# thierrydumas/context_adaptive_neural_network_based_prediction

Hardware: AMD Instinct MI355X
Metric: pnn_intra_pred_blocks_per_s (higher is better)
Workload: dtype f32; 1 GPU; configs[1]: 8x8 fully-connected PNN, batch 4096; batch_per_gpu=4096, global_batch=4096, weights=seeded random init (reference initialisers' statistics), parallelism=independent blocks sharded over ranks, no collective, timing=one region of K steps

## Files before the change

### context_adaptive_neural_network_based_prediction_amd/_lib.py

```python
import ctypes
import os

_HERE = os.path.dirname(os.path.abspath(__file__))
LIB_PATH = os.environ.get("PNN_LIB_PATH") or os.path.join(_HERE, "libpnn_hip.so")

f32p = ctypes.POINTER(ctypes.c_float)
i32p = ctypes.POINTER(ctypes.c_int32)
u8p = ctypes.POINTER(ctypes.c_uint8)
vp = ctypes.c_void_p
ci = ctypes.c_int


class TbDev(ctypes.Structure):
    _fields_ = [("origin", ctypes.c_int64), ("stride", ctypes.c_int32), ("above_mask", ctypes.c_uint32),
                ("left_units", ctypes.c_int32), ("reserved", ctypes.c_int32)]


BACKEND = ctypes.CFUNCTYPE(ci, vp, ci, f32p, f32p, ci, i32p, f32p)

SERVICE_SIGNATURES = {
    "pnn_service_run_backend": (ci, [ctypes.c_char_p, BACKEND, vp, ci, ci, ctypes.POINTER(ci), ctypes.POINTER(ctypes.c_long)]),
    "pnn_service_run": (ci, [ctypes.c_char_p, vp, ci, ci, ctypes.POINTER(ci), ctypes.POINTER(ctypes.c_long)]),
    "pnn_service_run_table": (ci, [ctypes.c_char_p, ctypes.c_char_p, ci, ctypes.c_float, ci, ci, ci, ctypes.POINTER(ci), ctypes.POINTER(ctypes.c_long)]),
    "pnn_client_connect": (ci, [ctypes.POINTER(vp), ctypes.c_char_p]),
    "pnn_client_predict_pel": (ci, [vp, ci, f32p, f32p, i32p, ci]),
    "pnn_client_predict_f32": (ci, [vp, ci, f32p, f32p, f32p]),
    "pnn_client_cache_stats": (ci, [vp, ctypes.POINTER(ctypes.c_long), ctypes.POINTER(ctypes.c_long)]),
    "pnn_client_arithmetic_tag": (ci, [vp, ci, ctypes.c_char_p, ctypes.c_size_t]),
    "pnn_client_close": (None, [vp]),
}

SIGNATURES = {
    "pnn_create_empty": (ci, [ctypes.POINTER(vp), ctypes.c_float, ci]),
    "pnn_create": (ci, [ctypes.POINTER(vp), ctypes.c_char_p, ci, ctypes.c_float, ci]),
    "pnn_load_model_file": (ci, [vp, ctypes.c_char_p]),
    "pnn_load_model_params": (ci, [vp, ci, ci, f32p, ctypes.c_size_t]),
    "pnn_model_info": (ci, [vp, ci, ctypes.POINTER(ci), ctypes.POINTER(ci), ctypes.POINTER(ctypes.c_long)]),
    "pnn_destroy": (None, [vp]),
    "pnn_last_error": (ctypes.c_char_p, [vp]),
    "pnn_mean": (ctypes.c_float, [vp]),
    "pnn_set_option": (ci, [vp, ctypes.c_char_p, ctypes.c_long]),
    "pnn_num_split_configs": (ci, []),
    "pnn_num_f32_configs": (ci, []),
    "pnn_check_range": (ci, [vp, vp, ctypes.POINTER(ctypes.c_long)]),
    "pnn_last_call_issued_flops": (ci, [vp, ctypes.POINTER(ctypes.c_double)]),
    "pnn_arithmetic_tag": (ci, [vp, ctypes.c_char_p, ctypes.c_size_t]),
    "pnn_host_alloc": (ci, [ctypes.POINTER(vp), ctypes.c_size_t]),
    "pnn_host_free": (None, [vp]),
    "pnn_streams_on_distinct_queues": (ci, [ctypes.POINTER(vp), ci]),
    "pnn_streams_release": (None, [ctypes.POINTER(vp), ci]),
    "pnn_cache_stats": (ci, [vp, ctypes.POINTER(ctypes.c_long), ctypes.POINTER(ctypes.c_long)]),
    "pnn_predict_fc": (ci, [vp, ci, f32p, ci, f32p]),
    "pnn_predict_conv": (ci, [vp, ci, f32p, f32p, ci, f32p]),
    "pnn_predict_pel": (ci, [vp, ci, f32p, f32p, ci, i32p, ci]),
    "pnn_predict_f32_pel": (ci, [vp, ci, f32p, f32p, ci, f32p, i32p]),
    "pnn_extract_context": (ci, [i32p, f32p, f32p, u8p] + [ci] * 8 + [ctypes.c_float]),
    "pnn_parse_model_table": (ci, [ctypes.c_char_p, ctypes.POINTER(ci), ctypes.POINTER(ci), ctypes.POINTER(ci),
                                   ctypes.POINTER(ctypes.c_char_p), ci]),
    "pnn_predict_fc_device": (ci, [vp, ci, vp, ci, vp, vp]),
    "pnn_predict_conv_device": (ci, [vp, ci, vp, vp, ci, vp, vp]),
    "pnn_make_tb_desc": (ci, [ctypes.POINTER(TbDev), ctypes.c_int64, ctypes.c_int32, u8p, ci, ci, ci]),
    "pnn_gather_device": (ci, [vp, ci, ci, vp, ci, vp, ci, vp, ctypes.c_long, vp, ctypes.c_long, vp]),
    "pnn_predict_tbs_device": (ci, [vp, ci, vp, ci, vp, ci, vp, vp, vp]),
    "pnn_block_cost_device": (ci, [vp, ci, vp, ci, vp, ci, vp, ci, vp, vp]),
    "pnn_predict_tbs_cost_device": (ci, [vp, ci, vp, vp, ci, vp, ci, ci, vp, vp, vp]),
    "pnn_hevc_intra_predict": (ci, [u8p, ci, ci, ci, ci, u8p]),
    "pnn_hevc_mode_uses_smoothing": (ci, [ci, ci]),
    "pnn_hevc_smoothed_reference_host": (ci, [vp, ci, ci, ci, ci, vp, ctypes.POINTER(ci)]),
    "pnn_hevc_intra_predict_hm": (ci, [u8p, ci, ci, ci, ci, ci, u8p]),
    "pnn_hevc_best_mode_device": (ci, [vp, ci, vp, ci, ci, vp, ci, vp, vp, vp, vp, vp]),
    "pnn_hevc_best_mode_hm_device": (ci, [vp, ci, vp, ci, ci, vp, ci, ci, vp, vp, vp, vp, vp]),
    "pnn_first_pass_list_size": (ci, [ci]),
    "pnn_hevc_mode_hads_host": (ci, [vp, ci, ci, vp, ci, ci, vp, vp, vp, vp, vp]),
    "pnn_hevc_mode_hads_device": (ci, [vp, ci, vp, ci, ci, vp, ci, vp, vp, vp, vp, vp, vp]),
    "pnn_hevc_mode_hads_hm_host": (ci, [vp, ci, ci, vp, ci, ci, vp, ci, vp, vp, vp, vp]),
    "pnn_hevc_mode_hads_hm_device": (ci, [vp, ci, vp, ci, ci, vp, ci, vp, ci, vp, vp, vp, vp, vp]),
    "pnn_first_pass_picture_pairs_device": (ci, [vp, ci, vp, vp, ci, ci, ci, vp, vp, ci, ci, ci, vp, vp, vp, vp, vp, vp]),
    "pnn_first_pass_picture_pairs_hm_device": (ci, [vp, ci, vp, vp, ci, ci, ci, vp, vp, ci, ci, ci, vp, ci, vp, vp, vp, vp, vp]),
    "pnn_ipfcns_forward_host": (ci, [ci, f32p, f32p, ci, ci, f32p]),
    "pnn_ipfcns_load": (ci, [vp, ci, f32p, ctypes.c_size_t]),
    "pnn_ipfcns_forward_device": (ci, [vp, ci, vp, ci, vp, vp]),
    "pnn_ipfcns_predict_device": (ci, [vp, ci, vp, ci, ci, ci, vp, vp, ci, vp, vp, vp, vp, vp, vp]),
    "pnn_score_pictures_device": (ci, [vp, ci, vp, ci, ci, ci, vp, vp, ci, ci, ci, vp, vp, vp, vp, vp, vp, vp, vp]),
    "pnn_score_picture_pairs_device": (ci, [vp, ci, vp, vp, ci, ci, ci, vp, vp, ci, ci, ci, vp, vp, vp, vp, vp, vp, vp, vp]),
    "pnn_score_picture_pairs_hm_device": (ci, [vp, ci, vp, vp, ci, ci, ci, vp, vp, ci, ci, ci, ci, vp, vp, vp, vp, vp, vp, vp, vp]),
    "pnn_score_f32_device": (ci, [vp, ci, vp, vp, ci, ci, ci, vp, vp, ci, vp, vp, vp]),
    "pnn_trquant_host": (ci, [vp, vp, ci, ci, ctypes.POINTER(ci), ci, vp, vp, vp, vp]),
    "pnn_trquant_stages_host": (ci, [vp, vp, ci, ci, vp, vp, vp, vp]),
    "pnn_trquant_device": (ci, [vp, ci, vp, vp, ci, ctypes.POINTER(ci), ci, vp, vp, vp, vp, vp]),
    "pnn_trquant_rate_host": (ci, [vp, vp, ci, ci, vp, ctypes.POINTER(ci), ci, vp, vp, vp, vp, vp]),
    "pnn_cabac_rate_levels_host": (ci, [vp, ci, ci, ci, ctypes.POINTER(ctypes.c_uint64)]),
    "pnn_trquant_rate_device": (ci, [vp, ci, vp, vp, ci, vp, ctypes.POINTER(ci), ci, vp, vp, vp, vp, vp, vp]),
    "pnn_sign_hide_unit_host": (ci, [vp, vp, vp, ci, ci]),
    "pnn_trquant_sdh_host": (ci, [vp, vp, ci, ci, vp, ctypes.POINTER(ci), ci, vp, vp, vp, vp, vp, ci]),
    "pnn_trquant_stages_sdh_host": (ci, [vp, vp, ci, ci, ci, ci, vp, vp, vp, vp, vp, vp]),
    "pnn_cabac_rate_levels_sdh_host": (ci, [vp, ci, ci, ci, ci, ctypes.POINTER(ctypes.c_uint64)]),
    "pnn_trquant_sdh_device": (ci, [vp, ci, vp, vp, ci, vp, ctypes.POINTER(ci), ci, vp, vp, vp, vp, vp, ci, vp]),
    "pnn_hm_intra_lambda": (ctypes.c_double, [ci]),
    "pnn_rd_pass_host": (ci, [vp, ci, ci, vp, ci, ci, vp, ci, ctypes.POINTER(ci), ci, ctypes.POINTER(ctypes.c_double), ci] + [vp] * 7),
    "pnn_rd_pass_workspace_bytes": (ctypes.c_size_t, [ci, ci, ci]),
    "pnn_rd_pass_device": (ci, [vp, ci, vp, ci, ci, vp, ci, vp, ci, ctypes.POINTER(ci), ci, ctypes.POINTER(ctypes.c_double), ci] + [vp] * 8 +
                           [ctypes.c_size_t, vp]),
    "pnn_rd_pass_picture_pairs_device": (ci, [vp, ci, vp, vp, ci, ci, ci, vp, vp, ci, ci, ci, vp, ci, ctypes.POINTER(ci), ci,
                                              ctypes.POINTER(ctypes.c_double), ci] + [vp] * 8 + [ctypes.c_size_t, vp]),
    "pnn_trquant_rdoq_host": (ci, [vp, vp, ci, ci, vp, ctypes.POINTER(ci), ci, vp, vp, vp, vp, vp, ci, ci, ctypes.POINTER(ctypes.c_double)]),
    "pnn_trquant_stages_rdoq_host": (ci, [vp, vp, ci, ci, ci, ci, ci, ctypes.c_double, ci, vp, vp, vp, vp, vp, vp]),
    "pnn_rdoq_unit_host": (ci, [vp, ci, ci, ci, ctypes.c_double, ci, ci, vp, ctypes.POINTER(ctypes.c_int32)]),
    "pnn_rdoq_est_bits_host": (ci, [ci, ci, vp]),
    "pnn_trquant_rdoq_device": (ci, [vp, ci, vp, vp, ci, vp, ctypes.POINTER(ci), ci, vp, vp, vp, vp, vp, ci, ci, ctypes.POINTER(ctypes.c_double),
                                     vp]),
    "pnn_rd_pass_rdoq_host": (ci, [vp, ci, ci, vp, ci, ci, vp, ci, ctypes.POINTER(ci), ci, ctypes.POINTER(ctypes.c_double), ci, ci] + [vp] * 7),
    "pnn_rd_pass_rdoq_device": (ci, [vp, ci, vp, ci, ci, vp, ci, vp, ci, ctypes.POINTER(ci), ci, ctypes.POINTER(ctypes.c_double), ci, ci] +
                                [vp] * 8 + [ctypes.c_size_t, vp]),
    "pnn_rd_pass_rdoq_picture_pairs_device": (ci, [vp, ci, vp, vp, ci, ci, ci, vp, vp, ci, ci, ci, vp, ci, ctypes.POINTER(ci), ci,
                                                   ctypes.POINTER(ctypes.c_double), ci, ci] + [vp] * 8 + [ctypes.c_size_t, vp]),
    "pnn_rd_pass_slot_count": (ci, [ci, ci]),
    "pnn_intra_mode_signal_host": (ci, [vp, vp, ci, ci, ci, vp, vp, vp, vp]),
    "pnn_first_pass_signal_host": (ci, [vp, ci, ci, vp, ci, ci, vp, ci, ctypes.POINTER(ci), ci, ctypes.POINTER(ctypes.c_double), vp, vp, vp, vp, vp]),
    "pnn_rd_pass_signal_host": (ci, [vp, ci, ci, vp, ci, ci, vp, ci, ctypes.POINTER(ci), ci, ctypes.POINTER(ctypes.c_double), ci, ci, ci, vp, vp] +
                                [vp] * 9),
    "pnn_rd_pass_signal_workspace_bytes": (ctypes.c_size_t, [ci, ci, ci, ci]),
    "pnn_rd_pass_signal_device": (ci, [vp, ci, vp, ci, ci, vp, ci, vp, ci, ctypes.POINTER(ci), ci, ctypes.POINTER(ctypes.c_double), ci, ci, ci,
                                       vp, vp] + [vp] * 10 + [ctypes.c_size_t, vp]),
    "pnn_rd_pass_signal_picture_pairs_device": (ci, [vp, ci, vp, vp, ci, ci, ci, vp, vp, ci, ci, ci, vp, ci, ctypes.POINTER(ci), ci,
                                                     ctypes.POINTER(ctypes.c_double), ci, ci, ci, vp, vp] + [vp] * 10 + [ctypes.c_size_t, vp]),
    "pnn_last_call_stats": (ci, [vp, ctypes.POINTER(ci), ctypes.POINTER(ctypes.c_double), ctypes.POINTER(ci)]),
    "pnn_launch_times": (ci, [vp, ci, ctypes.POINTER(ci), ctypes.POINTER(ctypes.c_double), ctypes.POINTER(ctypes.c_double)]),
}

_lib = None
SKIP_TORCH = False


def lib():
    global _lib
    if _lib is None:
        if not os.path.exists(LIB_PATH):
            raise ImportError("%s is missing: build it with `python -c 'import __graft_entry__ as g; g.build()'` "
                              "(or `make -C %s/csrc`). There is no CPU fallback." % (LIB_PATH, _HERE))
        if not SKIP_TORCH:
            try:
                import torch
            except ImportError:
                pass
        L = ctypes.CDLL(LIB_PATH)
        for name, (res, args) in list(SIGNATURES.items()) + list(SERVICE_SIGNATURES.items()):
            if os.environ.get("PNN_LIB_PATH") and not hasattr(L, name):
                continue
            fn = getattr(L, name)
            fn.restype = res
            fn.argtypes = args
        _lib = L
    return _lib


class PnnError(RuntimeError):
    pass


def check(rc, ctx=None):
    if rc != 0:
        msg = lib().pnn_last_error(ctx)
        raise PnnError("libpnn_hip error %d: %s" % (rc, msg.decode() if msg else "?"))
```

### context_adaptive_neural_network_based_prediction_amd/csrc/pnn_abi.cpp

```cpp
#include "pnn_ctx.h"

#include <algorithm>
#include <cmath>
#include <cstdarg>
#include <cstdio>
#include <cstdlib>
#include <cstring>
#include <ctime>
#include <condition_variable>
#include <mutex>
#include <thread>

using namespace pnn;

namespace pnn { std::recursive_mutex& unsafe_calls_lock() { static std::recursive_mutex m; return m; } }
namespace pnn { thread_local const LaunchEvents* g_launch_events = nullptr; thread_local double g_last_issued_frac = 1.0; }
namespace { thread_local std::string g_create_error; }
namespace pnn {

const DeviceInfo& device_info()
{
    static DeviceInfo cache[16];
    static std::once_flag filled[16];
    int dev = 0;
// ... 89 lines not shown
            HIPCHK(c, launch_gather(g, s));
            c->stat_launches++;
        }
        rc = run_net(c, m, ab, pa, lf, pl, nb, d_out_f32 ? d_out_f32 + b0 * w2 : nullptr, d_dst ? d_dst + b0 * w2 : nullptr, s, split_ctx);
        c->lazy = pnn_ctx::LazyGather();
        if (rc) return rc;
    }
    return PNN_OK;
}

}

namespace {

Model* model_for(pnn_ctx* c, int width, int want_fc , int* rc)
{
    const int idx = width_index(width);
    if (!c) { *rc = PNN_E_ARG; return nullptr; }
    if (idx < 0 || !c->models[idx]) { *rc = fail(c, PNN_E_MODEL, "no model loaded for width %d", width); return nullptr; }
    Model* m = c->models[idx];
    if (want_fc >= 0 && (int)m->is_fc != want_fc) {
        *rc = fail(c, PNN_E_MODEL, "model for width %d is %s", width, m->is_fc ? "fully-connected" : "convolutional");
        return nullptr;
    }
    *rc = PNN_OK;
    return m;
}

int wait_stream(pnn_ctx* c, hipStream_t s)
{
    HIPCHK(c, hipStreamSynchronize(s));
    return PNN_OK;
}

int wait_done_flag(pnn_ctx* c, hipStream_t s, long n = 1, int width = 4)
{
    const unsigned* const flag0 = reinterpret_cast<const unsigned*>(c->h_range) + (c->done_nflags > 0 ? pnn_ctx::kDoneFlag0 : 1);
    const int nflags = c->done_nflags > 0 ? c->done_nflags : 1;
    int first_open = 0;
    auto raised = [&]() {
        while (first_open < nflags && __atomic_load_n(flag0 + first_open, __ATOMIC_ACQUIRE) == c->done_seq) ++first_open;
        return first_open == nflags;
    };
    if (c->opt_wait_sleep) {
        constexpr double kMarginUs = 14.0, kMinSleepUs = 12.0;
        int b = 0;
        while ((2L << b) <= n && b < 11) b++;
        const int wi = width_index(width) < 0 ? 0 : width_index(width);
        double& ema = c->wait_ema_us[wi][b];
        timespec t0, t1;
        clock_gettime(CLOCK_MONOTONIC, &t0);
        const double nap = ema - kMarginUs;
        bool overslept = false;
        if (nap >= kMinSleepUs) {
            timespec ts{0, (long)(nap * 1e3)};
            nanosleep(&ts, nullptr);
            overslept = raised();
        }
        for (long spins = 0; !raised(); spins++) {
            if (spins < 400000) { __builtin_ia32_pause(); continue; }
            HIPCHK(c, hipStreamSynchronize(s));
            if (!raised()) return fail(c, PNN_E_HIP, "the pass finished without raising its completion flag");
            break;
        }
        clock_gettime(CLOCK_MONOTONIC, &t1);
        const double us = (t1.tv_sec - t0.tv_sec) * 1e6 + (t1.tv_nsec - t0.tv_nsec) * 1e-3;
        ema = overslept ? ema * 0.85 : (ema == 0.0 ? us : 0.9 * ema + 0.1 * us);
        return PNN_OK;
    }
    for (long spins = 0; !raised(); spins++) {
        if (spins < 200000) { __builtin_ia32_pause(); continue; }
        HIPCHK(c, hipStreamSynchronize(s));
        if (!raised()) return fail(c, PNN_E_HIP, "the pass finished without raising its completion flag");
        break;
    }
    return PNN_OK;
}

template <typename Pass>
int range_fallback(pnn_ctx* c, long n, Pass pass, hipStream_t s)
{
    constexpr long kPerBlockMax = 256;
    *c->h_range = 0;
    c->range_fallbacks++;
    const long keep = c->opt_precision;
    int rc = PNN_OK;
    if (n == 1 || n > kPerBlockMax) {
        c->opt_precision = 0;
        rc = pass(0, n);
        c->opt_precision = keep;
        if (rc) return rc;
        HIPCHK(c, hipStreamSynchronize(s));
        return PNN_OK;
    }
    for (long i = 0; i < n; i++) {
        if ((rc = pass(i, 1))) return rc;
        HIPCHK(c, hipStreamSynchronize(s));
        if (!*c->h_range) continue;
        *c->h_range = 0;
        c->opt_precision = 0;
        rc = pass(i, 1);
        c->opt_precision = keep;
        if (rc) return rc;
        HIPCHK(c, hipStreamSynchronize(s));
    }
    return PNN_OK;
}

struct PnnwHeader { char magic[4]; uint32_t version, width, is_fc; uint64_t n_params, reserved; };

enum OptionEffect { kStore, kRetune, kNewTuneGen };

int set_canonical_order(pnn_ctx* c, long value)
{
    if (value != 1) return fail(c, PNN_E_ARG, "canonical_order = %ld: the kernels with another summation order were removed; 1 is the only mode", value);
    return PNN_OK;
}

int set_stream_priority(pnn_ctx* c, long value)
{
    HIPCHK(c, hipSetDevice(c->device));
    int least = 0, greatest = 0;
    HIPCHK(c, hipDeviceGetStreamPriorityRange(&least, &greatest));
    const int pr = value < 0 ? greatest : value > 0 ? least : (least + greatest) / 2;
    hipStream_t ns = nullptr;
    HIPCHK(c, hipStreamCreateWithPriority(&ns, hipStreamNonBlocking, pr));
    if (c->stream) { (void)hipStreamSynchronize(c->stream); if (c->stream_owned) (void)hipStreamDestroy(c->stream); }
    c->stream = ns; c->stream_owned = true;
    return PNN_OK;
}

int set_stream(pnn_ctx* c, long value)
{
    if (!value) return fail(c, PNN_E_ARG, "stream = NULL");
    HIPCHK(c, hipSetDevice(c->device));
    if (c->stream) { (void)hipStreamSynchronize(c->stream); if (c->stream_owned) (void)hipStreamDestroy(c->stream); }
    c->stream = reinterpret_cast<hipStream_t>(value); c->stream_owned = false;
    return PNN_OK;
}

int set_cache_mb(pnn_ctx* c, long value) { c->opt_cache_mb = value; c->cache_hits = c->cache_misses = 0; return PNN_OK; }
int set_ws_cap_mb(pnn_ctx* c, long value) { c->ws_cap_bytes = (size_t)value << 20; return PNN_OK; }

struct OptionRow { const char* name; long pnn_ctx::*field; const char* env; OptionEffect effect; int (*set)(pnn_ctx*, long); };
const OptionRow kOptions[] = {
    {"precision",            &pnn_ctx::opt_precision,           "PNN_PRECISION",        kStore,       nullptr},
    {"canonical_order",      nullptr,                           nullptr,                kStore,       set_canonical_order},
    {"f32_small",            &pnn_ctx::opt_f32_small,           "PNN_F32_SMALL",        kStore,       nullptr},
    {"f32_small_max_tiles",  &pnn_ctx::opt_f32_small_tiles,     "PNN_F32_SMALL_TILES",  kStore,       nullptr},
    {"fc_out_f32",           &pnn_ctx::opt_fc_out_f32,          nullptr,                kStore,       nullptr},
    {"chain_io",             &pnn_ctx::opt_chain_io,            "PNN_CHAIN_IO",         kStore,       nullptr},
    {"tails",                &pnn_ctx::opt_tails,               "PNN_TAILS",            kStore,       nullptr},
    {"f32_cfg",              &pnn_ctx::opt_f32_cfg,             "PNN_F32_CFG",          kStore,       nullptr},
    {"f32_seg_mode",         &pnn_ctx::opt_f32_seg_mode,        "PNN_F32_SEG_MODE",     kRetune,      nullptr},
    {"f32_persist",          &pnn_ctx::opt_f32_persist,         "PNN_F32_PERSIST",      kRetune,      nullptr},
    {"f32_overlap",          &pnn_ctx::opt_f32_overlap,         "PNN_F32_OVERLAP",      kStore,       nullptr},
    {"fuse_last",            &pnn_ctx::opt_fuse_last,           "PNN_FUSE_LAST",        kStore,       nullptr},
    {"seg_fold",             &pnn_ctx::opt_seg_fold,            nullptr,                kStore,       nullptr},
    {"f32_small_deep",       &pnn_ctx::opt_f32_small_deep,      "PNN_F32_SMALL_DEEP",   kStore,       nullptr},
    {"sp_cfg",               &pnn_ctx::opt_sp_cfg,              nullptr,                kStore,       nullptr},
    {"ring",                 &pnn_ctx::opt_ring,                "PNN_RING",             kRetune,      nullptr},
    {"convimg",              &pnn_ctx::opt_convimg,             "PNN_CONVIMG",          kRetune,      nullptr},
    {"small",                &pnn_ctx::opt_small,               "PNN_SMALL",            kStore,       nullptr},
    {"small_max_tiles",      &pnn_ctx::opt_small_tiles,         nullptr,                kStore,       nullptr},
    {"fuse_first",           &pnn_ctx::opt_fuse_first,          "PNN_FUSE_FIRST",       kRetune,      nullptr},
    {"fuse_tail",            &pnn_ctx::opt_fuse_tail,           "PNN_FUSE_TAIL",        kRetune,      nullptr},
    {"ring_pm",              &pnn_ctx::opt_ring_pm,             "PNN_RING_PM",          kRetune,      nullptr},
    {"autotune",             &pnn_ctx::opt_autotune,            "PNN_AUTOTUNE",         kNewTuneGen,  nullptr},
    {"host_slice",           &pnn_ctx::opt_host_slice,          nullptr,                kStore,       nullptr},
    {"pair",                 &pnn_ctx::opt_pair,                nullptr,                kStore,       nullptr},
    {"branch_streams",       &pnn_ctx::opt_branch_streams,      "PNN_BRANCH_STREAMS",   kStore,       nullptr},
    {"fuse_gather",          &pnn_ctx::opt_fuse_gather,         "PNN_FUSE_GATHER",      kStore,       nullptr},
    {"cache_mb",             &pnn_ctx::opt_cache_mb,            "PNN_CACHE_MB",         kStore,       set_cache_mb},
    {"flag_wait",            &pnn_ctx::opt_flag_wait,           "PNN_FLAG_WAIT",        kStore,       nullptr},
    {"stream_priority",      nullptr,                           nullptr,                kStore,       set_stream_priority},
    {"stream",               nullptr,                           nullptr,                kStore,       set_stream},
    {"wait_sleep",           &pnn_ctx::opt_wait_sleep,          "PNN_WAIT_SLEEP",       kStore,       nullptr},
    {"graphs",               &pnn_ctx::opt_graphs,              "PNN_GRAPHS",           kStore,       nullptr},
    {"max_chunk",            &pnn_ctx::opt_max_chunk,           "PNN_MAX_CHUNK",        kStore,       nullptr},
    {"ws_cap_mb",            nullptr,                           nullptr,                kStore,       set_ws_cap_mb},
    {"time_launches",        &pnn_ctx::opt_time_launches,       nullptr,                kStore,       nullptr},
};

}

extern "C" {

int pnn_create_empty(pnn_ctx** out, float mean, int device)
{
    PNN_UNSAFE_CALLS_GUARD;
    if (!out) return fail(nullptr, PNN_E_ARG, "`out` is NULL");
    *out = nullptr;
    int ndev = 0;
    if (hipGetDeviceCount(&ndev) != hipSuccess || ndev <= 0)
        return fail(nullptr, PNN_E_HIP, "no HIP device is visible: libpnn_hip.so has no CPU fallback");
    if (device < 0 || device >= ndev) return fail(nullptr, PNN_E_ARG, "device %d out of range [0, %d)", device, ndev);
    pnn_ctx* c = new pnn_ctx();
    c->device = device; c->mean = mean;
    if (hipSetDevice(device) != hipSuccess || hipStreamCreateWithFlags(&c->stream, hipStreamNonBlocking) != hipSuccess) {
        delete c;
        return fail(nullptr, PNN_E_HIP, "cannot initialise HIP device %d", device);
    }
    for (const OptionRow& o : kOptions)
        if (o.env)
            if (const char* e = getenv(o.env)) c->*o.field = atol(e);
    if (hipHostMalloc((void**)&c->h_range, (pnn_ctx::kDoneFlag0 + pnn_ctx::kDoneFlagsMax) * 4, hipHostMallocDefault) != hipSuccess) {
        pnn_destroy(c);
        return fail(nullptr, PNN_E_NOMEM, "hipHostMalloc of the range flag failed");
    }
    *c->h_range = 0;
    for (int i = 1; i < pnn_ctx::kDoneFlag0 + pnn_ctx::kDoneFlagsMax; i++) c->h_range[i] = 0;
    if (hipMalloc((void**)&c->d_done, 256) != hipSuccess || hipMemset(c->d_done, 0, 256) != hipSuccess) {
        pnn_destroy(c);
        return fail(nullptr, PNN_E_NOMEM, "hipMalloc of the completion counter failed");
    }
    if (hipMalloc((void**)&c->d_seg_cnt, pnn_ctx::kCntWords * 4) != hipSuccess || hipMemset(c->d_seg_cnt, 0, pnn_ctx::kCntWords * 4) != hipSuccess) {
        pnn_destroy(c);
        return fail(nullptr, PNN_E_NOMEM, "hipMalloc of the K-segment counters failed");
    }
    if (hipMalloc(&c->d_zero, 4096) != hipSuccess || hipMemset(c->d_zero, 0, 4096) != hipSuccess) {
        pnn_destroy(c);
        return fail(nullptr, PNN_E_NOMEM, "hipMalloc of the zero page failed");
    }
    *out = c;
    return PNN_OK;
}

int pnn_load_model_params(pnn_ctx* c, int width, int is_fc, const float* params, size_t n)
{
    if (!c || !params) return fail(c, PNN_E_ARG, "NULL argument");
    const int idx = width_index(width);
    if (idx < 0) return fail(c, PNN_E_ARG, "width %d is not in {4, 8, 16, 32, 64}", width);
    HIPCHK(c, hipSetDevice(c->device));
    Model* m = nullptr;
    const int rc = build_model(c, width, is_fc, params, n, &m);
    if (rc) return rc;
    PNN_UNSAFE_CALLS_GUARD;
    free_model(c->models[idx]);
    c->models[idx] = m;
    c->tuned.clear(); c->tune_gen++;
    cache_clear(c);
    return PNN_OK;
}

int pnn_load_model_file(pnn_ctx* c, const char* path)
{
    if (!c || !path) return fail(c, PNN_E_ARG, "NULL argument");
    std::vector<char> data;
    if (!read_file(path, &data)) return fail(c, PNN_E_IO, "The model file at \"%s\" cannot be loaded.", path);
    if (data.size() < sizeof(PnnwHeader)) return fail(c, PNN_E_IO, "%s: truncated header", path);
    PnnwHeader h;
    memcpy(&h, data.data(), sizeof h);
    if (memcmp(h.magic, "PNNW", 4) || h.version != 1) return fail(c, PNN_E_IO, "%s is not a PNNW v1 file", path);
    if (data.size() != sizeof h + h.n_params * 4) return fail(c, PNN_E_IO, "%s: size does not match its header", path);
    std::vector<float> params(h.n_params);
    memcpy(params.data(), data.data() + sizeof h, h.n_params * 4);
    return pnn_load_model_params(c, (int)h.width, (int)h.is_fc, params.data(), params.size());
}

int pnn_create(pnn_ctx** out, const char* table_path, int use_pair, float mean, int device)
{
    if (!out) return fail(nullptr, PNN_E_ARG, "`out` is NULL");
    *out = nullptr;
    std::vector<TableEntry> entries;
    std::string err;
    int rc = parse_table(table_path, &entries, &err);
    if (rc) return fail(nullptr, rc, "%s", err.c_str());
    bool have_pair = false;
    for (const TableEntry& e : entries) have_pair |= e.is_pair != 0;
    const int want_pair = (have_pair && use_pair) ? 1 : 0;
    pnn_ctx* c = nullptr;
    if ((rc = pnn_create_empty(&c, mean, device))) return rc;
    std::string dir(table_path);
    const size_t slash = dir.find_last_of('/');
    dir = slash == std::string::npos ? std::string(".") : dir.substr(0, slash);
    static const int widths[5] = {4, 8, 16, 32, 64};
    for (int wi = 0; wi < 5; wi++) {
        const TableEntry* hit = nullptr;
        for (const TableEntry& e : entries)
            if (e.width == widths[wi] && e.is_pair == want_pair && e.channel == 0) hit = &e;
        if (!hit) {
            rc = fail(nullptr, PNN_E_MODEL, "model table has no (%d, %s, luminance) entry", widths[wi], want_pair ? "pair" : "single");
            break;
        }
        std::string p = hit->path;
        if (!p.empty() && p[0] != '/') {
            FILE* f = fopen((dir + "/" + p).c_str(), "rb");
            if (f) { fclose(f); p = dir + "/" + p; }
        }
        rc = pnn_load_model_file(c, p.c_str());
        if (rc) { g_create_error = c->err; break; }
        const Model* m = c->models[wi];
        if (m->width != widths[wi]) { rc = fail(nullptr, PNN_E_MODEL, "%s holds a width-%d model, table says %d", p.c_str(), m->width, widths[wi]); break; }
    }
    if (rc) { pnn_destroy(c); return rc; }
    *out = c;
    return PNN_OK;
}

void pnn_destroy(pnn_ctx* c)
{
    if (!c) return;
    PNN_UNSAFE_CALLS_GUARD;
    (void)hipSetDevice(c->device);
    if (c->stream) (void)hipStreamSynchronize(c->stream);
    cache_clear(c);
    for (Model*& m : c->models) { free_model(m); m = nullptr; }
    for (Model*& m : c->ipfcns) { free_model(m); m = nullptr; }
    for (DevBuf& b : c->ws) if (b.p) (void)hipFree(b.p);
    for (DevBuf& b : c->ipfcns_ws) if (b.p) (void)hipFree(b.p);
    for (DevBuf& b : c->score_ws) if (b.p) (void)hipFree(b.p);
    for (DevBuf& b : c->stage_in) if (b.p) (void)hipFree(b.p);
    for (DevBuf& b : c->stage_out) if (b.p) (void)hipFree(b.p);
    if (c->stage_tbs.p) (void)hipFree(c->stage_tbs.p);
    for (auto& b : c->seg_part) if (b.p) (void)hipFree(b.p);
    if (c->d_zero) (void)hipFree(c->d_zero);
    if (c->d_done) (void)hipFree(c->d_done);
    if (c->d_seg_cnt) (void)hipFree(c->d_seg_cnt);
    if (c->copy_in) {
        (void)hipStreamDestroy(c->copy_in); (void)hipStreamDestroy(c->copy_out);
        for (int i = 0; i < 2; i++) { (void)hipEventDestroy(c->ev_in[i]); (void)hipEventDestroy(c->ev_pass[i]); (void)hipEventDestroy(c->ev_out[i]); }
    }
    for (pnn::DevBuf* b : {&c->stage2_in[0], &c->stage2_in[1], &c->stage2_out[0], &c->stage2_out[1]}) if (b->p) (void)hipFree(b->p);
    if (c->side_stream) { (void)hipStreamSynchronize(c->side_stream); (void)hipStreamDestroy(c->side_stream); }
    if (c->ev_fork) (void)hipEventDestroy(c->ev_fork);
    if (c->ev_join) (void)hipEventDestroy(c->ev_join);
    if (c->h_pin) (void)hipHostFree(c->h_pin);
    if (c->h_range) (void)hipHostFree(c->h_range);
    if (c->stream && c->stream_owned) (void)hipStreamDestroy(c->stream);
    delete c;
}

const char* pnn_last_error(const pnn_ctx* c) { return c ? c->err.c_str() : g_create_error.c_str(); }
float pnn_mean(const pnn_ctx* c) { return c ? c->mean : 0.f; }

int pnn_model_info(const pnn_ctx* c, int width, int* is_fc, int* n_layers, long* n_params)
{
    const int idx = width_index(width);
    if (!c || idx < 0 || !c->models[idx]) return PNN_E_MODEL;
    if (is_fc) *is_fc = c->models[idx]->is_fc;
    if (n_layers) *n_layers = c->models[idx]->n_layers;
    if (n_params) *n_params = c->models[idx]->n_params;
    return PNN_OK;
}

int pnn_arithmetic_tag(const pnn_ctx* c, char* out, size_t bytes)
{
    if (!c || !out || bytes == 0) return PNN_E_ARG;
    if (c->opt_precision == 0)
        snprintf(out, bytes, "pnn-order-6:f32:fmaf-chain k=0,8,1,9..7,15 per 16:kseg %d/%d:fc-kseg %d:fc-out-seg 160", kSegDepth, kSegMinDepth, 16 * kFcSegChunks);
    else
        snprintf(out, bytes, "pnn-order-5:split-f16x3:hi*hi,hi*lo,lo*hi per 16:fc-out-seg %d", 16 * kFuseSegChunks);
    return PNN_OK;
}

int pnn_num_split_configs(void) { return tapgemm_sp_num_cfgs() + convimg_sp_num_cfgs() + tapgemm_ring_num_cfgs(); }
int pnn_num_f32_configs(void) { return tapgemm_f32_num_cfgs(); }

int pnn_set_option(pnn_ctx* c, const char* name, long value)
{
    if (!c || !name) return PNN_E_ARG;
    PNN_UNSAFE_CALLS_GUARD;
    const OptionRow* o = std::find_if(std::begin(kOptions), std::end(kOptions), [name](const OptionRow& r) { return !strcmp(r.name, name); });
    if (o == std::end(kOptions)) return fail(c, PNN_E_ARG, "unknown option %s", name);
    if (o->set) {
        if (const int rc = o->set(c, value)) return rc;
    } else {
        c->*o->field = value;
    }
    if (o->effect == kRetune) c->tuned.clear();
    if (o->effect != kStore) c->tune_gen++;
    cache_clear(c);
    return PNN_OK;
}

int pnn_last_call_stats(const pnn_ctx* c, int* n_gemm, double* flops, int* n_launches)
{
    if (!c) return PNN_E_ARG;
    if (n_gemm) *n_gemm = c->stat_gemm_launches;
    if (flops) *flops = c->stat_gemm_flops;
    if (n_launches) *n_launches = c->stat_launches;
    return PNN_OK;
}

int pnn_last_call_issued_flops(const pnn_ctx* c, double* flops)
{
    if (!c || !flops) return PNN_E_ARG;
    *flops = c->stat_gemm_flops - c->stat_gemm_flops_skipped;
    return PNN_OK;
}

int pnn_launch_times(pnn_ctx* c, int kind, int* n_launches, double* total_us, double* total_flops)
{
    if (!c) return PNN_E_ARG;
    int n = 0;
    double us = 0, fl = 0;
    std::vector<pnn_ctx::LaunchRec> keep;
    for (pnn_ctx::LaunchRec& r : c->launch_recs) {
        if (r.kind != kind) { keep.push_back(r); continue; }
        HIPCHK(c, hipEventSynchronize(r.e1));
        float ms = 0.f;
        HIPCHK(c, hipEventElapsedTime(&ms, r.e0, r.e1));
        us += ms * 1e3; fl += r.flops; n++;
        (void)hipEventDestroy(r.e0);
        (void)hipEventDestroy(r.e1);
    }
    c->launch_recs.swap(keep);
    if (n_launches) *n_launches = n;
    if (total_us) *total_us = us;
    if (total_flops) *total_flops = fl;
    return PNN_OK;
}


int pnn_predict_fc_device(pnn_ctx* c, int width, const float* d_ctx, int n, float* d_out, void* stream)
{
    int rc;
    Model* m = model_for(c, width, 1, &rc);
    if (!m) return rc;
    if (n < 0 || (n > 0 && (!d_ctx || !d_out))) return fail(c, PNN_E_ARG, "bad buffers / batch size");
    HIPCHK(c, hipSetDevice(c->device));
    if ((rc = pending_range_error(c))) return rc;
    reset_stats(c);
    hipStream_t s = (hipStream_t)stream;
    return run_net(c, m, d_ctx, 5L * width * width, nullptr, 0, n, d_out, nullptr, s);
}

int pnn_predict_conv_device(pnn_ctx* c, int width, const float* d_above, const float* d_left, int n, float* d_out, void* stream)
{
    int rc;
    Model* m = model_for(c, width, 0, &rc);
    if (!m) return rc;
    if (n < 0 || (n > 0 && (!d_above || !d_left || !d_out))) return fail(c, PNN_E_ARG, "bad buffers / batch size");
    HIPCHK(c, hipSetDevice(c->device));
    if ((rc = pending_range_error(c))) return rc;
    reset_stats(c);
    hipStream_t s = (hipStream_t)stream;
    return run_net(c, m, d_above, 3L * width * width, d_left, 2L * width * width, n, d_out, nullptr, s);
}

int pnn_gather_device(pnn_ctx* c, int width, int unit, const void* d_plane, int pel_bytes, const pnn_tb_dev* d_tbs, int n,
                      float* d_above, long pitch_above, float* d_left, long pitch_left, void* stream)
{
    if (!c) return PNN_E_ARG;
    if (width_index(width) < 0 || (unit != 4 && unit != 2) || n < 0 || (n > 0 && (!d_plane || !d_tbs || !d_above || !d_left)))
        return fail(c, PNN_E_ARG, "bad gather arguments");
    if (pel_bytes != 4 && pel_bytes != 1) return fail(c, PNN_E_ARG, "pel_bytes must be 4 (HM Pel) or 1 (uint8)");
    HIPCHK(c, hipSetDevice(c->device));
    GatherParams g;
    g.plane = d_plane; g.pel_bytes = pel_bytes; g.tbs = reinterpret_cast<const TbDev*>(d_tbs); g.N = n; g.w = width;
    g.unit = unit; g.mean = c->mean; g.above = d_above; g.left = d_left; g.pitch_above = pitch_above; g.pitch_left = pitch_left;
    g.split = 0;
    HIPCHK(c, launch_gather(g, (hipStream_t)stream));
    return PNN_OK;
}

int pnn_predict_tbs_device(pnn_ctx* c, int width, const void* d_plane, int pel_bytes, const pnn_tb_dev* d_tbs, int n,
                           int32_t* d_dst, float* d_out_f32, void* stream)
{
    int rc;
    Model* m = model_for(c, width, -1, &rc);
    if (!m) return rc;
    if (n < 0 || (n > 0 && (!d_plane || !d_tbs || (!d_dst && !d_out_f32)))) return fail(c, PNN_E_ARG, "bad buffers / batch size");
    HIPCHK(c, hipSetDevice(c->device));
    if ((rc = pending_range_error(c))) return rc;
    reset_stats(c);
    return tbs_pass(c, m, d_plane, pel_bytes, d_tbs, n, d_dst, d_out_f32, (hipStream_t)stream);
}

int pnn_block_cost_device(pnn_ctx* c, int width, const void* d_org_plane, int pel_bytes, const pnn_tb_dev* d_tbs, int n,
                          const int32_t* d_pred, int hadamard, uint32_t* d_cost, void* stream)
{
    if (!c) return PNN_E_ARG;
    if (width_index(width) < 0 || n < 0 || (n > 0 && (!d_org_plane || !d_tbs || !d_pred || !d_cost))) return fail(c, PNN_E_ARG, "bad cost arguments");
    if (pel_bytes != 4 && pel_bytes != 1) return fail(c, PNN_E_ARG, "pel_bytes must be 4 (HM Pel) or 1 (uint8)");
    HIPCHK(c, hipSetDevice(c->device));
    BlockCostParams b;
    b.org_plane = d_org_plane; b.pel_bytes = pel_bytes; b.tbs = reinterpret_cast<const TbDev*>(d_tbs); b.N = n; b.w = width;
    b.pred = d_pred; b.hadamard = hadamard; b.cost = d_cost;
    HIPCHK(c, launch_block_cost(b, (hipStream_t)stream));
    return PNN_OK;
}

int pnn_predict_tbs_cost_device(pnn_ctx* c, int width, const void* d_plane, const void* d_org_plane, int pel_bytes,
                                const pnn_tb_dev* d_tbs, int n, int hadamard, uint32_t* d_cost, int32_t* d_dst, void* stream)
{
    if (!c) return PNN_E_ARG;
    if (n > 0 && (!d_org_plane || !d_cost)) return fail(c, PNN_E_ARG, "bad cost arguments");
    int rc;
    if (!d_dst && n > 0) {
        if ((rc = dev_reserve(c, c->stage_out[1], (size_t)n * width * width * 4))) return rc;
        d_dst = (int32_t*)c->stage_out[1].p;
    }
    if ((rc = pnn_predict_tbs_device(c, width, d_plane, pel_bytes, d_tbs, n, d_dst, nullptr, stream))) return rc;
    rc = pnn_block_cost_device(c, width, d_org_plane, pel_bytes, d_tbs, n, d_dst, hadamard, d_cost, stream);
    if (rc == PNN_OK) c->stat_launches++;
    return rc;
}


static uint64_t hash_bytes(const void* data, size_t bytes, uint64_t h = 0x9e3779b97f4a7c15ull)
{
    const unsigned char* p = static_cast<const unsigned char*>(data);
    size_t i = 0;
    for (; i + 8 <= bytes; i += 8) {
        uint64_t v;
        memcpy(&v, p + i, 8);
        h = (h ^ v) * 0xff51afd7ed558ccdull;
        h ^= h >> 32;
    }
    for (; i < bytes; i++) h = (h ^ p[i]) * 0x100000001b3ull;
    return h ^ (h >> 29);
}

static bool all_finite(const float* x, size_t n)
{
    uint32_t bad = 0;
    for (size_t i = 0; i < n; i++) {
        uint32_t u;
        memcpy(&u, x + i, 4);
        bad |= (uint32_t)((u & 0x7f800000u) == 0x7f800000u);
    }
    return bad == 0;
}

static int host_predict(pnn_ctx* c, Model* m, const float* above, const float* left, int n, float* out, int32_t* dst, int dst_stride);

static int host_predict_sliced(pnn_ctx* c, Model* m, const float* above, const float* left, int n, float* out, int32_t* dst, int dst_stride, long slice)
{
    const int w = m->width;
    const long w2 = (long)w * w;
    const size_t pa = (size_t)(m->is_fc ? 5 : 3) * w2, pl = m->is_fc ? 0 : (size_t)2 * w2;
    HIPCHK(c, hipSetDevice(c->device));
    reset_stats(c);
// ... 447 lines not shown
```

### context_adaptive_neural_network_based_prediction_amd/csrc/pnn_ctx.h

```cpp
#pragma once
#include "../../include/pnn_hip.h"
#include "pnn_kernels.h"
#include "pnn_host.h"

#include <functional>
#include <map>
#include <mutex>
#include <tuple>
#include <string>
#include <vector>

namespace pnn {

constexpr int kHidden = 1200;
constexpr int kFuseSegChunks = 10;
inline int strides_for(int w, int* st)
{
    switch (w) {
    case 4: st[0] = 1; st[1] = 1; return 2;
    case 8: st[0] = 2; st[1] = 1; return 2;
    case 16: st[0] = 2; st[1] = 1; st[2] = 2; st[3] = 1; return 4;
    case 32: st[0] = 2; st[1] = 2; st[2] = 1; st[3] = 2; st[4] = 1; return 5;
    case 64: st[0] = 2; st[1] = 2; st[2] = 2; st[3] = 2; st[4] = 1; return 5;
    default: return -1;
    }
}

inline int width_index(int w)
{
    switch (w) { case 4: return 0; case 8: return 1; case 16: return 2; case 32: return 3; case 64: return 4; default: return -1; }
}

inline bool ipfcns_dims(int w, int* K, int* H)
{
    switch (w) {
    case 4: *H = 512; break;
    case 8: case 16: *H = 1024; break;
    case 32: *H = 2048; break;
    default: return false;
    }
    *K = 64 + 32 * w;
    return true;
}
inline int ipfcns_index(int w) { return w == 4 ? 0 : w == 8 ? 1 : w == 16 ? 2 : w == 32 ? 3 : -1; }
inline long ipfcns_n_params(int w)
{
    int K, H;
    if (!ipfcns_dims(w, &K, &H)) return -1;
    const long o = (long)w * w;
    return (long)H * K + 2L * H + 2L * ((long)H * H + 2L * H) + o * H + o;
}

struct DevBuf {
    void* p = nullptr;
    size_t bytes = 0;
};

struct GemmLayer {
    TapGemmParams proto{};
    float* d_w = nullptr;
    float* d_w_ch = nullptr;
    float* d_w_sp = nullptr;
    float sp_inv_scale = 1.f;
    float* d_bias = nullptr;
    double k_total = 0;
    int nseg = 1;
    int fc_seg_chunks = 0;
    long out_per_block = 0;
};
struct Conv1Layer { Conv1Params proto{}; float* d_w = nullptr; float* d_w_sp = nullptr; float sp_inv_scale = 1.f; int npad = 0; float* d_bias = nullptr; long out_per_block = 0; };
struct TConv1Layer { TConv1Params proto{}; float* d_w = nullptr; };
struct MergerLayer { MergerParams proto{}; float* d_w = nullptr; float* d_bias = nullptr; };

struct Model {
    int width = 0;
    bool is_fc = false;
    long n_params = 0;
    int n_layers = 0;
    std::vector<GemmLayer> fc;
    Conv1Layer first[2];
    std::vector<GemmLayer> branch[2];
    MergerLayer merger;
    std::vector<GemmLayer> tconv;
    TConv1Layer last;
    int C = 0;
    long pmax = 0;
    float* d_slope[3] = {nullptr, nullptr, nullptr};
    std::vector<void*> allocs;
};

}

struct pnn_ctx {
    int device = 0;
    float mean = 0.f;
    hipStream_t stream = nullptr;
    pnn::Model* models[5] = {nullptr, nullptr, nullptr, nullptr, nullptr};
    pnn::Model* ipfcns[4] = {nullptr, nullptr, nullptr, nullptr};
    pnn::DevBuf ipfcns_ws[4];
    pnn::DevBuf score_ws[2];
    pnn::DevBuf ws[6];
    bool stream_owned = true;
    long opt_branch_streams = 1;
    hipStream_t side_stream = nullptr;
    hipEvent_t ev_fork = nullptr, ev_join = nullptr;
    pnn::DevBuf stage_in[2], stage_out[2], stage_tbs;
    pnn::DevBuf stage2_in[2], stage2_out[2];
    hipStream_t copy_in = nullptr, copy_out = nullptr;
    hipEvent_t ev_in[2] = {nullptr, nullptr}, ev_pass[2] = {nullptr, nullptr}, ev_out[2] = {nullptr, nullptr};
    long opt_host_slice = 0;
    pnn::DevBuf seg_part[2];
    struct CacheEntry { uint64_t hash = 0; bool valid = false; std::vector<float> in, out; std::vector<int32_t> pel; };
    std::vector<CacheEntry> cache[5];
    long opt_cache_mb = 0;
    long cache_hits = 0, cache_misses = 0;
    char* h_pin = nullptr;
    struct GraphEntry {
        hipGraphExec_t exec = nullptr;
        int uses = 0;
        bool failed = false, armed = false;
        unsigned seq = 0;
        int nflags = 0;
        int stat_gemm_launches = 0, stat_launches = 0;
        double stat_gemm_flops = 0, stat_gemm_flops_skipped = 0;
    };
    std::map<std::tuple<const void*, int, int>, GraphEntry> graphs;
    long opt_graphs = 0;
    void* d_zero = nullptr;
    long opt_max_chunk = 0;
    long opt_precision = 0;
    long opt_sp_cfg = -1;
    long opt_f32_small = 1;
    long opt_fc_out_f32 = 1;
    long opt_seg_fold = 1;
    long opt_f32_small_deep = 1;
    unsigned* d_seg_cnt = nullptr;
    bool seg_cnt_dirty = false;
    static constexpr int kSegCntTiles = 2048;
    static constexpr int kTailCnt = 2048, kCntWords = 2 * kSegCntTiles + kTailCnt;
    long opt_tails = 1;
    long opt_chain_io = 1;
    long opt_f32_small_tiles = 1024;
    long opt_f32_overlap = 1;
    long opt_f32_cfg = -1;
    long opt_fuse_first = 1;
    long opt_fuse_last = 1;
    long opt_f32_seg_mode = 0;
    long opt_f32_persist = -1;
    long opt_ring = 1;
    long opt_small = 1;
    long opt_small_tiles = 512;
    long opt_pair = 1;
    long opt_convimg = 1;
    long opt_autotune = 2;
    std::map<std::pair<const void*, long>, int> tuned;
    long tune_gen = 0;
    std::map<std::pair<const void*, long>, long> overlap_ready;
    long opt_time_launches = 0;
    struct LaunchRec { hipEvent_t e0, e1; int kind; double flops; };
    std::vector<LaunchRec> launch_recs;
    int* h_range = nullptr;
    long range_fallbacks = 0;
    const float* host_input = nullptr;
    struct LazyGather { const void* plane = nullptr; const void* tbs = nullptr; int pel_bytes = 0, unit = 0; } lazy;
    long opt_fuse_gather = 1;
    long opt_fuse_tail = 1;
    unsigned* d_done = nullptr;
    unsigned done_seq = 0;
    unsigned done_seq_alloc = 0;
    bool done_want = false, done_last_chunk = true, done_armed = false;
    int done_nflags = 0;
    static constexpr int kDoneFlag0 = 16, kDoneFlagsMax = 512;
    long opt_flag_wait = 1;
    long opt_wait_sleep = 0;
    double wait_ema_us[5][12] = {};
    long opt_ring_pm = 1;
    size_t ws_cap_bytes = (size_t)8 << 30;
    static constexpr int kDiagLaunches = 32, kDiagWgs = 2048;
    void* diag_stamps = nullptr;
    int diag_launch = 0;
    std::vector<std::string> diag_names;
    std::vector<int> diag_wgs;
    std::vector<double> diag_k;
    std::string err;
    int stat_gemm_launches = 0, stat_launches = 0;
    double stat_gemm_flops = 0;
    double stat_gemm_flops_skipped = 0;
};

namespace pnn {

int fail(pnn_ctx* c, int code, const char* fmt, ...);
std::recursive_mutex& unsafe_calls_lock();
#define PNN_UNSAFE_CALLS_GUARD std::lock_guard<std::recursive_mutex> unsafe_guard_(pnn::unsafe_calls_lock())

#define HIPCHK(c, expr)                                                                             \
    do {                                                                                            \
        hipError_t e_ = (expr);                                                                     \
        if (e_ != hipSuccess) return pnn::fail((c), PNN_E_HIP, "%s failed: %s", #expr, hipGetErrorString(e_)); \
    } while (0)

int dev_reserve(pnn_ctx* c, DevBuf& b, size_t bytes);
void reset_stats(pnn_ctx* c);
int pending_range_error(pnn_ctx* c);
int tbs_pass(pnn_ctx* c, Model* m, const void* d_plane, int pel_bytes, const pnn_tb_dev* d_tbs, long n, int32_t* d_dst, float* d_out_f32,
             hipStream_t s);
int build_model(pnn_ctx* c, int width, int is_fc, const float* params, size_t n, Model** out);
int build_ipfcns_model(pnn_ctx* c, int width, const float* params, size_t n, Model** out);
void free_model(Model* m);
int convimg_images(const TapGemmParams& p, const TileCfg& t, bool one_tap);
int choose_cfg_convimg(const TapGemmParams& p, bool one_tap);
bool pnn_ring_few_images(const TapGemmParams& p, long M, double k_total);
int choose_cfg_ring(const TapGemmParams& p, long M, bool one_tap, double k_total, bool fused = false);
int choose_cfg_sp(const pnn_ctx* c, long M, int cout, int ncls, int cin, double k_total);
int choose_cfg_f32(const pnn_ctx* c, long M, int cout, int ncls, int cin, double k_total, bool fused, double* cost_out = nullptr);
inline DoneSignal take_done_signal(pnn_ctx* c)
{
    if (!c->done_want || !c->done_last_chunk || !c->d_done) return DoneSignal{nullptr, nullptr, 0, 0};
    c->done_armed = true;
    c->done_nflags = 0;
    c->done_seq = ++c->done_seq_alloc;
    return DoneSignal{c->d_done, reinterpret_cast<unsigned*>(c->h_range) + 1, c->done_seq, 0};
}
inline DoneSignal take_done_signal_per_wg(pnn_ctx* c, int nwg)
{
    if (nwg < 1 || nwg > pnn_ctx::kDoneFlagsMax) return take_done_signal(c);
    if (!c->done_want || !c->done_last_chunk || !c->d_done) return DoneSignal{nullptr, nullptr, 0, 0};
    c->done_armed = true;
    c->done_nflags = nwg;
    c->done_seq = ++c->done_seq_alloc;
    return DoneSignal{nullptr, reinterpret_cast<unsigned*>(c->h_range) + pnn_ctx::kDoneFlag0, c->done_seq, 1};
}
int tuned_cfg(pnn_ctx* c, const void* key, long M, int ncodes, int rule, const std::function<bool(int)>& legal,
              const std::function<hipError_t(int)>& launch, hipStream_t s, int* cfg, float* best_us);
bool env_debug();
bool env_profile();
bool env_f32s_diag();
bool env_f32_diag();
bool env_sp_diag();
void* diag_stamp_slot(pnn_ctx* c, const char* name, long wgs, double k);
int diag_f32_small(pnn_ctx* c, const GemmLayer& L, const TapGemmParams& ps, int nseg, const float* host_rows, hipStream_t s);
int diag_f32_tiles(pnn_ctx* c, const GemmLayer& L, const TapGemmParams& p, int tile, bool fused, int par_segs, hipStream_t s);
int diag_sp(pnn_ctx* c, const GemmLayer& L, const TapGemmParams& p, int cfg, hipStream_t s);
long chunk_blocks(const pnn_ctx* c, const Model* m);
bool pass_uses_split(const pnn_ctx* c, const Model* m, long nb);
bool conv_pass_fuses_first(pnn_ctx* c, Model* m, long nb);
long ipfcns_chunk(const pnn_ctx* c, const Model* m);
int ipfcns_pass(pnn_ctx* c, const Model* m, const float* d_x, long n, float* d_fc4, hipStream_t s);
int run_net(pnn_ctx* c, Model* m, const float* d_a, long pitch_a, const float* d_l, long pitch_l, long n, float* d_out,
            int32_t* d_dst, hipStream_t s, bool ctx_is_split = false);

}
```

### context_adaptive_neural_network_based_prediction_amd/csrc/pnn_diag.cpp

```cpp
#include "pnn_ctx.h"

#include <algorithm>
#include <cmath>
#include <cstdio>
#include <cstdlib>
#include <vector>

namespace pnn {

bool env_debug() { static const bool on = getenv("PNN_DEBUG") != nullptr; return on; }
bool env_profile() { static const bool on = getenv("PNN_PROFILE") != nullptr; return on; }
bool env_f32s_diag() { static const bool on = getenv("PNN_F32S_DIAG") != nullptr; return on; }
bool env_f32_diag() { static const bool on = getenv("PNN_F32_DIAG") != nullptr; return on; }
bool env_sp_diag() { static const bool on = getenv("PNN_SP_DIAG") != nullptr; return on; }

void* diag_stamp_slot(pnn_ctx* c, const char* name, long wgs, double k)
{
    if (!c->diag_stamps || c->diag_launch >= pnn_ctx::kDiagLaunches || wgs > pnn_ctx::kDiagWgs) return nullptr;
    c->diag_names.push_back(name);
    c->diag_wgs.push_back((int)wgs);
    c->diag_k.push_back(k);
    return (char*)c->diag_stamps + (size_t)c->diag_launch++ * pnn_ctx::kDiagWgs * 64;
}

int diag_f32_small(pnn_ctx* c, const GemmLayer& L, const TapGemmParams& ps, int nseg, const float* host_rows, hipStream_t s)
{
    HIPCHK(c, hipStreamSynchronize(s));
    if (dev_reserve(c, c->stage_tbs, (size_t)4 << 20)) return PNN_E_NOMEM;
    HIPCHK(c, hipMemset(c->stage_tbs.p, 0, (size_t)4 << 20));
    TapGemmParams q = ps;
    q.Xlo = c->stage_tbs.p;
    HIPCHK(c, launch_tapgemm_f32_small(q, s, host_rows, (int)c->opt_f32_small_deep));
    HIPCHK(c, hipStreamSynchronize(s));
    const size_t nwg = std::min<size_t>((size_t)tapgemm_f32_small_tiles(ps), ((size_t)4 << 20) / 64);
    std::vector<unsigned long long> hbuf(8 * nwg);
    HIPCHK(c, hipMemcpy(hbuf.data(), c->stage_tbs.p, hbuf.size() * 8, hipMemcpyDeviceToHost));
    double cyc = 0, ticks = 0, chunks = 0;
    unsigned long long r0 = ~0ull, r1 = 0;
    for (size_t i = 0; i < nwg; i++) { cyc += (double)hbuf[8 * i]; ticks += (double)hbuf[8 * i + 1]; chunks += (double)hbuf[8 * i + 2]; r0 = std::min(r0, hbuf[8 * i + 3]); r1 = std::max(r1, hbuf[8 * i + 3] + hbuf[8 * i + 1]); }
    fprintf(stderr, "[pnn-f32s-diag] M=%ld K=%.0f N=%d ncls=%d nseg=%d: %zu WGs, loop %.0f cycles for %.0f chunks = %.0f cycles per chunk (160 = the chain), %.2f us, clock %.0f MHz; first loop start -> last loop end %.1f us\n",
            (long)ps.M, L.k_total, ps.Cout, ps.ncls, nseg, nwg, cyc / nwg, chunks / nwg, cyc / std::max(1.0, chunks), ticks / nwg / 100.0, cyc / std::max(1.0, ticks) * 100.0, (double)(r1 - r0) / 100.0);
    return PNN_OK;
}

int diag_f32_tiles(pnn_ctx* c, const GemmLayer& L, const TapGemmParams& p, int tile, bool fused, int par_segs, hipStream_t s)
{
    const TileCfg t = tapgemm_f32_cfg(tile);
    const long M = p.M;
    HIPCHK(c, hipStreamSynchronize(s));
    if (dev_reserve(c, c->stage_tbs, (size_t)16 << 20)) return PNN_E_NOMEM;
    TapGemmParams q = p;
    q.Xlo = c->stage_tbs.p;
    HIPCHK(c, hipMemset(c->stage_tbs.p, 0, (size_t)16 << 20));
    for (int rep = 0; rep < 400; rep++) HIPCHK(c, launch_tapgemm_f32(q, tile, fused, s));
    HIPCHK(c, hipStreamSynchronize(s));
    const size_t nwg = (size_t)((M + 128L * t.rt - 1) / (128L * t.rt)) * ((p.Cout + 32L * t.nt - 1) / (32L * t.nt)) * p.ncls * par_segs;
    std::vector<unsigned long long> hbuf(8 * nwg);
    HIPCHK(c, hipMemcpy(hbuf.data(), c->stage_tbs.p, hbuf.size() * 8, hipMemcpyDeviceToHost));
    double sum[4] = {0, 0, 0, 0};
    unsigned long long r0 = ~0ull, r1 = 0;
    for (size_t i = 0; i < nwg; i++) {
        for (int k = 0; k < 4; k++) sum[k] += (double)hbuf[8 * i + k];
        r0 = std::min(r0, hbuf[8 * i + 4]); r1 = std::max(r1, hbuf[8 * i + 4] + hbuf[8 * i + 3]);
    }
    size_t late = 0; unsigned long long life_max = 0;
    for (size_t i = 0; i < nwg; i++) { late += hbuf[8 * i + 4] > r0 + 500; life_max = std::max(life_max, hbuf[8 * i + 3]); }
    const double chunks = std::ceil(L.k_total / 16.0 / p.ncls / par_segs / t.kc) * t.kc;
    const double cyc = (sum[0] + sum[1] + sum[2]) / nwg, rt_ticks = sum[3] / nwg;
    fprintf(stderr, "[pnn-f32diag] M=%ld K=%.0f N=%d {%d,%d,%d}%s: %zu WGs; wave 0 mean cycles: prologue %.0f  loop %.0f (MFMA work %.0f = %.3f)  epilogue %.0f;"
            " lifetime %.1f us (max %.1f), in-kernel clock %.0f MHz; first start -> last end %.1f us, %zu workgroups start > 5 us late\n", M, L.k_total, p.Cout, t.rt, t.nt, t.kc, fused ? "+out" : "", nwg,
            sum[0] / nwg, sum[1] / nwg, chunks * 8 * t.rt * t.nt * 64, chunks * 8 * t.rt * t.nt * 64 / (sum[1] / nwg), sum[2] / nwg, rt_ticks / 100.0, (double)life_max / 100.0,
            cyc / (rt_ticks / 100.0), (double)(r1 - r0) / 100.0, late);
    return PNN_OK;
}

int diag_sp(pnn_ctx* c, const GemmLayer& L, const TapGemmParams& p, int cfg, hipStream_t s)
{
    HIPCHK(c, hipStreamSynchronize(s));
    const TileCfg tt = tapgemm_sp_cfg(cfg);
    const long M = p.M, bm = 32L * tt.rt * tt.wm, bn = 32L * tt.nt * (4 / tt.wm);
    const size_t nwg = (size_t)((M + bm - 1) / bm) * ((p.Cout + bn - 1) / bn) * p.ncls;
    std::vector<unsigned long long> h(4 * nwg);
    HIPCHK(c, hipMemcpy(h.data(), c->stage_tbs.p, h.size() * 8, hipMemcpyDeviceToHost));
    double sum[4] = {0, 0, 0, 0};
    for (size_t i = 0; i < nwg; i++) for (int k = 0; k < 4; k++) sum[k] += (double)h[4 * i + k];
    const double stages = std::ceil(L.k_total / 16.0 / p.ncls / tt.kc);
    fprintf(stderr, "[pnn-diag] M=%ld K=%.0f N=%d cfg {%d,%d,%d,wm%d}: per stage (cycles, wave 0 mean over %zu WGs): issue %.0f  mfma %.0f  store %.0f  barrier %.0f\n",
            M, L.k_total, p.Cout, tt.rt, tt.nt, tt.kc, tt.wm, nwg, sum[0] / nwg / stages, sum[1] / nwg / stages, sum[2] / nwg / stages, sum[3] / nwg / stages);
    return PNN_OK;
}

}
```

### context_adaptive_neural_network_based_prediction_amd/csrc/pnn_gemm_f32.hip

```cpp
#include "pnn_kernels.h"
#include "pnn_device_common.h"

#include <algorithm>
#include <cstdio>
#include <cstdlib>

namespace pnn {

typedef float f32x16 __attribute__((ext_vector_type(16)));

namespace {

__device__ __forceinline__ void dma16(const __amdgpu_buffer_rsrc_t& r, unsigned voff, unsigned soff, f32x4* l)
{
    __builtin_amdgcn_raw_ptr_buffer_load_lds(r, (__attribute__((address_space(3))) void*)l, 16, voff, soff, 0, 0);
}

template <int N>
__device__ __forceinline__ void wait_vm_le()
{
    asm volatile("s_waitcnt vmcnt(%0)" ::"n"(N) : "memory");
}

}

template <int RT, int NT, int KC, bool FUSE, int SEQ>
__device__ __forceinline__ void f32_tile(const TapGemmParams& p, f32x4* const lds, const int bx, const int by, const int bz, const int gx, const int gy)
{
    static_assert(KC >= 2 && KC % 2 == 0, "fragment sets alternate by chunk parity");
    constexpr int BM = 128 * RT, BN = 32 * NT;
    constexpr int E = 4 * BN;
    constexpr int SE = KC * E;
    constexpr int NDMA = SE / 64;
    constexpr int NPW = NDMA / 4;
    constexpr int W2R = BN / 4;
    static_assert(SE % 64 == 0 && NDMA % 4 == 0, "a stage is a whole number of wave instructions, the same number for every wave");
    constexpr int SLOTS = 8 * NT * RT;
    constexpr bool kCoalescedOut = true;
    f32x4* const W2s = lds + 3 * SE;

    const int tid = threadIdx.x;
    const int lane = tid & 63, wave = __builtin_amdgcn_readfirstlane(tid >> 6);
    const int l31 = lane & 31, h = lane >> 5;
    const int nseg = (!FUSE && !SEQ && p.nseg > 1) ? p.nseg : 1;
    const int cls = nseg > 1 ? bz / nseg : bz;
    const int seg = bz - cls * nseg;
    const int n0 = by * BN;
    const int m0 = bx * BM + wave * (32 * RT);
#ifdef PNN_F32_DIAG
    const unsigned long long dq0 = __builtin_amdgcn_s_memtime(), dr0 = __builtin_amdgcn_s_memrealtime();
    unsigned long long dq1 = 0, dq2 = 0;
#endif

    const int SP = p.SH * p.SW;
    const int cpt = p.Cin >> 4;
    const int t0 = p.tap_begin[cls], t1 = p.tap_begin[cls + 1];
    const int pmg = p.pm_groups;
    int pmi = 0, pmj = 0, mblk = 0;
    unsigned tmask = t1 - t0 >= 32 ? 0xffffffffu : (1u << (t1 - t0)) - 1u;
    unsigned smask = 0xffffffffu;
    if (nseg > 1) {
        const int base = (t1 - t0) / nseg, rem = (t1 - t0) - base * nseg;
        smask = ((1u << (base + (seg < rem ? 1 : 0))) - 1u) << (seg * base + (seg < rem ? seg : rem));
        tmask &= smask;
    }
    if (pmg) {
        const int gc = bx / (SP * 8), r = bx - gc * (SP * 8);
        const int c = gc < (pmg >> 3) ? 8 : (pmg & 7);
        const int pr = r / c;
        const int pos = SP <= 64 ? (int)((p.pos_order[pr >> 2] >> ((pr & 3) * 8)) & 0xffu) : pr;
        pmi = pos / p.SW;
        pmj = pos - pmi * p.SW;
        mblk = (gc * 8 + r - pr * c) * BM;
        unsigned m = 0;
        for (int t = t0; t < t1; t++) {
            const int tp = p.tap[t];
            const int iy = pmi * p.a + (tp >> 16), ix = pmj * p.a + (int)(short)(tp & 0xffff);
            if ((unsigned)iy < (unsigned)p.IH && (unsigned)ix < (unsigned)p.IW) m |= 1u << (t - t0);
        }
        m &= smask;
        tmask = m ? m : (smask & (0u - smask));
    }
    auto next_tap = [&](int t) {
        const unsigned rest = tmask & ~((2u << t) - 1u);
        return rest ? (int)__builtin_ctz(rest) : t;
    };
    int pb[RT], pi[RT], pj[RT];
    bool mv[RT];
#pragma unroll
    for (int rt = 0; rt < RT; rt++) {
        const int row = wave * (32 * RT) + rt * 32 + l31;
        if (pmg) {
            mv[rt] = mblk + row < p.nblk;
            pb[rt] = mv[rt] ? mblk + row : 0; pi[rt] = pmi; pj[rt] = pmj;
            continue;
        }
        const int mg = m0 + rt * 32 + l31;
        mv[rt] = mg < p.M;
        const int mc = mv[rt] ? mg : 0;
        if (SP == 1) { pb[rt] = mc; pi[rt] = 0; pj[rt] = 0; }
        else {
            const int b = mc / SP;
            const int r = mc - b * SP;
            pb[rt] = b;
            pi[rt] = r / p.SW;
            pj[rt] = r - pi[rt] * p.SW;
        }
    }
    const int nchunks = __builtin_popcount(tmask) * cpt;
    const int nstages = (nchunks + KC - 1) / KC;
    const int sq_n = SEQ != 0 ? p.nseg : 1, sq_base = (t1 - t0) / sq_n, sq_rem = (t1 - t0) - sq_base * sq_n;
    auto seg_stages = [&](int k) {
        const unsigned mk = ((1u << (sq_base + (k < sq_rem ? 1 : 0))) - 1u) << (k * sq_base + (k < sq_rem ? k : sq_rem));
        return __builtin_popcount(tmask & mk) * (cpt / KC);
    };
    int sq_k = 0, fold_at = SEQ == 1 ? seg_stages(0) : 0, sq_done = 0;

    const unsigned wbytes = (unsigned)p.chunk_begin[p.ncls] * 4u * (unsigned)p.Npad * 16u;
    const __amdgpu_buffer_rsrc_t wrsrc = __builtin_amdgcn_make_buffer_rsrc((void*)p.Wp, 0, wbytes, 0x00020000);
    const unsigned wcls = (unsigned)p.chunk_begin[cls] * 4u * (unsigned)p.Npad * 16u;
    const unsigned wchunk = 4u * (unsigned)p.Npad * 16u;
    int dt = (int)__builtin_ctz(tmask), dcc = 0;
    auto advance_d = [&]() {
        dcc += KC;
        if (dcc >= cpt) {
            const int n = next_tap(dt);
            if (n != dt) { dt = n; dcc = 0; } else dcc -= KC;
        }
    };
    unsigned bsrc[NPW];
#pragma unroll
    for (int ii = 0; ii < NPW; ii++) {
        const int i = wave + 4 * ii;
        const int e = 64 * i + lane;
        const int j = e / E, ee = e - j * E;
        const int q = ee / BN, nn = ee - q * BN;
        bsrc[ii] = (unsigned)(((j * 4 + q) * p.Npad + n0 + nn) << 4) + wcls;
    }
    auto dma_b = [&](int buf, int ii) {
        dma16(wrsrc, bsrc[ii], (unsigned)(dt * cpt + dcc) * wchunk, lds + buf * SE + 64 * (wave + 4 * ii));
    };

    const __amdgpu_buffer_rsrc_t xrsrc = __builtin_amdgcn_make_buffer_rsrc((void*)p.X, 0, p.x_bytes, 0x00020000);
    unsigned aoff[RT];
    auto tap_setup = [&](int tp) {
        const int dy = tp >> 16, dx = (int)(short)(tp & 0xffff);
#pragma unroll
        for (int rt = 0; rt < RT; rt++) {
            const int iy = pi[rt] * p.a + dy, ix = pj[rt] * p.a + dx;
            const bool ok = mv[rt] && (unsigned)iy < (unsigned)p.IH && (unsigned)ix < (unsigned)p.IW;
            const unsigned off = ((unsigned)((pb[rt] * p.IH + iy) * p.IW + ix) * (unsigned)p.Cin + (h << 3)) << 2;
            aoff[rt] = ok ? off : 0x80000000u;
        }
    };
    int lt = (int)__builtin_ctz(tmask), lcc = 0;
    tap_setup(p.tap[t0 + lt]);
    int ltp_next = p.tap[t0 + next_tap(lt)];
    auto load_a_chunk = [&](int j, f32x4 (&dst)[KC][RT][2]) {
        const int cj = lcc + j < cpt ? lcc + j : cpt - 1;
#pragma unroll
        for (int rt = 0; rt < RT; rt++) {
            dst[j][rt][0] = __builtin_bit_cast(f32x4, __builtin_amdgcn_raw_buffer_load_b128(xrsrc, aoff[rt], cj << 6, 0));
            dst[j][rt][1] = __builtin_bit_cast(f32x4, __builtin_amdgcn_raw_buffer_load_b128(xrsrc, aoff[rt] + 16u, cj << 6, 0));
        }
    };
    auto advance_a = [&]() {
        lcc += KC;
        if (lcc >= cpt) {
            const int n = next_tap(lt);
            if (n != lt) {
                lcc = 0;
                lt = n;
                tap_setup(ltp_next);
                ltp_next = p.tap[t0 + next_tap(lt)];
            }
        }
    };

    f32x16 acc[RT][NT];
    f32x16 total[SEQ ? RT : 1][SEQ ? NT : 1];
#pragma unroll
    for (int rt = 0; rt < RT; rt++)
#pragma unroll
        for (int nt = 0; nt < NT; nt++)
#pragma unroll
            for (int i = 0; i < 16; i++) {
                acc[rt][nt][i] = 0.f;
                if (SEQ) total[SEQ ? rt : 0][SEQ ? nt : 0][i] = 0.f;
            }
    auto fold_now = [&](bool first = false) {
#pragma unroll
        for (int rt = 0; rt < RT; rt++)
#pragma unroll
            for (int nt = 0; nt < NT; nt++)
#pragma unroll
                for (int i = 0; i < 16; i++) {
                    if (first) total[SEQ ? rt : 0][SEQ ? nt : 0][i] = acc[rt][nt][i];
                    else total[SEQ ? rt : 0][SEQ ? nt : 0][i] += acc[rt][nt][i];
                    acc[rt][nt][i] = 0.f;
                }
    };
    auto after_stage = [&]() {
        if (SEQ != 1) return;
        ++sq_done;
        if (sq_done != fold_at || sq_k >= sq_n - 1) return;
        fold_now();
        do { ++sq_k; fold_at += seg_stages(sq_k); } while (fold_at == sq_done && sq_k < sq_n - 1);
    };

    auto read_wf = [&](int buf, int j, int nt, f32x4 (&wf)[NT][2]) {
        wf[nt][0] = lds[buf * SE + j * E + (2 * h) * BN + nt * 32 + l31];
        wf[nt][1] = lds[buf * SE + j * E + (2 * h + 1) * BN + nt * 32 + l31];
    };

    f32x4 a0[KC][RT][2], a1[KC][RT][2];
    f32x4 wf0[NT][2], wf1[NT][2];
#pragma unroll
    for (int ii = 0; ii < NPW; ii++) dma_b(0, ii);
    advance_d();
#pragma unroll
    for (int j = 0; j < KC; j++) load_a_chunk(j, a0);
    advance_a();
#pragma unroll
    for (int ii = 0; ii < NPW; ii++) dma_b(1, ii);
    advance_d();
    if (FUSE) {
        const __amdgpu_buffer_rsrc_t w2rsrc = __builtin_amdgcn_make_buffer_rsrc((void*)p.W2p, 0, (unsigned)p.K2chunks * 4u * (unsigned)p.Npad2 * 16u, 0x00020000);
        for (int r = wave; r < W2R; r += 4) dma16(w2rsrc, (unsigned)(((n0 >> 2) + r) * p.Npad2 + lane) << 4, 0, W2s + r * 64);
    }
    static_assert(!FUSE || W2R % 4 == 0, "every wave fetches the same number of rows of the output layer's tile");
    wait_vm_le<NPW + (FUSE ? W2R / 4 : 0)>();
    __builtin_amdgcn_s_barrier();
#pragma unroll
    for (int nt = 0; nt < NT; nt++) read_wf(0, 0, nt, wf0);

    auto stage = [&](int buf, f32x4 (&acur)[KC][RT][2], f32x4 (&anxt)[KC][RT][2]) {
        const int buf1 = buf == 2 ? 0 : buf + 1, buf2 = buf == 0 ? 2 : buf - 1;
#pragma unroll
        for (int j = 0; j < KC; j++) {
            constexpr int kLast = KC - 1;
            const int d0 = j * NPW / KC, d1 = (j + 1) * NPW / KC;
            const int nops = 2 * NT + 2 * RT + (d1 - d0);
            if (j == kLast) {
                wait_vm_le<(2 * RT) * (KC - 1) + (KC - 1) * NPW / KC>();
                asm volatile("s_waitcnt lgkmcnt(0)" ::: "memory");
                __builtin_amdgcn_s_barrier();
            }
            f32x4 (&wc)[NT][2] = (j & 1) ? wf1 : wf0;
            f32x4 (&wn)[NT][2] = (j & 1) ? wf0 : wf1;
#pragma unroll
            for (int e = 0; e < 8; e++)
#pragma unroll
                for (int nt = 0; nt < NT; nt++)
#pragma unroll
                    for (int rt = 0; rt < RT; rt++) {
                        acc[rt][nt] = __builtin_amdgcn_mfma_f32_32x32x2f32(wc[nt][e >> 2][e & 3], acur[j][rt][e >> 2][e & 3], acc[rt][nt], 0, 0, 0);
                        const int sl = (e * NT + nt) * RT + rt;
                        const int k = (sl * nops + SLOTS - 1) / SLOTS;
                        if (k < nops && k * SLOTS / nops == sl) {
                            if (k < 2 * NT) {
                                const int fnt = k >> 1, fh = k & 1;
                                const int src = (j == kLast ? buf1 * SE : buf * SE + (j + 1) * E) + (2 * h + fh) * BN + fnt * 32 + l31;
                                wn[fnt][fh] = lds[src];
                            } else if (k < 2 * NT + 2 * RT) {
                                const int ar = (k - 2 * NT) >> 1, ah = (k - 2 * NT) & 1;
                                const int cj = lcc + j < cpt ? lcc + j : cpt - 1;
                                anxt[j][ar][ah] = __builtin_bit_cast(f32x4, __builtin_amdgcn_raw_buffer_load_b128(xrsrc, aoff[ar] + 16u * ah, cj << 6, 0));
                            } else {
                                dma_b(buf2, d0 + (k - 2 * NT - 2 * RT));
                            }
                        }
                        __builtin_amdgcn_sched_barrier(0);
                    }
        }
        advance_a();
        advance_d();
    };
#ifdef PNN_F32_DIAG
    dq1 = __builtin_amdgcn_s_memtime();
#endif
    auto tail = [&](int buf, f32x4 (&acur)[KC][RT][2], int nlive) {
#pragma unroll
        for (int j = 0; j < KC; j++) {
            if (j >= nlive) break;
            f32x4 (&wc)[NT][2] = (j & 1) ? wf1 : wf0;
            f32x4 (&wn)[NT][2] = (j & 1) ? wf0 : wf1;
#pragma unroll
            for (int e = 0; e < 8; e++)
#pragma unroll
                for (int nt = 0; nt < NT; nt++)
#pragma unroll
                    for (int rt = 0; rt < RT; rt++) {
                        acc[rt][nt] = __builtin_amdgcn_mfma_f32_32x32x2f32(wc[nt][e >> 2][e & 3], acur[j][rt][e >> 2][e & 3], acc[rt][nt], 0, 0, 0);
                        const int sl = (e * NT + nt) * RT + rt;
                        constexpr int nops = 2 * NT;
                        const int k = (sl * nops + SLOTS - 1) / SLOTS;
                        if (j + 1 < KC && k < nops && k * SLOTS / nops == sl)
                            wn[k >> 1][k & 1] = lds[buf * SE + (j + 1) * E + (2 * h + (k & 1)) * BN + (k >> 1) * 32 + l31];
                        __builtin_amdgcn_sched_barrier(0);
                    }
        }
    };
    const int nlive = nchunks - (nstages - 1) * KC;
    int s = 0, buf = 0;
    if (SEQ == 1) while (fold_at == 0 && sq_k < sq_n - 1) { ++sq_k; fold_at += seg_stages(sq_k); }
    if constexpr (SEQ == 2) {
        const bool one_tap_seq = t1 - t0 == 1;
        int last_live = 0;
        if (one_tap_seq) last_live = p.nseg - 1;
        else for (int k = 0; k < p.nseg; k++) if (seg_stages(k) > 0) last_live = k;
        for (int k = 0; k < last_live; k++) {
            const int spp = one_tap_seq ? (int)p.seg_chunks / KC : seg_stages(k);
            for (int i = 0; i < spp; i += 2) {
                stage(buf, a0, a1);
                buf = buf == 2 ? 0 : buf + 1;
                stage(buf, a1, a0);
                buf = buf == 2 ? 0 : buf + 1;
            }
            s += spp;
            if (k == 0) fold_now(true); else fold_now();
        }
    }
    for (; s + 2 < nstages; s += 2) {
        stage(buf, a0, a1);
        buf = buf == 2 ? 0 : buf + 1;
        after_stage();
        stage(buf, a1, a0);
        buf = buf == 2 ? 0 : buf + 1;
        after_stage();
    }
    if (s + 1 < nstages) {
        stage(buf, a0, a1);
        buf = buf == 2 ? 0 : buf + 1;
        after_stage();
        tail(buf, a1, nlive);
    } else {
        tail(buf, a0, nlive);
    }
    if (SEQ) {
#pragma unroll
        for (int rt = 0; rt < RT; rt++)
#pragma unroll
            for (int nt = 0; nt < NT; nt++)
#pragma unroll
                for (int i = 0; i < 16; i++) acc[rt][nt][i] = total[SEQ ? rt : 0][SEQ ? nt : 0][i] + acc[rt][nt][i];
    }
#ifdef PNN_F32_DIAG
    dq2 = __builtin_amdgcn_s_memtime();
    auto diag_out = [&]() {
        if (tid == 0 && p.Xlo) {
            unsigned long long* d = (unsigned long long*)p.Xlo + 8 * ((bz * gy + by) * gx + bx);
            d[0] = dq1 - dq0; d[1] = dq2 - dq1; d[2] = __builtin_amdgcn_s_memtime() - dq2; d[3] = __builtin_amdgcn_s_memrealtime() - dr0;
            d[4] = dr0;
        }
    };
#else
    auto diag_out = [&]() {};
#endif

    asm volatile("s_waitcnt vmcnt(0)" ::: "memory");
    if (FUSE && nstages < 2) __builtin_amdgcn_s_barrier();
    const int py = p.py[cls], px = p.px[cls];
    f32x4 bvs[NT][4];
#pragma unroll
    for (int nt = 0; nt < NT; nt++)
#pragma unroll
        for (int g = 0; g < 4; g++) {
            const int n = n0 + nt * 32 + 8 * g + 4 * h;
            bvs[nt][g] = *reinterpret_cast<const f32x4*>(p.bias + (n < p.Cout ? n : 0));
        }
    if (FUSE && p.W2p) {
        static_assert(!FUSE || RT == 1, "the fused output layer is written for one row tile per wave");
        constexpr int OT = 2;
        f32x16 acc2[OT];
#pragma unroll
        for (int ot = 0; ot < OT; ot++)
#pragma unroll
            for (int i = 0; i < 16; i++) acc2[ot][i] = 0.f;
#pragma unroll
        for (int nt = 0; nt < NT; nt++) {
            f32x4 w2[4][OT];
#pragma unroll
            for (int g = 0; g < 4; g++)
#pragma unroll
                for (int ot = 0; ot < OT; ot++) w2[g][ot] = W2s[(8 * nt + 2 * g + h) * 64 + ot * 32 + l31];
#pragma unroll
            for (int g = 0; g < 4; g++) {
                f32x4 v = (f32x4){acc[0][nt][4 * g], acc[0][nt][4 * g + 1], acc[0][nt][4 * g + 2], acc[0][nt][4 * g + 3]} + bvs[nt][g];
                if (p.act) { v[0] = leaky(v[0]); v[1] = leaky(v[1]); v[2] = leaky(v[2]); v[3] = leaky(v[3]); }
#pragma unroll
                for (int r = 0; r < 4; r++)
#pragma unroll
                    for (int ot = 0; ot < OT; ot++) acc2[ot] = __builtin_amdgcn_mfma_f32_32x32x2f32(w2[g][ot][r], v[r], acc2[ot], 0, 0, 0);
            }
        }
        if (mv[0]) {
            float* dst = p.part + ((size_t)by * p.M + (m0 + l31)) * 64;
#pragma unroll
            for (int ot = 0; ot < OT; ot++)
#pragma unroll
                for (int g = 0; g < 4; g++)
                    *reinterpret_cast<f32x4*>(dst + ot * 32 + 8 * g + 4 * h) =
                        (f32x4){acc2[ot][4 * g], acc2[ot][4 * g + 1], acc2[ot][4 * g + 2], acc2[ot][4 * g + 3]};
        }
        diag_out();
        return;
    }
    constexpr int TP = BN / 4 + 1;
    float* const Yo = (nseg > 1 && p.Y) ? p.Y + (size_t)seg * p.seg_stride : p.Y;
    if (kCoalescedOut && p.Y && !p.Yi && SP == 1) {
        asm volatile("s_waitcnt vmcnt(0)" ::: "memory");
        __syncthreads();
        f32x4* tile = lds + wave * (32 * RT * TP);
#pragma unroll
        for (int rt = 0; rt < RT; rt++)
#pragma unroll
            for (int nt = 0; nt < NT; nt++)
#pragma unroll
                for (int g = 0; g < 4; g++) {
                    f32x4 v = (f32x4){acc[rt][nt][4 * g], acc[rt][nt][4 * g + 1], acc[rt][nt][4 * g + 2], acc[rt][nt][4 * g + 3]} + bvs[nt][g];
                    if (p.act) { v[0] = leaky(v[0]); v[1] = leaky(v[1]); v[2] = leaky(v[2]); v[3] = leaky(v[3]); }
                    tile[(rt * 32 + l31) * TP + nt * 8 + 2 * g + h] = v;
                }
        __builtin_amdgcn_wave_barrier();
        const int cq = p.Cout >> 2, nq0 = n0 >> 2;
        const int rows = p.M - m0 < 32 * RT ? p.M - m0 : 32 * RT;
        f32x4* __restrict__ yo = reinterpret_cast<f32x4*>(Yo) + (size_t)m0 * cq + nq0;
#pragma unroll 4
        for (int i = lane; i < 32 * RT * (BN / 4); i += 64) {
            const int row = i / (BN / 4), col = i - row * (BN / 4);
            if (row < rows && nq0 + col < cq) store16_through(yo + (size_t)row * cq + col, tile[row * TP + col]);
        }
        diag_out();
        return;
    }
#pragma unroll
    for (int rt = 0; rt < RT; rt++) {
        if (!mv[rt]) continue;
        const int oy = pi[rt] * p.os + py, ox = pj[rt] * p.os + px;
        const size_t obase = (((size_t)pb[rt] * p.OH + oy) * p.OW + ox) * p.Cout;
#pragma unroll
        for (int nt = 0; nt < NT; nt++)
#pragma unroll
            for (int g = 0; g < 4; g++) {
                const int n = n0 + nt * 32 + 8 * g + 4 * h;
                if (n < p.Cout) {
                    f32x4 v = (f32x4){acc[rt][nt][4 * g], acc[rt][nt][4 * g + 1], acc[rt][nt][4 * g + 2], acc[rt][nt][4 * g + 3]} + bvs[nt][g];
                    if (p.act) { v[0] = leaky(v[0]); v[1] = leaky(v[1]); v[2] = leaky(v[2]); v[3] = leaky(v[3]); }
                    if (p.Y) *reinterpret_cast<f32x4*>(Yo + obase + n) = v;
                    if (p.Yi) {
                        int4 iv = make_int4(hm_round(v[0], p.mean), hm_round(v[1], p.mean), hm_round(v[2], p.mean), hm_round(v[3], p.mean));
                        *reinterpret_cast<int4*>(p.Yi + obase + n) = iv;
                    }
                }
            }
    }
    diag_out();
}

template <int RT, int NT, int KC, bool FUSE, int SEQ = 0>
__global__ __launch_bounds__(256) void tapgemm_f32_kernel(const TapGemmParams p)
{
    touch_kernargs<sizeof(TapGemmParams)>();
    extern __shared__ __attribute__((aligned(16))) f32x4 lds[];
    const int gx = p.grid_x, gy = p.grid_y, ntiles = gx * gy * p.grid_z;
    for (int lin = blockIdx.x; lin < ntiles; lin += gridDim.x) {
        if (lin != (int)blockIdx.x) __syncthreads();
        const int bx = lin % gx, rest = lin / gx;
        f32_tile<RT, NT, KC, FUSE, SEQ>(p, lds, bx, rest % gy, rest / gy, gx, gy);
    }
}

__global__ __launch_bounds__(64) void fc_out_f32_kernel(const TapGemmParams p)
{
    constexpr int NT = 5, OT = 2;
    const int lane = threadIdx.x, l31 = lane & 31, h = lane >> 5;
    const int m = blockIdx.x * 32 + l31, seg = blockIdx.y, n0 = seg * 32 * NT;
    const bool mv = m < p.M;
    const __amdgpu_buffer_rsrc_t xrsrc = __builtin_amdgcn_make_buffer_rsrc((void*)p.X, 0, p.x_bytes, 0x00020000);
    const __amdgpu_buffer_rsrc_t wrsrc = __builtin_amdgcn_make_buffer_rsrc((void*)p.Wp, 0, (unsigned)p.chunk_begin[1] * 4u * (unsigned)p.Npad * 16u, 0x00020000);
    f32x16 acc2[OT];
#pragma unroll
    for (int ot = 0; ot < OT; ot++)
#pragma unroll
        for (int i = 0; i < 16; i++) acc2[ot][i] = 0.f;
    f32x4 x[NT][4], w2[NT][4][OT];
#pragma unroll
    for (int nt = 0; nt < NT; nt++)
#pragma unroll
        for (int g = 0; g < 4; g++) {
            const int n = n0 + 32 * nt + 8 * g + 4 * h;
            const unsigned xo = (mv && n < p.Cin) ? ((unsigned)m * (unsigned)p.Cin + (unsigned)n) << 2 : 0x80000000u;
            x[nt][g] = __builtin_bit_cast(f32x4, __builtin_amdgcn_raw_buffer_load_b128(xrsrc, xo, 0, 0));
#pragma unroll
            for (int ot = 0; ot < OT; ot++)
                w2[nt][g][ot] = __builtin_bit_cast(f32x4, __builtin_amdgcn_raw_buffer_load_b128(wrsrc, (unsigned)((n >> 2) * p.Npad + ot * 32 + l31) << 4, 0, 0));
        }
#pragma unroll
    for (int nt = 0; nt < NT; nt++)
#pragma unroll
        for (int g = 0; g < 4; g++)
#pragma unroll
            for (int r = 0; r < 4; r++)
#pragma unroll
                for (int ot = 0; ot < OT; ot++) acc2[ot] = __builtin_amdgcn_mfma_f32_32x32x2f32(w2[nt][g][ot][r], x[nt][g][r], acc2[ot], 0, 0, 0);
    if (mv) {
        float* dst = p.part + ((size_t)seg * p.M + m) * 64;
#pragma unroll
        for (int ot = 0; ot < OT; ot++)
#pragma unroll
            for (int g = 0; g < 4; g++)
                *reinterpret_cast<f32x4*>(dst + ot * 32 + 8 * g + 4 * h) = (f32x4){acc2[ot][4 * g], acc2[ot][4 * g + 1], acc2[ot][4 * g + 2], acc2[ot][4 * g + 3]};
    }
}

hipError_t launch_fc_out_f32(const TapGemmParams& p, hipStream_t s, int* segments)
{
    if (p.M <= 0) return hipSuccess;
    const int segs = (p.Cin + 159) / 160;
    if (segments) *segments = segs;
    pnn_launch(fc_out_f32_kernel, dim3((p.M + 31) / 32, segs), dim3(64), 0, s, p);
    return hipGetLastError();
}

struct FcOutF32Args { TapGemmParams p; DoneSignal done; };
__global__ __launch_bounds__(512) void fc_out_f32_chain_kernel(const FcOutF32Args a)
{
    touch_kernargs<sizeof(FcOutF32Args)>();
#ifdef PNN_F32_DIAG
    const unsigned long long de0 = __builtin_amdgcn_s_memrealtime();
#endif
    const TapGemmParams& p = a.p;
    constexpr int NT = 5;
    __shared__ __attribute__((aligned(16))) float part[8][16][16];
    const int tid = threadIdx.x, lane = tid & 63, l15 = lane & 15, q = lane >> 4;
    const int z = __builtin_amdgcn_readfirstlane(tid >> 6);
    const int mblk = blockIdx.x * 16, nblk = blockIdx.y * 16;
    const int segs = (p.Cin + 159) / 160;
    const bool odd = (q >> 1) != 0;
#ifdef PNN_F32_DIAG
    unsigned long long dr0 = 0, dr1 = 0;
#endif
    f32x4 bias4 = {0.f, 0.f, 0.f, 0.f};
    if (z == 0 && nblk + 4 * q < p.Cout) bias4 = *reinterpret_cast<const f32x4*>(p.bias + nblk + 4 * q);
    if (z < segs) {
        const int m = mblk + l15, n0 = z * 32 * NT;
        const bool mv = m < p.M;
        const __amdgpu_buffer_rsrc_t xrsrc = __builtin_amdgcn_make_buffer_rsrc((void*)p.X, 0, p.x_bytes, 0x00020000);
        const __amdgpu_buffer_rsrc_t wrsrc = __builtin_amdgcn_make_buffer_rsrc((void*)p.Wp, 0, (unsigned)p.chunk_begin[1] * 4u * (unsigned)p.Npad * 16u, 0x00020000);
        f32x4 x[NT][4], w2[NT][4];
#pragma unroll
        for (int nt = 0; nt < NT; nt++)
#pragma unroll
            for (int g = 0; g < 4; g++) {
                const int n = n0 + 32 * nt + 8 * g + 4 * (q & 1);
                const unsigned xo = (mv && n < p.Cin) ? ((unsigned)m * (unsigned)p.Cin + (unsigned)n) << 2 : 0x80000000u;
                x[nt][g] = __builtin_bit_cast(f32x4, __builtin_amdgcn_raw_buffer_load_b128(xrsrc, xo, 0, 0));
                w2[nt][g] = __builtin_bit_cast(f32x4, __builtin_amdgcn_raw_buffer_load_b128(wrsrc, (unsigned)((n >> 2) * p.Npad + nblk + l15) << 4, 0, 0));
            }
        __builtin_amdgcn_sched_barrier(0);
        float xs[NT][4][2], ws[NT][4][2];
#pragma unroll
        for (int nt = 0; nt < NT; nt++)
#pragma unroll
            for (int g = 0; g < 4; g++) {
                xs[nt][g][0] = odd ? x[nt][g][1] : x[nt][g][0]; xs[nt][g][1] = odd ? x[nt][g][3] : x[nt][g][2];
                ws[nt][g][0] = odd ? w2[nt][g][1] : w2[nt][g][0]; ws[nt][g][1] = odd ? w2[nt][g][3] : w2[nt][g][2];
            }
        __builtin_amdgcn_sched_barrier(0);
#ifdef PNN_F32_DIAG
        dr0 = __builtin_amdgcn_s_memrealtime();
#endif
        f32x4 acc = {0.f, 0.f, 0.f, 0.f};
#pragma unroll
        for (int nt = 0; nt < NT; nt++)
#pragma unroll
            for (int g = 0; g < 4; g++) {
                acc = __builtin_amdgcn_mfma_f32_16x16x4f32(ws[nt][g][0], xs[nt][g][0], acc, 0, 0, 0);
                acc = __builtin_amdgcn_mfma_f32_16x16x4f32(ws[nt][g][1], xs[nt][g][1], acc, 0, 0, 0);
            }
        *reinterpret_cast<f32x4*>(&part[z][l15][4 * q]) = acc;
#ifdef PNN_F32_DIAG
        dr1 = __builtin_amdgcn_s_memrealtime();
#endif
    }
    __syncthreads();
    const int mg = mblk + l15, n = nblk + 4 * q;
    if (z == 0 && mg < p.M && n < p.Cout) {
        f32x4 sum = {0.f, 0.f, 0.f, 0.f};
        for (int t = 0; t < segs; t++) sum += *reinterpret_cast<const f32x4*>(&part[t][l15][4 * q]);
        const f32x4 v = sum + bias4;
        if (p.Y) *reinterpret_cast<f32x4*>(p.Y + (size_t)mg * p.Cout + n) = v;
        if (p.Yi) *reinterpret_cast<int4*>(p.Yi + (size_t)mg * p.Cout + n) = make_int4(hm_round(v[0], p.mean), hm_round(v[1], p.mean), hm_round(v[2], p.mean), hm_round(v[3], p.mean));
    }
#ifdef PNN_F32_DIAG
    const unsigned long long dr2 = __builtin_amdgcn_s_memrealtime();
#endif
    if (a.done.per_wg) { if (z == 0) signal_done_by_wave(a.done, blockIdx.y * gridDim.x + blockIdx.x); }
    else signal_done(a.done);
#ifdef PNN_F32_DIAG
    if (p.Xlo && tid == 0) {
        unsigned long long* d = (unsigned long long*)p.Xlo + 8 * (blockIdx.y * gridDim.x + blockIdx.x);
        d[1] = dr1 - dr0; d[3] = dr0; d[4] = de0; d[5] = __builtin_amdgcn_s_memrealtime(); d[6] = dr2;
    }
#endif
}

bool fc_out_f32_small_fits(const TapGemmParams& p) { return p.ncls == 1 && p.SH * p.SW == 1 && p.Cout <= 64 && p.Cout % 4 == 0 && (p.Cin + 159) / 160 <= 8 && p.M > 0; }

hipError_t launch_fc_out_f32_small(const TapGemmParams& p, hipStream_t s, const DoneSignal& done)
{
    if (!fc_out_f32_small_fits(p)) return hipErrorInvalidValue;
    const FcOutF32Args a{p, done};
    pnn_launch(fc_out_f32_chain_kernel, dim3((unsigned)((p.M + 15) / 16), (unsigned)((p.Cout + 15) / 16)), dim3(512), 0, s, a);
    return hipGetLastError();
}

__global__ __launch_bounds__(256) void seg_reduce_kernel(const float* __restrict__ part, int nseg, size_t n4, size_t stride4, int cq, const float* __restrict__ bias,
                                                         int act, float* __restrict__ Y)
{
    const size_t i = (size_t)blockIdx.x * 256 + threadIdx.x;
    if (i >= n4) return;
    const f32x4* __restrict__ src = reinterpret_cast<const f32x4*>(part) + i;
    f32x4 acc = src[0];
    for (int sgm = 1; sgm < nseg; sgm++) acc += src[(size_t)sgm * stride4];
    f32x4 v = acc + reinterpret_cast<const f32x4*>(bias)[i % (size_t)cq];
    if (act) { v[0] = leaky(v[0]); v[1] = leaky(v[1]); v[2] = leaky(v[2]); v[3] = leaky(v[3]); }
    reinterpret_cast<f32x4*>(Y)[i] = v;
}

hipError_t launch_seg_reduce(const float* part, int nseg, size_t n, int Cout, const float* bias, int act, float* Y, hipStream_t s)
{
    if (n == 0) return hipSuccess;
    if (nseg < 1 || n % 4 || Cout % 4) return hipErrorInvalidValue;
    const size_t n4 = n / 4;
    hipLaunchKernelGGL(seg_reduce_kernel, dim3((unsigned)((n4 + 255) / 256)), dim3(256), 0, s, part, nseg, n4, n4, Cout / 4, bias, act, Y);
    return hipGetLastError();
}

#define PNN_F32_CFGS(X) \
    X(1, 5, 4) X(1, 5, 2) X(1, 4, 4) X(1, 4, 2) X(1, 3, 4) X(1, 2, 4) X(1, 2, 2) X(1, 1, 4) X(1, 1, 2) \
    X(2, 4, 2) X(2, 2, 4) X(2, 2, 2) X(2, 1, 4) X(2, 3, 2)

static const TileCfg kCfgsF32[] = {
#define X(rt, nt, kc) {rt, nt, kc, 32},
    PNN_F32_CFGS(X)
#undef X
};

static const int kRegsF32[] = {360, 360, 296, 296, 224, 176, 152, 116, 92, 492, 288, 252, 208, 360};
static_assert(sizeof(kRegsF32) / sizeof(kRegsF32[0]) == sizeof(kCfgsF32) / sizeof(kCfgsF32[0]), "one register count per tile");
int tapgemm_f32_regs(int idx) { return kRegsF32[idx]; }

int tapgemm_f32_num_cfgs() { return (int)(sizeof(kCfgsF32) / sizeof(kCfgsF32[0])); }
TileCfg tapgemm_f32_cfg(int idx) { return kCfgsF32[idx]; }
size_t tapgemm_f32_lds_bytes(const TileCfg& t, bool fuse, bool row_out)
{
    const size_t ring = (size_t)3 * t.kc * 4 * 32 * t.nt, out_tile = (size_t)128 * t.rt * (8 * t.nt + 1);
    return (std::max(ring, (row_out && !fuse) ? out_tile : (size_t)0) + (fuse ? (size_t)8 * t.nt * 64 : 0)) * 16;
}
bool tapgemm_f32_can_fuse(int idx) { return kCfgsF32[idx].rt == 1 && kCfgsF32[idx].nt == 5; }

template <int RT, int NT, int KC>
static hipError_t launch_f32(const TapGemmParams& p0, bool fuse, hipStream_t s)
{
    const bool seq = p0.nseg > 1 && p0.seg_seq;
    if (fuse && p0.nseg > 1 && !seq) return hipErrorInvalidValue;
    dim3 grid((p0.M + 128 * RT - 1) / (128 * RT), (p0.Cout + 32 * NT - 1) / (32 * NT), p0.ncls * (!seq && p0.nseg > 1 ? p0.nseg : 1));
    const TileCfg t{RT, NT, KC, 32};
    TapGemmParams p = p0;
    p.pm_groups = 0;
    g_last_issued_frac = 1.0;
    const long nblk = p0.M / (p0.SH * p0.SW), bm = 128 * RT;
    if (!fuse && p0.pm_groups >= 0 && p0.SH * p0.SW > 1 && (p0.pm_groups == 1 || (nblk + bm - 1) / bm * bm * 100 <= nblk * 115)) {
        TapGemmParams q = p0;
        q.W2p = nullptr;
        static const double l2_mb = getenv("PNN_F32_PM_L2_MB") ? atof(getenv("PNN_F32_PM_L2_MB")) : 7.0;
        const PmPlan& plan = position_major_plan(q, 128 * RT, 32 * NT, KC, tapgemm_f32_lds_bytes(t, false, false), l2_mb);
        g_last_issued_frac = plan.use ? plan.live_frac : 1.0;
        if (plan.use) {
            p.pm_groups = plan.groups;
            p.nblk = p0.M / (p0.SH * p0.SW);
            for (int i = 0; i < 16; i++) p.pos_order[i] = plan.order[i];
            grid.x = (unsigned)(plan.groups * p0.SH * p0.SW);
            static const bool debug = getenv("PNN_DEBUG") != nullptr;
            if (debug) fprintf(stderr, "[pnn] f32 %dx%d: position-major tiles, %d block groups x %d positions\n", 128 * RT, 32 * NT, plan.groups, p0.SH * p0.SW);
        }
    }
    p.grid_x = (int)grid.x; p.grid_y = (int)grid.y; p.grid_z = (int)grid.z;
    const long ntiles = (long)grid.x * grid.y * grid.z;
    if (ntiles > 0x7fffffffL) return hipErrorInvalidValue;
    const DeviceInfo& di = device_info();
    int idx_self = 0;
    for (int i = 0; i < tapgemm_f32_num_cfgs(); i++) if (kCfgsF32[i].rt == RT && kCfgsF32[i].nt == NT && kCfgsF32[i].kc == KC) idx_self = i;
    const int by_regs = std::max(1, 512 / kRegsF32[idx_self]);
    int W = p0.persist >= 0 ? p0.persist : (ntiles > 2L * di.cus && ntiles <= 6L * di.cus ? 2 : 0);
    W = std::min(W, by_regs);
    size_t lds = tapgemm_f32_lds_bytes(t, fuse, p0.SH * p0.SW == 1);
    dim3 g1((unsigned)ntiles);
    if (W > 0 && ntiles > (long)di.cus * W && lds * (size_t)W <= di.lds) {
        g1.x = (unsigned)di.cus * (unsigned)W;
        lds = std::max(lds, (size_t)(di.lds / (W + 1) + 1024) / 16 * 16);
    }
    auto set_attr = [&](const void* fn, int (&done)[16]) -> hipError_t {
        const int dev = di.dev >= 0 && di.dev < 16 ? di.dev : 0;
        if (done[dev]) return hipSuccess;
        const hipError_t e = hipFuncSetAttribute(fn, hipFuncAttributeMaxDynamicSharedMemorySize, (int)di.lds);
        if (e == hipSuccess) done[dev] = 1;
        return e;
    };
    const bool one_tap = p0.ncls == 1 && p0.tap_begin[1] - p0.tap_begin[0] == 1;
    if (seq && (one_tap ? (p0.seg_chunks == 0 || p0.seg_chunks % (2 * KC) || (long)(p0.nseg - 1) * p0.seg_chunks >= p0.Cin / 16) : ((p0.Cin / 16) % KC) != 0)) return hipErrorInvalidValue;
    if constexpr (RT == 1 && NT == 5) {
        if (fuse && seq) {
            if (!one_tap) return hipErrorInvalidValue;
            static int done[16] = {};
            const hipError_t e = set_attr((const void*)tapgemm_f32_kernel<RT, NT, KC, true, 2>, done);
            if (e != hipSuccess) return e;
            pnn_launch(tapgemm_f32_kernel<RT, NT, KC, true, 2>, g1, dim3(256), lds, s, p);
            return hipGetLastError();
        }
        if (fuse) {
            static int done[16] = {};
            const hipError_t e = set_attr((const void*)tapgemm_f32_kernel<RT, NT, KC, true>, done);
            if (e != hipSuccess) return e;
            pnn_launch(tapgemm_f32_kernel<RT, NT, KC, true>, g1, dim3(256), lds, s, p);
            return hipGetLastError();
        }
    }
    if (fuse) return hipErrorInvalidValue;
    if (seq && one_tap) {
        static int done[16] = {};
        const hipError_t e = set_attr((const void*)tapgemm_f32_kernel<RT, NT, KC, false, 2>, done);
        if (e != hipSuccess) return e;
        pnn_launch(tapgemm_f32_kernel<RT, NT, KC, false, 2>, g1, dim3(256), lds, s, p);
        return hipGetLastError();
    }
    if (seq && ((p0.Cin / 16) / KC) % 2 == 0) {
        static int done[16] = {};
        const hipError_t e = set_attr((const void*)tapgemm_f32_kernel<RT, NT, KC, false, 2>, done);
        if (e != hipSuccess) return e;
        pnn_launch(tapgemm_f32_kernel<RT, NT, KC, false, 2>, g1, dim3(256), lds, s, p);
        return hipGetLastError();
    }
    if (seq) {
        static int done[16] = {};
        const hipError_t e = set_attr((const void*)tapgemm_f32_kernel<RT, NT, KC, false, 1>, done);
        if (e != hipSuccess) return e;
        pnn_launch(tapgemm_f32_kernel<RT, NT, KC, false, 1>, g1, dim3(256), lds, s, p);
        return hipGetLastError();
    }
    static int done[16] = {};
    const hipError_t e = set_attr((const void*)tapgemm_f32_kernel<RT, NT, KC, false>, done);
    if (e != hipSuccess) return e;
    pnn_launch(tapgemm_f32_kernel<RT, NT, KC, false>, g1, dim3(256), lds, s, p);
    return hipGetLastError();
}

hipError_t launch_tapgemm_f32(const TapGemmParams& p, int idx, bool fuse, hipStream_t s)
{
    if (p.M <= 0) return hipSuccess;
    int i = 0;
#define X(rt, nt, kc) if (idx == i++) return launch_f32<rt, nt, kc>(p, fuse, s);
    PNN_F32_CFGS(X)
#undef X
    return hipErrorInvalidValue;
}

}
```

### context_adaptive_neural_network_based_prediction_amd/csrc/pnn_kernels.h

```cpp
#pragma once
#include <hip/hip_runtime.h>
#include <hip/hip_ext.h>
#include <stdint.h>

#include "pnn_cabac_tables.h"
#include "pnn_mode_signal.h"
#include "pnn_rdoq.h"
#include "pnn_trquant_tables.h"

namespace pnn {

struct DoneSignal { unsigned* counter; unsigned* host_flag; unsigned seq, per_wg; };

struct LaunchEvents { hipEvent_t start, stop; };
extern thread_local const LaunchEvents* g_launch_events;
template <typename K, typename... A>
inline void pnn_launch(K kernel, dim3 grid, dim3 block, size_t lds, hipStream_t s, A... args)
{
    if (g_launch_events) hipExtLaunchKernelGGL(kernel, grid, block, (unsigned)lds, s, g_launch_events->start, g_launch_events->stop, 0, args...);
    else hipLaunchKernelGGL(kernel, grid, block, lds, s, args...);
}

struct DeviceInfo { int cus = 256; size_t lds = (size_t)160 << 10; int dev = -1; };
const DeviceInfo& device_info();

hipError_t probe_queue_shared(hipStream_t a, hipStream_t b, bool* shared);

constexpr int kMaxTaps = 32;
constexpr int kMaxClasses = 4;

struct TbDev;
struct TapGemmParams {
    const float* X;
    const void* Xlo;
    const void* zero;
    union {
        struct { const float* W2p; int Npad2; int K2chunks; float* part; };
        struct { const float* W1; float* Y1; int32_t* Yi1; };
        struct { unsigned* seg_cnt; float* seg_Y; };
    };
    union {
        struct {
            const float* X0; const float* W0; const float* B0; int s0, k0, pad0;
            const float* W0sp; float scale0; int Npad0;
            const void* plane0; const void* tbs0; int pel0, branch0, unit0, w0;
        };
        unsigned pos_order[16];
    };
    const float* Wp;
    const float* bias;
    float* Y;
    int32_t* Yi;
    void* Yhi;
    void* Ylo;
    int* range_flag;
    float out_scale;
    unsigned x_bytes;
    int M, SH, SW;
    int IH, IW, Cin, a;
    int OH, OW, Cout, os;
    int Npad;
    int act;
    float mean;
    int ncls;
    int tap_begin[kMaxClasses + 1];
    int chunk_begin[kMaxClasses + 1];
    int py[kMaxClasses], px[kMaxClasses];
    int tap[kMaxTaps];
    int pm_groups; union { int nblk; int chain_io; };
    float bias1; int k1, s1, pad1;
    int nseg; union { unsigned seg_stride; unsigned seg_chunks; };
    int seg_seq;
    int grid_x, grid_y, grid_z;
    int persist;
};
static_assert(sizeof(TapGemmParams) <= 512, "the argument block of the tap-GEMM kernels: 8 lines of 64 bytes");
inline int pack_tap(int dy, int dx) { return (int)(((unsigned)dy << 16) | ((unsigned)dx & 0xffffu)); }

constexpr int kChunkPad = 4;
constexpr int kSegDepth = 1600, kSegMinDepth = 2304;
constexpr int kFcSegChunks = 20;
struct TileCfg { int rt, nt, kc, mf, wm = 4, d = 2; };
int tapgemm_sp_num_cfgs();
TileCfg tapgemm_sp_cfg(int idx);
hipError_t launch_tapgemm_sp(const TapGemmParams& p, int idx, hipStream_t s);
int tapgemm_ring_num_cfgs();
TileCfg tapgemm_ring_cfg(int idx);
size_t tapgemm_ring_lds_bytes(const TileCfg& t);
bool tapgemm_ring_can_fuse(int idx);
hipError_t launch_seg_reduce(const float* part, int nseg, size_t n, int Cout, const float* bias, int act, float* Y, hipStream_t s);
hipError_t launch_fuse_reduce(const float* part, int ntiles, int M, int N2, const float* bias, float scale, float mean, float* Y, int32_t* Yi,
                              hipStream_t s, const DoneSignal& done = DoneSignal{nullptr, nullptr, 0, 0});
hipError_t launch_tapgemm_ring(const TapGemmParams& p, int idx, hipStream_t s);
struct PmPlan { bool use = false; int groups = 0; unsigned order[16] = {}; double live_frac = 1.0; };
extern thread_local double g_last_issued_frac;
const PmPlan& position_major_plan(const TapGemmParams& p, int BM, int BN, int KC, size_t lds, double l2_mb = 4.5);
int convimg_sp_num_cfgs();
TileCfg convimg_sp_cfg(int idx);
size_t convimg_sp_lds_bytes(const TapGemmParams& p, const TileCfg& t, int G);
bool convimg_sp_can_fuse_first(const TapGemmParams& p, const TileCfg& t, int G, int s0, int k0);
struct TConv1Params;
bool convimg_sp_can_fuse_last(const TapGemmParams& p, const TileCfg& t, int G, const TConv1Params& last);
hipError_t launch_convimg_sp(const TapGemmParams& p, int idx, int G, hipStream_t s);
hipError_t launch_split(const float* x, long n, void* hi, void* lo, int* range_flag, hipStream_t s);
long tapgemm_small_tiles(const TapGemmParams& p);
hipError_t launch_tapgemm_small(const TapGemmParams& p, bool a_is_f32, int seg_chunks, hipStream_t s, const float* host_input = nullptr);
hipError_t launch_tapgemm_small_pair(const TapGemmParams& a, const TapGemmParams& b, hipStream_t s);
int tapgemm_f32_num_cfgs();
TileCfg tapgemm_f32_cfg(int idx);
size_t tapgemm_f32_lds_bytes(const TileCfg& t, bool fuse, bool row_out = false);
bool tapgemm_f32_can_fuse(int idx);
int tapgemm_f32_regs(int idx);
hipError_t launch_tapgemm_f32(const TapGemmParams& p, int idx, bool fuse, hipStream_t s);
long tapgemm_f32_small_tiles(const TapGemmParams& p);
hipError_t launch_tapgemm_f32_small(const TapGemmParams& p, hipStream_t s, const float* host_input = nullptr, int deep_mode = 1);
hipError_t launch_tapgemm_f32_small_pair(const TapGemmParams& a, const TapGemmParams& b, hipStream_t s, int deep_mode = 1);
long fcseg_f32_small_tiles(const TapGemmParams& p);
bool fcseg_f32_small_fits(const TapGemmParams& p);
hipError_t launch_fcseg_f32_small(const TapGemmParams& p, hipStream_t s);
hipError_t launch_fc_out_f32(const TapGemmParams& p, hipStream_t s, int* segments);
bool fc_out_f32_small_fits(const TapGemmParams& p);
hipError_t launch_fc_out_f32_small(const TapGemmParams& p, hipStream_t s, const DoneSignal& done = DoneSignal{nullptr, nullptr, 0, 0});

struct Conv1Params {
    const float* X; const float* W; const float* bias; float* Y;
    int B, IH, IW, s, k, pad, OH, OW, Cout;
    int split;
    int band_rows;
    int* range_flag;
    const float* Wsp; float out_scale; int npad;
    const void* plane; const TbDev* tbs; int pel_bytes, unit, w, branch; float mean;
    int chain;
    int mfma;
};
hipError_t launch_conv_cin1(const Conv1Params& p, hipStream_t s);
hipError_t launch_conv_cin1_pair(const Conv1Params& a, const Conv1Params& b, hipStream_t s);

struct TConv1Params {
    const float* X; const float* W;  float bias; float* Y; int32_t* Yi;
    int B, IH, IW, Cin, s, k, pad; float mean;
    int ni;
    DoneSignal done;
};
hipError_t launch_tconv_cout1(const TConv1Params& p, hipStream_t s);

struct MergerParams {
    const float* A; const float* L; const float* Wp; const float* bias ; float* Y;
    int B, C, na, nl, nout;
    int split;
    int* range_flag;
    int chain;
};
hipError_t launch_merger(const MergerParams& p, hipStream_t s);

struct SmallTail { int kind; unsigned* cnt; MergerParams m; TConv1Params t; };
bool f32_small_cout1_tail_ok(const TapGemmParams& p, const TConv1Params& t);
bool f32_small_merger_tail_ok(const TapGemmParams& a, const TapGemmParams& b, const MergerParams& m);
hipError_t launch_tapgemm_f32_small_tail(const TapGemmParams& p, const SmallTail& t, hipStream_t s, int deep_mode = 1);
hipError_t launch_tapgemm_f32_small_pair_tail(const TapGemmParams& a, const TapGemmParams& b, const SmallTail& t, hipStream_t s, int deep_mode = 1);

struct TbDev {
    int64_t origin;
    int32_t stride;
    uint32_t above_mask;
    int32_t left_units;
    int32_t reserved;
};
struct GatherParams {
    const void* plane; int pel_bytes; const TbDev* tbs; int N; int w; int unit; float mean;
    float* above; float* left; long pitch_above; long pitch_left;
    int split;
};
hipError_t launch_gather(const GatherParams& p, hipStream_t s);

struct BlockCostParams {
    const void* org_plane; int pel_bytes; const TbDev* tbs; int N; int w; const int32_t* pred; int hadamard; uint32_t* cost;
};
hipError_t launch_block_cost(const BlockCostParams& p, hipStream_t s);

struct PictureBlocks {
    const uint8_t* channels; int H, W; const int32_t* rows; const int32_t* cols; int positions;
};

struct HevcBestModeParams {
    const uint8_t* patterns; int ph; int pw; const uint8_t* targets; int N; int w;
    uint8_t* best_mode; uint32_t* best_sse; uint8_t* best_pred; uint32_t* mode_sse;
    PictureBlocks pic;
    const uint8_t* pic_targets;
    int smoothing;
};
hipError_t launch_hevc_best_mode(const HevcBestModeParams& p, hipStream_t s);

struct HevcModeHadsParams {
    const uint8_t* patterns; int ph; int pw; const uint8_t* targets; int N; int w;
    const uint8_t* cand_pred; uint32_t* mode_hads; uint32_t* cand_hads; uint8_t* list_modes; uint32_t* list_costs;
    PictureBlocks pic;
    const uint8_t* pic_targets;
    int smoothing;
};
inline int hevc_first_pass_list_size(int w) { return w <= 8 ? 8 : 3; }
hipError_t launch_hevc_mode_hads(const HevcModeHadsParams& p, hipStream_t s);

struct RdCandidatesParams {
    const uint8_t* patterns; int ph; int pw; const uint8_t* targets; int N; int w;
    const uint8_t* cand_pred; const uint8_t* list_modes; uint8_t* cand_modes; uint8_t* slot_pred; uint8_t* slot_targets;
    PictureBlocks pic;
    const uint8_t* pic_targets;
    int smoothing;
};
constexpr int kRdUnusedSlot = 255;
int rd_candidates_blocks_per_workgroup(int w);
hipError_t launch_rd_candidates(const RdCandidatesParams& p, hipStream_t s);
struct RdDecideParams {
    const uint32_t* sse; const uint64_t* rate; const uint8_t* cand_modes; int N; int w; int nb_qps; double lambda[trquant::kMaxQps];
    double* cand_costs; uint8_t* best_mode; uint8_t* best_slot; double* best_cost; uint32_t* best_sse; uint64_t* best_rate;
};
hipError_t launch_rd_decide(const RdDecideParams& p, hipStream_t s);

struct SignalListParams {
    const uint32_t* mode_hads; const uint32_t* cand_hads; const uint8_t* left; const uint8_t* above; int N; int w; int nb_qps;
    msig::FlagBits bits[trquant::kMaxQps]; double sqrt_lambda[trquant::kMaxQps];
    double* list_costs; uint8_t* slot_modes;
};
hipError_t launch_signal_list(const SignalListParams& p, hipStream_t s);
hipError_t launch_rd_candidates_slots(const RdCandidatesParams& p, hipStream_t s);
struct RdDecideSignalParams {
    const uint32_t* sse; const uint64_t* rate; const uint32_t* nonzero; const uint8_t* slot_modes; const uint8_t* left; const uint8_t* above;
    int N; int w; int cbf_ctx; double lambda; msig::FlagBits bits;
    double* cand_costs; uint8_t* best_mode; uint8_t* best_slot; double* best_cost; uint32_t* best_sse; uint64_t* best_rate;
    uint64_t* best_side_rate;
};
hipError_t launch_rd_decide_signal(const RdDecideSignalParams& p, hipStream_t s);

struct TrQuantParams {
    const uint8_t* pred; const uint8_t* targets; int N; int w; int nb_qps; trquant::QpConsts qp[trquant::kMaxQps];
    uint32_t* sse; uint32_t* nonzero; uint32_t* sum_abs; uint8_t* recon;
    uint64_t* rate; const uint8_t* modes; uint8_t init_states[trquant::kMaxQps][cabac::kNumCtx];
    int sdh;
    int rdoq; int cbf_ctx; rdoq::Consts rd[trquant::kMaxQps]; uint8_t cbf_states[trquant::kMaxQps][2];
};
int trquant_blocks_per_workgroup(int w);
hipError_t launch_trquant(const TrQuantParams& p, hipStream_t s);

struct IpfcnsGatherParams {
    const uint8_t* channels; int H, W; const int32_t* rows; const int32_t* cols; int positions; long b0; int nb; int w;
    float* x; float* mean;
};
hipError_t launch_ipfcns_gather(const IpfcnsGatherParams& p, hipStream_t s);
hipError_t launch_ipfcns_prelu(float* y, const float* slope, long total, int H, hipStream_t s);
struct IpfcnsEpilogueParams {
    const float* fc4; const float* mean; int nb; int w2; uint8_t* u8; float* f32; const uint8_t* targets; uint32_t* sse;
};
hipError_t launch_ipfcns_epilogue(const IpfcnsEpilogueParams& p, hipStream_t s);

struct ScoreDescParams { PictureBlocks pic; long b0; int nb; int w; int mask_w, mask_h; TbDev* tbs; };
hipError_t launch_score_desc(const ScoreDescParams& p, hipStream_t s);
struct ScoreEpilogueParams {
    PictureBlocks pic; long b0; int nb; int w; const float* pred; float mean; uint8_t* u8; uint8_t* targets; uint32_t* sse;
};
hipError_t launch_score_epilogue(const ScoreEpilogueParams& p, hipStream_t s);

hipError_t launch_epilogue(const float* pred, long n, float mean, int32_t* dst, hipStream_t s);

}
```

### context_adaptive_neural_network_based_prediction_amd/csrc/pnn_passes.cpp

```cpp
#include "pnn_ctx.h"

#include <algorithm>
#include <cmath>
#include <cstdio>
#include <cstdlib>
#include <cstring>
#include <thread>
#include <vector>

namespace pnn {

namespace {

void count_gemm(pnn_ctx* c, double flops)
{
    c->stat_gemm_launches++; c->stat_launches++;
    c->stat_gemm_flops += flops;
}

template <typename Launch, typename... Args>
int timed_launch(pnn_ctx* c, int kind, double flops, bool profile, Launch&& launch, const char* fmt = nullptr, Args... args)
{
    if (profile || c->opt_time_launches) {
        pnn_ctx::LaunchRec r;
// ... 6 lines not shown
        g_launch_events = nullptr;
        HIPCHK(c, le);
        if (profile) {
            HIPCHK(c, hipEventSynchronize(r.e1));
            float ms = 0.f;
            HIPCHK(c, hipEventElapsedTime(&ms, r.e0, r.e1));
            fprintf(stderr, fmt, args..., ms * 1e3, flops / (ms * 1e-3) / 1e12);
            (void)hipEventDestroy(r.e0);
            (void)hipEventDestroy(r.e1);
        } else {
            c->launch_recs.push_back(r);
        }
    } else {
        HIPCHK(c, launch());
    }
    count_gemm(c, flops);
    return PNN_OK;
}

int bind_layer(pnn_ctx* c, const GemmLayer& L, long nblocks, const char* noun, TapGemmParams* p)
{
    *p = L.proto;
    const long M = nblocks * p->SH * p->SW;
    if (M > 0x7fffffffL) return fail(c, PNN_E_ARG, "batch too large for one pass");
    p->M = (int)M;
    const double xb = 4.0 * (double)nblocks * p->IH * p->IW * p->Cin;
    if (xb >= 2147483648.0) return fail(c, PNN_E_ARG, "activation %s of %.0f bytes exceeds the 2 GiB descriptor bound", noun, xb);
    p->x_bytes = (unsigned)xb;
    return PNN_OK;
}

bool fc_segmented(const GemmLayer& L) { return L.fc_seg_chunks > 0 && L.nseg > 1; }

bool f32_small_applies(pnn_ctx* c, const GemmLayer& L, long nb, bool has_next, bool has_yi)
{
    if (has_next || !c->opt_f32_small || c->opt_f32_cfg >= 0 || env_f32_diag()) return false;
    TapGemmParams p;
    if (bind_layer(c, L, nb, "tensor", &p)) return false;
    if (fc_segmented(L)) {
        p.nseg = L.nseg; p.seg_chunks = (unsigned)L.fc_seg_chunks;
        return fcseg_f32_small_fits(p) && fcseg_f32_small_tiles(p) <= c->opt_f32_small_tiles;
    }
    p.nseg = (!has_yi && L.nseg > 1) ? L.nseg : 1;
    return tapgemm_f32_small_tiles(p) <= c->opt_f32_small_tiles;
}

bool launch_folds_segments(const pnn_ctx* c, const TapGemmParams& p)
{
    return p.nseg > 1 && c->opt_seg_fold && c->d_seg_cnt && !c->opt_time_launches && tapgemm_f32_small_tiles(p) / p.nseg <= pnn_ctx::kSegCntTiles;
}

bool f32_small_chain_out_ok(pnn_ctx* c, const GemmLayer& L, long nb)
{
    if (!c->opt_chain_io || L.proto.Cout % 16) return false;
    if (L.nseg <= 1 || L.fc_seg_chunks > 0) return true;
    TapGemmParams p;
    if (bind_layer(c, L, nb, "tensor", &p)) return false;
    p.nseg = L.nseg;
    return launch_folds_segments(c, p);
}

int stream_slot(const pnn_ctx* c, hipStream_t s) { return (c->side_stream && s == c->side_stream) ? 1 : 0; }

int seg_planes(pnn_ctx* c, TapGemmParams& p, int nseg, size_t out_floats, DevBuf& sb)
{
    int rc;
    if ((rc = dev_reserve(c, sb, (size_t)nseg * out_floats * 4))) return rc;
    if (out_floats >= 0xffffffffull) return fail(c, PNN_E_ARG, "batch too large for one pass");
    p.Y = (float*)sb.p; p.bias = (const float*)c->d_zero; p.act = 0; p.nseg = nseg; p.seg_stride = (unsigned)out_floats;
    return PNN_OK;
}

int seg_planes_folded(pnn_ctx* c, TapGemmParams& p, const GemmLayer& L, float* Y, DevBuf& sb, int slot)
{
    int rc;
    if ((rc = dev_reserve(c, sb, (size_t)tapgemm_f32_small_tiles(p) * 1024))) return rc;
    p.Y = (float*)sb.p;
    p.seg_cnt = c->d_seg_cnt + slot * pnn_ctx::kSegCntTiles;
    p.seg_Y = Y; p.bias = L.d_bias; p.act = L.proto.act;
    return PNN_OK;
}

int clear_tail_counters(pnn_ctx* c, hipStream_t s, bool sync_for_side)
{
    if (!c->seg_cnt_dirty) return PNN_OK;
    HIPCHK(c, hipMemsetAsync(c->d_seg_cnt, 0, pnn_ctx::kCntWords * 4, s));
    if (sync_for_side && c->side_stream && s != c->side_stream) HIPCHK(c, hipStreamSynchronize(s));
    c->seg_cnt_dirty = false;
    return PNN_OK;
}

int gemm_fcseg_small(pnn_ctx* c, const GemmLayer& L, const TapGemmParams& p, double flops, int chain_io, hipStream_t s)
{
    const long M = p.M;
    TapGemmParams ps = p;
    ps.Wp = L.d_w_ch;
    ps.chain_io = chain_io;
    if (env_debug()) fprintf(stderr, "[pnn] gemm M=%ld K=%.0f N=%d nseg=%d -> f32 small kernel, %d K segments side by side (%ld tiles of 16 x 16)\n", M, L.k_total, p.Cout, L.nseg, L.nseg, fcseg_f32_small_tiles(p));
    if (void* slot = diag_stamp_slot(c, "fcseg_f32_small", fcseg_f32_small_tiles(p), L.k_total)) ps.Xlo = slot;
    return timed_launch(c, 6, flops, env_profile(), [&] { return launch_fcseg_f32_small(ps, s); },
                        "[pnn-prof] M=%ld K=%.0f N=%d nseg=%d f32-small-fcseg us=%.1f tflops=%.2f\n", M, L.k_total, p.Cout, L.nseg);
}

int gemm_small(pnn_ctx* c, const GemmLayer& L, const TapGemmParams& p, float* Y, int nseg, long nblocks, double flops, hipStream_t s,
               const float* host_rows, int chain_io, const SmallTail* tail, bool* tail_ran)
{
    const long M = p.M;
    const bool debug = env_debug(), profile = env_profile();
    TapGemmParams ps = p;
    ps.Wp = L.d_w_ch;
    ps.chain_io = chain_io;
    if ((chain_io & 1) && host_rows) host_rows = nullptr;
    const bool fold = nseg > 1 && launch_folds_segments(c, p);
    if (fold) {
        int rc;
        if ((rc = clear_tail_counters(c, s, true))) return rc;
        if ((rc = seg_planes_folded(c, ps, L, Y, c->seg_part[stream_slot(c, s)], stream_slot(c, s)))) return rc;
    }
    if (debug) fprintf(stderr, "[pnn] gemm M=%ld K=%.0f N=%d ncls=%d nseg=%d -> f32 small kernel (%ld tiles of 16 x 16)\n", M, L.k_total, p.Cout, p.ncls, nseg, tapgemm_f32_small_tiles(p));
    if (void* slot = diag_stamp_slot(c, "tapgemm_f32_small", tapgemm_f32_small_tiles(p), L.k_total)) ps.Xlo = slot;
    const bool with_tail = !profile && !c->opt_time_launches && tail && tail_ran && nseg == 1 && !(chain_io & 2) && f32_small_cout1_tail_ok(ps, tail->t);
    if (with_tail && debug) fprintf(stderr, "[pnn]   ... with the last transposed convolution as its tail\n");
    const int rc = timed_launch(c, 6, flops, profile, [&] {
        return with_tail ? launch_tapgemm_f32_small_tail(ps, *tail, s, (int)c->opt_f32_small_deep)
                         : launch_tapgemm_f32_small(ps, s, host_rows, (int)c->opt_f32_small_deep);
    }, "[pnn-prof] M=%ld K=%.0f N=%d ncls=%d f32-small us=%.1f tflops=%.2f\n", M, L.k_total, p.Cout, p.ncls);
    if (rc) return rc;
    if (with_tail) *tail_ran = true;
    if (nseg > 1 && !fold) {
        if (chain_io & 2) return fail(c, PNN_E_ARG, "internal: chain-order output of a layer whose K segments are reduced by a second launch");
        HIPCHK(c, launch_seg_reduce(p.Y, nseg, (size_t)nblocks * (size_t)L.out_per_block, p.Cout, L.d_bias, L.proto.act, Y, s));
        c->stat_launches++;
    }
    return env_f32s_diag() ? diag_f32_small(c, L, ps, nseg, host_rows, s) : PNN_OK;
}

int gemm_tiles(pnn_ctx* c, const GemmLayer& L, TapGemmParams& p, const TapGemmParams& pseq, float* Y, int nseg, long nblocks, double flops,
               hipStream_t s, const GemmLayer* next, float* part, int* tiles_out)
{
    const long M = p.M;
    const bool debug = env_debug(), fcseg = fc_segmented(L);
    const bool one_tap = (L.k_total == (double)p.Cin);
    const int cpt = p.Cin / 16;
    const size_t out_floats = (size_t)nblocks * (size_t)L.out_per_block;
    const int ntile = tapgemm_f32_num_cfgs();
    if (next) { p.W2p = next->d_w; p.Npad2 = next->proto.Npad; p.K2chunks = next->proto.chunk_begin[1]; p.part = part; }
    const long seg_mode = c->opt_f32_seg_mode;
    auto legal = [&](int code) {
        if (code >= ntile && (nseg == 1 || seg_mode == 0)) return false;
        if (code < ntile && nseg > 1 && seg_mode == 1) return false;
        const TileCfg t = tapgemm_f32_cfg(code % ntile);
        if (fcseg && L.fc_seg_chunks % (2 * t.kc)) return false;
        if (fcseg && t.rt * t.nt >= 8) return false;
        return (one_tap || cpt % t.kc == 0) && (!next || tapgemm_f32_can_fuse(code % ntile));
    };
    float* const Yreal = Y;
    const float* const bias_real = L.d_bias;
    const int act_real = L.proto.act;
    std::function<hipError_t(int)> launch = [&, p, pseq, Yreal, bias_real, act_real, fcseg](int code) {
        if (code >= ntile) return launch_tapgemm_f32(pseq, code - ntile, false, s);
        const hipError_t e = launch_tapgemm_f32(p, code, next != nullptr, s);
        if (e != hipSuccess || p.nseg <= 1 || fcseg) return e;
        return launch_seg_reduce(p.Y, p.nseg, out_floats, p.Cout, bias_real, act_real, Yreal, s);
    };
    double cost_par = 0, cost_seq = 0;
    int cfg = choose_cfg_f32(c, M, p.Cout, p.ncls * nseg, p.Cin, L.k_total, next != nullptr, &cost_par);
    if (cfg < 0) return fail(c, PNN_E_ARG, "no tapgemm_f32 tile fits a layer with %d-deep taps", p.Cin);
    if (fcseg && !legal(cfg)) {
        const TileCfg want = tapgemm_f32_cfg(cfg);
        int alt = -1;
        for (int i = 0; i < ntile; i++) if (legal(i) && (alt < 0 || (tapgemm_f32_cfg(i).rt == want.rt && tapgemm_f32_cfg(i).nt == want.nt))) alt = i;
        if (alt < 0) return fail(c, PNN_E_ARG, "no tapgemm_f32 tile fits K segments of %d chunks", L.fc_seg_chunks);
        cfg = alt;
    }
    if (nseg > 1) {
        cost_par += (double)(nseg + 1) * (double)out_floats * 4.0 / 4.0e12 * 2.4e9 + 9000.0;
        const int cs = choose_cfg_f32(c, M, p.Cout, p.ncls, p.Cin, L.k_total, false, &cost_seq);
        if (seg_mode == 1 || (seg_mode < 0 && cs >= 0 && cost_seq < cost_par)) cfg = ntile + cs;
    }
    bool tune = c->opt_f32_cfg < 0 && (c->opt_autotune == 1 || (c->opt_autotune == 2 && flops >= 4.0e9));
    if (tune) {
        hipStreamCaptureStatus cap = hipStreamCaptureStatusNone;
        if (hipStreamIsCapturing(s, &cap) == hipSuccess && cap != hipStreamCaptureStatusNone) tune = false;
    }
    if (tune) {
        const void* key = (const void*)((const char*)&L + 8 + (next ? 1 : 0));
        float best_us = -1.f;
        const int rule = cfg;
        const int trc = tuned_cfg(c, key, M, nseg > 1 ? 2 * ntile : ntile, rule, legal, launch, s, &cfg, &best_us);
        if (trc) return trc;
        if (best_us >= 0.f && debug) {
            const TileCfg tb = tapgemm_f32_cfg(cfg % ntile), th = tapgemm_f32_cfg(rule % ntile);
            fprintf(stderr, "[pnn] f32 autotune M=%ld K=%.0f N=%d ncls=%d nseg=%d: best {%d,%d,%d}%s %.1f us (rule {%d,%d,%d}%s)\n", M, L.k_total, p.Cout, p.ncls, nseg,
                    tb.rt, tb.nt, tb.kc, cfg >= ntile ? " seq" : "", best_us, th.rt, th.nt, th.kc, rule >= ntile ? " seq" : "");
        }
    }
    const bool seq = nseg > 1 && cfg >= ntile;
    const TileCfg t = tapgemm_f32_cfg(cfg % ntile);
    if (tiles_out) *tiles_out = (int)((p.Cout + 32L * t.nt - 1) / (32L * t.nt));
    if (debug) fprintf(stderr, "[pnn] gemm M=%ld K=%.0f N=%d ncls=%d -> f32 cfg %d {rt %d, nt %d, kc %d}%s%s\n", M, L.k_total, p.Cout, p.ncls,
                       cfg, t.rt, t.nt, t.kc, next ? " + fused output layer" : "",
                       nseg > 1 ? (seq ? ", K segments in sequence" : ", K segments in parallel + reduce") : "");
    const int trc = timed_launch(c, 0, flops, env_profile(), [&] { return launch(cfg); },
                                 "[pnn-prof] M=%ld K=%.0f N=%d ncls=%d f32 cfg=%d rt=%d nt=%d kc=%d mf=%d us=%.1f tflops=%.1f\n", M, L.k_total,
                                 p.Cout, p.ncls, cfg, t.rt, t.nt, t.kc, t.mf);
    if (trc) return trc;
    if (nseg > 1 && !seq) c->stat_launches++;
    c->stat_gemm_flops_skipped += flops * (1.0 - g_last_issued_frac);
    return env_f32_diag() ? diag_f32_tiles(c, L, seq ? pseq : p, cfg % ntile, next != nullptr, seq ? 1 : nseg, s) : PNN_OK;
}

int run_gemm(pnn_ctx* c, const GemmLayer& L, const float* X, float* Y, int32_t* Yi, long nblocks, hipStream_t s,
             const GemmLayer* next = nullptr, float* part = nullptr, int* tiles_out = nullptr, const float* host_rows = nullptr, int chain_io = 0,
             const SmallTail* tail = nullptr, bool* tail_ran = nullptr)
{
    TapGemmParams p;
    int rc;
    if ((rc = bind_layer(c, L, nblocks, "tensor", &p))) return rc;
    p.X = X; p.Wp = L.d_w; p.bias = L.d_bias; p.Y = Y; p.Yi = Yi; p.mean = c->mean;
    const double flops = 2.0 * (double)p.M * L.k_total * p.Cout + (next ? 2.0 * (double)p.M * next->k_total * next->proto.Cout : 0.0);
    const bool one_tap = (L.k_total == (double)p.Cin);
    p.pm_groups = c->opt_ring_pm == 0 ? -1 : c->opt_ring_pm == 2 ? 1 : 0;
    const bool fcseg = fc_segmented(L);
    const int nseg = (!fcseg && !next && !Yi && L.nseg > 1) ? L.nseg : 1;
    if (!fcseg && L.nseg > 1 && nseg == 1) return fail(c, PNN_E_ARG, "a K-segmented layer cannot carry the HM epilogue or a fused output layer");
    if (fcseg) { p.nseg = L.nseg; p.seg_chunks = (unsigned)L.fc_seg_chunks; p.seg_seq = 1; }
    p.persist = (next || one_tap) ? 0 : (int)c->opt_f32_persist;
    TapGemmParams pseq = p;
    if (nseg > 1) {
        pseq.nseg = nseg; pseq.seg_seq = 1;
        if ((rc = seg_planes(c, p, nseg, (size_t)nblocks * (size_t)L.out_per_block, c->seg_part[stream_slot(c, s)]))) return rc;
        p.seg_seq = 0;
    }
    const bool small_f32 = f32_small_applies(c, L, nblocks, next != nullptr, Yi != nullptr);
    if (chain_io && !small_f32) return fail(c, PNN_E_ARG, "internal: chain-order activations for a layer that does not run on the small kernels");
    if (small_f32 && fcseg) return gemm_fcseg_small(c, L, p, flops, chain_io, s);
    if (small_f32) return gemm_small(c, L, p, Y, nseg, nblocks, flops, s, host_rows, chain_io, tail, tail_ran);
    return gemm_tiles(c, L, p, pseq, Y, nseg, nblocks, flops, s, next, part, tiles_out);
}

int run_gemm_sp(pnn_ctx* c, const GemmLayer& L, const void* Xhi, const void* Xlo, float* Y, void* Yhi, void* Ylo, int32_t* Yi,
                long nblocks, hipStream_t s, const GemmLayer* next = nullptr, float* part = nullptr, int* tiles_out = nullptr,
                const Conv1Params* first = nullptr, bool x_is_f32 = false, int seg_chunks = 0, bool* query_fuse_first = nullptr,
                const TConv1Params* lastp = nullptr)
{
    if (query_fuse_first) *query_fuse_first = false;
    TapGemmParams p;
    int brc;
    if ((brc = bind_layer(c, L, nblocks, "plane", &p))) return brc;
    const long M = p.M;
    if (next) {
        p.W2p = next->d_w_sp; p.Npad2 = next->proto.Npad; p.K2chunks = next->proto.chunk_begin[1]; p.part = part;
    }
    p.X = (const float*)Xhi; p.Xlo = Xlo; p.Wp = L.d_w_sp;
    const bool diag = env_sp_diag();
    if (diag) {
        if (dev_reserve(c, c->stage_tbs, (size_t)64 << 20)) return PNN_E_NOMEM;
        p.Xlo = c->stage_tbs.p;
    }
    p.bias = L.d_bias; p.Y = Y; p.Yhi = Yhi; p.Ylo = Ylo; p.Yi = Yi;
    p.mean = c->mean; p.out_scale = L.sp_inv_scale; p.range_flag = c->h_range;
    p.pm_groups = c->opt_ring_pm == 0 ? -1 : c->opt_ring_pm == 2 ? 1 : 0;
    const int cpt = p.Cin / 16;
    const bool one_tap = (L.k_total == (double)p.Cin);
    const bool debug = env_debug();
    const bool small = seg_chunks > 0 || (!next && !diag && c->opt_small && c->opt_sp_cfg < 0 && tapgemm_small_tiles(p) <= c->opt_small_tiles);
    if (small && query_fuse_first) return PNN_OK;
    if (small) {
        if (seg_chunks > 0) p.part = part;
        if (first) { HIPCHK(c, launch_conv_cin1(*first, s)); c->stat_launches++; }
        if (debug) fprintf(stderr, "[pnn] sp-gemm M=%ld K=%.0f N=%d ncls=%d -> small kernel (%ld tiles%s%s)\n", M, L.k_total, p.Cout, p.ncls,
                           tapgemm_small_tiles(p), x_is_f32 ? ", f32 input" : "", seg_chunks ? ", K segments" : "");
        const int trc = timed_launch(c, 5, 2.0 * (double)M * L.k_total * p.Cout, false,
                                     [&] { return launch_tapgemm_small(p, x_is_f32, seg_chunks, s, x_is_f32 ? c->host_input : nullptr); });
        if (trc) return trc;
        if (tiles_out) *tiles_out = seg_chunks > 0 ? (int)(((long)(L.k_total / 16.0) + seg_chunks - 1) / seg_chunks) : 0;
        if (lastp) { HIPCHK(c, launch_tconv_cout1(*lastp, s)); c->stat_launches++; }
        return PNN_OK;
    }
    if (x_is_f32 && !query_fuse_first) {
        const long nin = nblocks * (long)p.IH * p.IW * p.Cin;
        HIPCHK(c, launch_split((const float*)Xhi, nin, c->ws[2].p, nullptr, c->h_range, s));
        c->stat_launches++;
        p.X = (const float*)c->ws[2].p;
    }
    const int nsp = tapgemm_sp_num_cfgs(), nci = convimg_sp_num_cfgs(), nrg = tapgemm_ring_num_cfgs();
    p.zero = c->d_zero;
    auto cfg_of = [&](int code) { return code < nsp ? tapgemm_sp_cfg(code) : code < nsp + nci ? convimg_sp_cfg(code - nsp) : tapgemm_ring_cfg(code - nsp - nci); };
    auto kind_of = [&](int code) { return code < nsp ? "" : code < nsp + nci ? "img" : "ring"; };
    auto legal = [&](int code) {
        if (next) return code >= nsp + nci && !diag && c->opt_ring && tapgemm_ring_can_fuse(code - nsp - nci) &&
                         32 * tapgemm_ring_cfg(code - nsp - nci).nt * (4 / tapgemm_ring_cfg(code - nsp - nci).wm) == 16 * kFuseSegChunks;
        if (code < nsp) return one_tap || cpt % tapgemm_sp_cfg(code).kc == 0;
        if (code < nsp + nci) return !diag && c->opt_convimg && convimg_images(p, convimg_sp_cfg(code - nsp), one_tap) > 0;
        return !diag && c->opt_ring && (one_tap || cpt % tapgemm_ring_cfg(code - nsp - nci).kc == 0);
    };
    bool fused_last = false;
    auto launch = [&](int code) {
        fused_last = false;
        if (first) {
            if (code >= nsp && code < nsp + nci) {
                const TileCfg t = convimg_sp_cfg(code - nsp);
                const int g = convimg_images(p, t, one_tap);
                if (c->opt_fuse_first && convimg_sp_can_fuse_first(p, t, g, first->s, first->k)) {
                    TapGemmParams q = p;
                    q.X0 = first->X; q.W0 = first->W; q.B0 = first->bias; q.s0 = first->s; q.k0 = first->k; q.pad0 = first->pad;
                    q.W0sp = first->Wsp; q.scale0 = first->out_scale; q.Npad0 = first->npad;
                    if (first->plane) {
                        q.plane0 = first->plane; q.tbs0 = first->tbs; q.pel0 = first->pel_bytes; q.unit0 = first->unit;
                        q.branch0 = first->branch; q.w0 = first->w;
                    }
                    return launch_convimg_sp(q, code - nsp, g, s);
                }
            }
            if (!first->X) return hipErrorInvalidValue;
            const hipError_t e = launch_conv_cin1(*first, s);
            if (e != hipSuccess) return e;
        }
        hipError_t e;
        if (code < nsp) e = launch_tapgemm_sp(p, code, s);
        else if (code < nsp + nci) {
            const TileCfg t = convimg_sp_cfg(code - nsp);
            const int g = convimg_images(p, t, one_tap);
            if (lastp && c->opt_fuse_tail && !lastp->done.host_flag && convimg_sp_can_fuse_last(p, t, g, *lastp)) {
                TapGemmParams q = p;
                q.Y = nullptr;
                q.W1 = lastp->W; q.Y1 = lastp->Y; q.Yi1 = lastp->Yi; q.bias1 = lastp->bias; q.k1 = lastp->k; q.s1 = lastp->s; q.pad1 = lastp->pad;
                fused_last = true;
                return launch_convimg_sp(q, code - nsp, g, s);
            }
            e = launch_convimg_sp(p, code - nsp, g, s);
        } else e = launch_tapgemm_ring(p, code - nsp - nci, s);
        if (e != hipSuccess || !lastp) return e;
        return launch_tconv_cout1(*lastp, s);
    };
    int cfg = choose_cfg_sp(c, M, p.Cout, p.ncls, p.Cin, L.k_total);
    if (c->opt_sp_cfg >= nsp && legal((int)c->opt_sp_cfg)) cfg = (int)c->opt_sp_cfg;
    else if (c->opt_sp_cfg < 0) {
        const int ci = c->opt_convimg ? choose_cfg_convimg(p, one_tap) : -1;
        const int ri = c->opt_ring ? choose_cfg_ring(p, M, one_tap, L.k_total, next != nullptr) : -1;
        const bool ring_conv = !one_tap && ri >= 0 && ((p.Cout % 128 == 0 && L.k_total / p.ncls >= 1152.0) || (p.ncls == 4 && p.Cout == 64 && M >= 8192) || pnn_ring_few_images(p, M, L.k_total));
        if (ring_conv && legal(nsp + nci + ri)) cfg = nsp + nci + ri;
        else if (ci >= 0 && legal(nsp + ci) && !one_tap) cfg = nsp + ci;
        else if (ri >= 0 && legal(nsp + nci + ri)) cfg = nsp + nci + ri;
        else if (ci >= 0 && legal(nsp + ci)) cfg = nsp + ci;
    }
    bool tune = c->opt_autotune == 1 || (c->opt_autotune == 2 && 2.0 * (double)M * L.k_total * p.Cout >= 4.0e9);
    const void* const key = (const void*)((const char*)&L + (next ? 1 : 0) + (first ? 2 : 0) + (lastp ? 4 : 0));
    if (tune && c->tuned.find(std::make_pair(key, M)) == c->tuned.end()) {
        hipStreamCaptureStatus cap = hipStreamCaptureStatusNone;
        if (hipStreamIsCapturing(s, &cap) == hipSuccess && cap != hipStreamCaptureStatusNone) tune = false;
    }
    if (query_fuse_first) {
        int code = cfg;
        if (tune && c->opt_sp_cfg < 0) {
            auto it = c->tuned.find(std::make_pair(key, M));
            if (it == c->tuned.end()) return PNN_OK;
            code = it->second;
        }
        if (first && code >= nsp && code < nsp + nci && legal(code)) {
// ... 509 lines not shown
```

### context_adaptive_neural_network_based_prediction_amd/csrc/pnn_tiles.cpp

```cpp
#include "pnn_ctx.h"

#include <algorithm>
#include <cmath>
#include <cstdio>
#include <cstdlib>
#include <cstring>
#include <thread>
#include <vector>

namespace pnn {

int choose_cfg_f32(const pnn_ctx* c, long M, int cout, int ncls, int cin, double k_total, bool fused, double* cost_out)
{
    const int cpt = cin / 16;
    const bool one_tap = (k_total == (double)cin);
    if (c->opt_f32_cfg >= 0 && c->opt_f32_cfg < tapgemm_f32_num_cfgs()) {
        const TileCfg t = tapgemm_f32_cfg((int)c->opt_f32_cfg);
        if ((one_tap || cpt % t.kc == 0) && (!fused || tapgemm_f32_can_fuse((int)c->opt_f32_cfg))) { if (cost_out) *cost_out = 0.0; return (int)c->opt_f32_cfg; }
    }
    int best = -1;
    double best_cost = 1e300;
    const DeviceInfo& di = device_info();
    const double ncu = (double)di.cus, lds_cu = (double)di.lds;
    for (int i = 0; i < tapgemm_f32_num_cfgs(); i++) {
        const TileCfg t = tapgemm_f32_cfg(i);
        if (fused && !tapgemm_f32_can_fuse(i)) continue;
        if (!one_tap && cpt % t.kc) continue;
        const long bm = 128L * t.rt, bn = 32L * t.nt;
        const double wgs = (double)((M + bm - 1) / bm) * (double)((cout + bn - 1) / bn) * ncls;
        const double regs = tapgemm_f32_regs(i);
        const int res = (int)std::max(1.0, std::min(std::min(4.0, std::floor(512.0 / regs)), std::floor(lds_cu / (double)tapgemm_f32_lds_bytes(t, fused))));
        const double chunks = std::ceil(k_total / 16.0 / ncls / t.kc) * t.kc;
        const double mfma = chunks * 8.0 * t.rt * t.nt * 64.0;
        const double fixed = 5000.0 + 2500.0 * t.rt * t.nt;
        const bool exact = std::fmod(wgs, ncu) == 0.0 && wgs / ncu <= res;
        const double per_cu = wgs / ncu, rounds = per_cu / res;
        const double fixed_eff = rounds >= 2.0 ? 0.4 * fixed : fixed * std::max(1.0, std::min((double)res, per_cu));
        double cost = wgs * mfma / ncu + (exact ? 0.0 : 0.6 * mfma) + fixed_eff;
        if (wgs < ncu) cost = mfma + fixed;
        if (t.rt == 2) cost *= 1.2;
        cost *= 1.0 + 0.01 / (t.rt * t.nt) + (t.kc == 2 ? 0.005 : 0.0);
        if (cost < best_cost) { best_cost = cost; best = i; }
    }
    if (cost_out) *cost_out = best_cost;
    return best;
}

int convimg_images(const TapGemmParams& p, const TileCfg& t, bool one_tap)
{
    if (one_tap || (p.Cin / 16) % t.kc) return 0;
    const int rows = 32 * t.rt * t.wm, sp = p.SH * p.SW;
    int g = rows / sp;
    while (g > 0 && convimg_sp_lds_bytes(p, t, g) > (size_t)156 * 1024) --g;
    return g;
}

int choose_cfg_convimg(const TapGemmParams& p, bool one_tap)
{
    int best = -1;
    double best_cost = 1e300, best_fit = 1e300;
    const long nimg = p.M / (p.SH * p.SW);
    for (int i = 0; i < convimg_sp_num_cfgs(); i++) {
        const TileCfg t = convimg_sp_cfg(i);
        const int g = convimg_images(p, t, one_tap);
        if (g <= 0) continue;
        const long rows = 32L * t.rt * t.wm, bn = 32L * t.nt * (4 / t.wm);
        const long tn = (p.Cout + bn - 1) / bn;
        const double pad = (double)rows * (tn * bn) / ((double)g * p.SH * p.SW * p.Cout);
        double height = rows <= 64 ? 1.15 : rows <= 128 ? 1.0 : rows <= 192 ? 1.05 : rows <= 256 ? 1.25 : rows <= 384 ? 1.6 : 2.0;
        if (p.Cout <= 32) height = 1.0 + 0.3 * std::fabs(std::log2((double)rows / (8.0 * p.SH * p.SW)));
        const double wgs = (double)((nimg + g - 1) / g) * tn * p.ncls;
        const double fill = wgs >= 512.0 ? 1.0 : 512.0 / wgs;
        const double cost = pad * height * fill;
        if (cost < best_cost) { best_cost = cost; best_fit = p.Cout <= 32 ? pad : pad * height; best = i; }
    }
    return best_fit <= (p.Cout <= 32 ? 3.0 : 1.6) ? best : -1;
}

bool pnn_ring_few_images(const TapGemmParams& p, long M, double k_total)
{
    return (p.ncls == 1 || p.ncls == 4) && p.Cout == 64 && k_total / p.ncls >= 512.0 && M / ((long)p.SH * p.SW) < 128 && (M + 63) / 64 * p.ncls >= 128;
}

int choose_cfg_ring(const TapGemmParams& p, long M, bool one_tap, double k_total, bool fused)
{
    if (!fused && !one_tap) {
        const bool wide = p.Cout % 128 == 0 && k_total / p.ncls >= 1152.0;
        const double col_tiles = (double)((p.Cout + 127) / 128) * p.ncls;
        const bool underfilled = k_total >= 1600.0 && (double)((M + 63) / 64) * col_tiles <= 256.0;
        if (p.ncls == 4 && p.Cout == 64 && M >= 8192) {
            for (int d = 3; d <= 4; d++)
                for (int i = 0; i < tapgemm_ring_num_cfgs(); i++) {
                    const TileCfg t = tapgemm_ring_cfg(i);
                    if (t.rt == 1 && t.nt == 2 && t.kc == 2 && t.wm == 4 && t.d == d) return i;
                }
        }
        const bool few_images = pnn_ring_few_images(p, M, k_total);
        if (!wide && !underfilled && !few_images) return -1;
        int rt = 1, wm = 2, d = 4;
        if (wide) {
            if ((double)((M + 191) / 192) * col_tiles >= 192.0) { rt = 3; d = 4; }
            else if ((double)((M + 127) / 128) * col_tiles >= 192.0) rt = 2;
        }
        for (int i = 0; i < tapgemm_ring_num_cfgs(); i++) {
            const TileCfg t = tapgemm_ring_cfg(i);
            if (t.rt == rt && t.nt == 2 && t.kc == 2 && t.wm == wm && t.d == d) return i;
        }
        return -1;
    }
    if (!fused && ((double)M * p.Cout < 5.0e5 || p.Cin < 64)) return -1;
    int best = -1;
    double best_cost = 1e300;
    for (int i = 0; i < tapgemm_ring_num_cfgs(); i++) {
        const TileCfg t = tapgemm_ring_cfg(i);
        if (fused && !tapgemm_ring_can_fuse(i)) continue;
        if (!one_tap && (p.Cin / 16) % t.kc) continue;
        const long bm = 32L * t.rt * t.wm, bn = 32L * t.nt * (4 / t.wm);
        const long nwg = ((M + bm - 1) / bm) * ((p.Cout + bn - 1) / bn) * p.ncls;
        const int resident = tapgemm_ring_lds_bytes(t) > (size_t)80 * 1024 ? 1 : 2;
        const double stages = std::ceil((k_total / 16.0 / p.ncls) / (double)t.kc);
        const double mfma = 96.0 * t.rt * t.nt * t.kc;
        const double slow = t.kc == 1 ? 1.35 : (resident == 2 ? 1.25 : (t.d >= 4 ? 1.17 : 1.6));
        const double wg = 5000.0 + 1400.0 * t.rt * t.nt + stages * mfma * slow;
        const double rounds = std::ceil(nwg / (256.0 * resident));
        double cost = rounds * wg * (resident == 2 ? 1.6 : 1.0);
        cost *= 1.0 + 0.05 * (1.0 - nwg / (256.0 * resident * rounds));
        if (cost < best_cost) { best_cost = cost; best = i; }
    }
    return best;
}

int choose_cfg_sp(const pnn_ctx* c, long M, int cout, int ncls, int cin, double k_total)
{
    const int cpt = cin / 16;
    const bool one_tap = (k_total == (double)cin);
    if (c->opt_sp_cfg >= 0 && c->opt_sp_cfg < tapgemm_sp_num_cfgs()) {
        const TileCfg t = tapgemm_sp_cfg((int)c->opt_sp_cfg);
        if (one_tap || cpt % t.kc == 0) return (int)c->opt_sp_cfg;
    }
    int best = -1;
    double best_cost = 1e300;
    for (int i = 0; i < tapgemm_sp_num_cfgs(); i++) {
        const TileCfg t = tapgemm_sp_cfg(i);
        if (!one_tap && cpt % t.kc) continue;
        const long bm = 32L * t.rt * t.wm, bn = 32L * t.nt * (4 / t.wm);
        const long tm = (M + bm - 1) / bm, tn = (cout + bn - 1) / bn;
        const double wgs = (double)tm * tn * ncls;
        const double per_cu = wgs / 256.0;
        const double fill = per_cu < 1.0 ? 1.2 * std::pow(1.0 / per_cu, 0.7) : 1.0 + 0.4 * std::max(0.0, 1.5 - per_cu);
        const double pad = (double)(tm * bm) * (tn * bn) / ((double)M * cout);
        const double reuse = 1.0 + 2.0 / (t.nt * (4 / t.wm));
        const double shape = (t.rt * t.wm >= 8 ? 1.15 : 1.0) * (t.kc == 4 ? 1.4 : (t.kc == 1 ? 1.08 : 1.0));
        const double cost = fill * pad * reuse * shape;
        if (cost < best_cost) { best_cost = cost; best = i; }
    }
    return best < 0 ? 0 : best;
}

}
```

### include/pnn_hip.h

```cpp
#ifndef PNN_HIP_H
#define PNN_HIP_H

#include <stddef.h>
#include <stdint.h>

#ifdef __cplusplus
extern "C" {
#endif

#define PNN_OK 0
#define PNN_E_ARG (-1)
#define PNN_E_IO (-2)
#define PNN_E_MODEL (-3)
#define PNN_E_HIP (-4)
#define PNN_E_NOMEM (-5)
#define PNN_E_RANGE (-6)

typedef struct pnn_ctx pnn_ctx;


int pnn_create_empty(pnn_ctx** out, float mean, int device);

int pnn_create(pnn_ctx** out, const char* model_table_path, int use_pair, float mean, int device);

int pnn_load_model_file(pnn_ctx* ctx, const char* path);
int pnn_load_model_params(pnn_ctx* ctx, int width, int is_fc, const float* params, size_t n_params);

int pnn_model_info(const pnn_ctx* ctx, int width, int* is_fc, int* n_layers, long* n_params);
void pnn_destroy(pnn_ctx* ctx);
const char* pnn_last_error(const pnn_ctx* ctx);
float pnn_mean(const pnn_ctx* ctx);

int pnn_set_option(pnn_ctx* ctx, const char* name, long value);
int pnn_check_range(pnn_ctx* ctx, void* stream, long* host_fallbacks);

int pnn_arithmetic_tag(const pnn_ctx* ctx, char* out, size_t bytes);

int pnn_num_split_configs(void);
int pnn_num_f32_configs(void);
int pnn_cache_stats(pnn_ctx* ctx, long* hits, long* misses);


int pnn_predict_fc(pnn_ctx* ctx, int width, const float* context, int n, float* out);
int pnn_predict_conv(pnn_ctx* ctx, int width, const float* above, const float* left, int n, float* out);
int pnn_predict_pel(pnn_ctx* ctx, int width, const float* above, const float* left, int n, int32_t* dst,
                    int dst_stride);

int pnn_host_alloc(void** out, size_t bytes);
void pnn_host_free(void* p);

int pnn_streams_on_distinct_queues(void** out_streams, int want);
void pnn_streams_release(void** streams, int n);

int pnn_predict_f32_pel(pnn_ctx* ctx, int width, const float* above, const float* left, int n, float* out, int32_t* dst);

int pnn_extract_context(const int32_t* roi_origin, float* above, float* left, const uint8_t* neighbor_flags,
                        int n_avail, int unit_w, int unit_h, int above_units, int left_units, int tu_w,
                        int tu_h, int pic_stride, float mean);

int pnn_parse_model_table(const char* path, int* widths, int* is_pair, int* channels, const char** paths,
                          int max_entries);


int pnn_predict_fc_device(pnn_ctx* ctx, int width, const float* d_context, int n, float* d_out, void* stream);
int pnn_predict_conv_device(pnn_ctx* ctx, int width, const float* d_above, const float* d_left, int n,
                            float* d_out, void* stream);

typedef struct {
    int64_t origin;
    int32_t stride;
    uint32_t above_mask;
    int32_t left_units;
    int32_t reserved;
} pnn_tb_dev;

int pnn_make_tb_desc(pnn_tb_dev* out, int64_t origin, int32_t stride, const uint8_t* neighbor_flags,
                     int n_avail, int above_units, int left_units);

int pnn_gather_device(pnn_ctx* ctx, int width, int unit, const void* d_plane, int pel_bytes,
                      const pnn_tb_dev* d_tbs, int n, float* d_above, long pitch_above, float* d_left,
                      long pitch_left, void* stream);

int pnn_predict_tbs_device(pnn_ctx* ctx, int width, const void* d_plane, int pel_bytes, const pnn_tb_dev* d_tbs,
                           int n, int32_t* d_dst, float* d_out_f32, void* stream);

int pnn_block_cost_device(pnn_ctx* ctx, int width, const void* d_org_plane, int pel_bytes, const pnn_tb_dev* d_tbs, int n,
                          const int32_t* d_pred, int hadamard, uint32_t* d_cost, void* stream);
int pnn_predict_tbs_cost_device(pnn_ctx* ctx, int width, const void* d_plane, const void* d_org_plane, int pel_bytes,
                                const pnn_tb_dev* d_tbs, int n, int hadamard, uint32_t* d_cost, int32_t* d_dst, void* stream);


int pnn_hevc_intra_predict(const uint8_t* intra_pattern, int pattern_h, int pattern_w, int width, int mode, uint8_t* out);

int pnn_hevc_mode_uses_smoothing(int width, int mode);
int pnn_hevc_smoothed_reference_host(const uint8_t* pattern, int pattern_h, int pattern_w, int width, int smoothing, uint8_t* line,
                                     int* strong_used);
int pnn_hevc_intra_predict_hm(const uint8_t* intra_pattern, int pattern_h, int pattern_w, int width, int mode, int smoothing,
                              uint8_t* out);

int pnn_hevc_best_mode_device(pnn_ctx* ctx, int width, const uint8_t* d_patterns, int pattern_h, int pattern_w,
                              const uint8_t* d_targets, int n, uint8_t* d_best_mode, uint32_t* d_best_sse,
                              uint8_t* d_best_pred, uint32_t* d_mode_sse, void* stream);
int pnn_hevc_best_mode_hm_device(pnn_ctx* ctx, int width, const uint8_t* d_patterns, int pattern_h, int pattern_w,
                                 const uint8_t* d_targets, int n, int smoothing, uint8_t* d_best_mode, uint32_t* d_best_sse,
                                 uint8_t* d_best_pred, uint32_t* d_mode_sse, void* stream);


int pnn_ipfcns_forward_host(int width, const float* params, const float* x, int n, int layers, float* out);
int pnn_ipfcns_load(pnn_ctx* ctx, int width, const float* params, size_t n_floats);
int pnn_ipfcns_forward_device(pnn_ctx* ctx, int width, const float* d_x, int n, float* d_out_f32, void* stream);
int pnn_ipfcns_predict_device(pnn_ctx* ctx, int width, const uint8_t* d_channels, int images, int height, int width_ch,
                              const int32_t* d_rows, const int32_t* d_cols, int positions, const uint8_t* d_targets,
                              uint8_t* d_pred_u8, float* d_pred_f32, float* d_means, uint32_t* d_sse, void* stream);


int pnn_score_pictures_device(pnn_ctx* ctx, int width, const uint8_t* d_channels, int images, int height, int width_ch,
                              const int32_t* d_rows, const int32_t* d_cols, int positions, int mask_w, int mask_h,
                              uint8_t* d_targets, uint8_t* d_pnn_u8, float* d_pnn_f32, uint32_t* d_pnn_sse,
                              uint8_t* d_hevc_mode, uint32_t* d_hevc_sse, uint8_t* d_hevc_pred, void* stream);
int pnn_score_picture_pairs_device(pnn_ctx* ctx, int width, const uint8_t* d_context_channels, const uint8_t* d_target_channels,
                                   int images, int height, int width_ch, const int32_t* d_rows, const int32_t* d_cols, int positions,
                                   int mask_w, int mask_h, uint8_t* d_targets, uint8_t* d_pnn_u8, float* d_pnn_f32, uint32_t* d_pnn_sse,
                                   uint8_t* d_hevc_mode, uint32_t* d_hevc_sse, uint8_t* d_hevc_pred, void* stream);
int pnn_score_picture_pairs_hm_device(pnn_ctx* ctx, int width, const uint8_t* d_context_channels, const uint8_t* d_target_channels,
                                      int images, int height, int width_ch, const int32_t* d_rows, const int32_t* d_cols, int positions,
                                      int mask_w, int mask_h, int smoothing, uint8_t* d_targets, uint8_t* d_pnn_u8, float* d_pnn_f32,
                                      uint32_t* d_pnn_sse, uint8_t* d_hevc_mode, uint32_t* d_hevc_sse, uint8_t* d_hevc_pred, void* stream);
int pnn_score_f32_device(pnn_ctx* ctx, int width, const float* d_pred_f32, const uint8_t* d_channels, int images, int height,
                         int width_ch, const int32_t* d_rows, const int32_t* d_cols, int positions,
                         uint8_t* d_pred_u8, uint32_t* d_sse, void* stream);


int pnn_first_pass_list_size(int width);
int pnn_hevc_mode_hads_host(const uint8_t* patterns, int pattern_h, int pattern_w, const uint8_t* targets, int width, int n,
                            const uint8_t* cand_pred, uint32_t* mode_hads, uint32_t* cand_hads, uint8_t* list_modes,
                            uint32_t* list_costs);
int pnn_hevc_mode_hads_hm_host(const uint8_t* patterns, int pattern_h, int pattern_w, const uint8_t* targets, int width, int n,
                               const uint8_t* cand_pred, int smoothing, uint32_t* mode_hads, uint32_t* cand_hads, uint8_t* list_modes,
                               uint32_t* list_costs);
int pnn_hevc_mode_hads_device(pnn_ctx* ctx, int width, const uint8_t* d_patterns, int pattern_h, int pattern_w,
                              const uint8_t* d_targets, int n, const uint8_t* d_cand_pred, uint32_t* d_mode_hads, uint32_t* d_cand_hads,
                              uint8_t* d_list_modes, uint32_t* d_list_costs, void* stream);
int pnn_hevc_mode_hads_hm_device(pnn_ctx* ctx, int width, const uint8_t* d_patterns, int pattern_h, int pattern_w,
                                 const uint8_t* d_targets, int n, const uint8_t* d_cand_pred, int smoothing, uint32_t* d_mode_hads,
                                 uint32_t* d_cand_hads, uint8_t* d_list_modes, uint32_t* d_list_costs, void* stream);
int pnn_first_pass_picture_pairs_device(pnn_ctx* ctx, int width, const uint8_t* d_context_channels, const uint8_t* d_target_channels,
                                        int images, int height, int width_ch, const int32_t* d_rows, const int32_t* d_cols,
                                        int positions, int mask_w, int mask_h, const uint8_t* d_cand_pred, uint32_t* d_mode_hads,
                                        uint32_t* d_cand_hads, uint8_t* d_list_modes, uint32_t* d_list_costs, void* stream);
int pnn_first_pass_picture_pairs_hm_device(pnn_ctx* ctx, int width, const uint8_t* d_context_channels, const uint8_t* d_target_channels,
                                           int images, int height, int width_ch, const int32_t* d_rows, const int32_t* d_cols,
                                           int positions, int mask_w, int mask_h, const uint8_t* d_cand_pred, int smoothing,
                                           uint32_t* d_mode_hads, uint32_t* d_cand_hads, uint8_t* d_list_modes, uint32_t* d_list_costs,
                                           void* stream);


int pnn_trquant_host(const uint8_t* predictions, const uint8_t* targets, int width, int n, const int* qps, int nb_qps,
                     uint32_t* sses_recon, uint32_t* nb_nonzero, uint32_t* sum_abs_levels, uint8_t* recon);
int pnn_trquant_stages_host(const uint8_t* prediction, const uint8_t* target, int width, int qp, int32_t* coeffs, int32_t* levels,
                            int32_t* dequant, int32_t* residual);
int pnn_trquant_device(pnn_ctx* ctx, int width, const uint8_t* d_predictions, const uint8_t* d_targets, int n, const int* qps, int nb_qps,
                       uint32_t* d_sses_recon, uint32_t* d_nb_nonzero, uint32_t* d_sum_abs_levels, uint8_t* d_recon, void* stream);


int pnn_trquant_rate_host(const uint8_t* predictions, const uint8_t* targets, int width, int n, const uint8_t* modes, const int* qps,
                          int nb_qps, uint32_t* sses_recon, uint32_t* nb_nonzero, uint32_t* sum_abs_levels, uint8_t* recon, uint64_t* rate);
int pnn_cabac_rate_levels_host(const int32_t* levels, int t, int scan, int qp, uint64_t* rate);
int pnn_trquant_rate_device(pnn_ctx* ctx, int width, const uint8_t* d_predictions, const uint8_t* d_targets, int n, const uint8_t* d_modes,
                            const int* qps, int nb_qps, uint32_t* d_sses_recon, uint32_t* d_nb_nonzero, uint32_t* d_sum_abs_levels,
                            uint8_t* d_recon, uint64_t* d_rate, void* stream);


int pnn_sign_hide_unit_host(int32_t* levels, const int32_t* coeffs, const int32_t* delta_u, int t, int scan);
int pnn_trquant_sdh_host(const uint8_t* predictions, const uint8_t* targets, int width, int n, const uint8_t* modes, const int* qps,
                         int nb_qps, uint32_t* sses_recon, uint32_t* nb_nonzero, uint32_t* sum_abs_levels, uint8_t* recon, uint64_t* rate,
                         int sign_data_hiding);
int pnn_trquant_stages_sdh_host(const uint8_t* prediction, const uint8_t* target, int width, int qp, int scan, int sign_data_hiding,
                                int32_t* coeffs, int32_t* levels, int32_t* delta_u, int32_t* levels_hidden, int32_t* dequant,
                                int32_t* residual);
int pnn_cabac_rate_levels_sdh_host(const int32_t* levels, int t, int scan, int qp, int sign_data_hiding, uint64_t* rate);
int pnn_trquant_sdh_device(pnn_ctx* ctx, int width, const uint8_t* d_predictions, const uint8_t* d_targets, int n, const uint8_t* d_modes,
                           const int* qps, int nb_qps, uint32_t* d_sses_recon, uint32_t* d_nb_nonzero, uint32_t* d_sum_abs_levels,
                           uint8_t* d_recon, uint64_t* d_rate, int sign_data_hiding, void* stream);


double pnn_hm_intra_lambda(int qp);
int pnn_rd_pass_host(const uint8_t* patterns, int pattern_h, int pattern_w, const uint8_t* targets, int width, int n,
                     const uint8_t* cand_pred, int smoothing, const int* qps, int nb_qps, const double* lambdas, int sign_data_hiding,
                     uint8_t* cand_modes, double* cand_costs, uint8_t* best_mode, uint8_t* best_slot, double* best_cost, uint32_t* best_sse,
                     uint64_t* best_rate);
size_t pnn_rd_pass_workspace_bytes(int width, int n, int nb_qps);
int pnn_rd_pass_device(pnn_ctx* ctx, int width, const uint8_t* d_patterns, int pattern_h, int pattern_w, const uint8_t* d_targets, int n,
// ... 79 lines not shown
```

Baseline: 17.56 million blocks/s.

## Add paired wide+narrow f32 GEMM tiles to split one-wave grids across two workgroups per CU

Adds a paired f32 tap-GEMM kernel that splits each 128x160 output tile into a 128x96 and a 128x64 workgroup. The launch order is arranged so both halves can co-reside on one CU, with two workgroups per CU via launch bounds. The tile chooser switches to this config when the default 1x5 tile would give exactly one workgroup per CU for a one-tap, unfused GEMM, aiming at better latency hiding and occupancy. It falls back to the old tile when occupancy is below two, and adds diagnostics and stats entry points.

```diff
diff --git a/context_adaptive_neural_network_based_prediction_amd/_lib.py b/context_adaptive_neural_network_based_prediction_amd/_lib.py
--- a/context_adaptive_neural_network_based_prediction_amd/_lib.py
+++ b/context_adaptive_neural_network_based_prediction_amd/_lib.py
@@ -42,6 +42,8 @@
     "pnn_set_option": (ci, [vp, ctypes.c_char_p, ctypes.c_long]),
     "pnn_num_split_configs": (ci, []),
     "pnn_num_f32_configs": (ci, []),
+    "pnn_f32_pair_stats": (ci, [vp, ctypes.POINTER(ctypes.c_long), ctypes.POINTER(ctypes.c_long)]),
+    "pnn_f32_pair_tile": (ci, [ci, ci, ci] + [ctypes.POINTER(ci)] * 4),
     "pnn_check_range": (ci, [vp, vp, ctypes.POINTER(ctypes.c_long)]),
     "pnn_last_call_issued_flops": (ci, [vp, ctypes.POINTER(ctypes.c_double)]),
     "pnn_arithmetic_tag": (ci, [vp, ctypes.c_char_p, ctypes.c_size_t]),
diff --git a/context_adaptive_neural_network_based_prediction_amd/csrc/pnn_abi.cpp b/context_adaptive_neural_network_based_prediction_amd/csrc/pnn_abi.cpp
--- a/context_adaptive_neural_network_based_prediction_amd/csrc/pnn_abi.cpp
+++ b/context_adaptive_neural_network_based_prediction_amd/csrc/pnn_abi.cpp
@@ -265,6 +265,7 @@
     {"chain_io",             &pnn_ctx::opt_chain_io,            "PNN_CHAIN_IO",         kStore,       nullptr},
     {"tails",                &pnn_ctx::opt_tails,               "PNN_TAILS",            kStore,       nullptr},
     {"f32_cfg",              &pnn_ctx::opt_f32_cfg,             "PNN_F32_CFG",          kStore,       nullptr},
+    {"f32_pair_occ",         &pnn_ctx::opt_f32_pair_occ,        nullptr,                kRetune,      nullptr},
     {"f32_seg_mode",         &pnn_ctx::opt_f32_seg_mode,        "PNN_F32_SEG_MODE",     kRetune,      nullptr},
     {"f32_persist",          &pnn_ctx::opt_f32_persist,         "PNN_F32_PERSIST",      kRetune,      nullptr},
     {"f32_overlap",          &pnn_ctx::opt_f32_overlap,         "PNN_F32_OVERLAP",      kStore,       nullptr},
@@ -493,6 +494,30 @@
     if (n_gemm) *n_gemm = c->stat_gemm_launches;
     if (flops) *flops = c->stat_gemm_flops;
     if (n_launches) *n_launches = c->stat_launches;
+    return PNN_OK;
+}
+
+int pnn_f32_pair_stats(const pnn_ctx* c, long* paired, long* fell_back)
+{
+    if (!c) return PNN_E_ARG;
+    if (paired) *paired = c->stat_pair_launches;
+    if (fell_back) *fell_back = c->stat_pair_fallbacks;
+    return PNN_OK;
+}
+
+int pnn_f32_pair_tile(int M, int cout, int wg, int* num_wgs, int* row0, int* col0, int* cols)
+{
+    if (M <= 0 || cout <= 0 || wg < 0) return PNN_E_ARG;
+    int gx = 0, groups = 0, nwg = 0;
+    f32_pair_grid(M, cout, &gx, &groups, &nwg);
+    if (num_wgs) *num_wgs = nwg;
+    if (wg >= nwg) return PNN_E_ARG;
+    const PairTile t = f32_pair_tile(wg, gx);
+    const int c0 = t.group * (kPairWide + kPairNarrow) + (t.narrow ? kPairWide : 0);
+    const bool live = t.group < groups && c0 < cout;
+    if (row0) *row0 = t.bx * 128;
+    if (col0) *col0 = c0;
+    if (cols) *cols = live ? (t.narrow ? kPairNarrow : kPairWide) : 0;
     return PNN_OK;
 }
 
diff --git a/context_adaptive_neural_network_based_prediction_amd/csrc/pnn_ctx.h b/context_adaptive_neural_network_based_prediction_amd/csrc/pnn_ctx.h
--- a/context_adaptive_neural_network_based_prediction_amd/csrc/pnn_ctx.h
+++ b/context_adaptive_neural_network_based_prediction_amd/csrc/pnn_ctx.h
@@ -143,6 +143,8 @@
     long opt_f32_small_tiles = 1024;
     long opt_f32_overlap = 1;
     long opt_f32_cfg = -1;
+    long opt_f32_pair_occ = 0;
+    long stat_pair_launches = 0, stat_pair_fallbacks = 0;
     long opt_fuse_first = 1;
     long opt_fuse_last = 1;
     long opt_f32_seg_mode = 0;
diff --git a/context_adaptive_neural_network_based_prediction_amd/csrc/pnn_diag.cpp b/context_adaptive_neural_network_based_prediction_amd/csrc/pnn_diag.cpp
--- a/context_adaptive_neural_network_based_prediction_amd/csrc/pnn_diag.cpp
+++ b/context_adaptive_neural_network_based_prediction_amd/csrc/pnn_diag.cpp
@@ -54,9 +54,39 @@
     HIPCHK(c, hipMemset(c->stage_tbs.p, 0, (size_t)16 << 20));
     for (int rep = 0; rep < 400; rep++) HIPCHK(c, launch_tapgemm_f32(q, tile, fused, s));
     HIPCHK(c, hipStreamSynchronize(s));
-    const size_t nwg = (size_t)((M + 128L * t.rt - 1) / (128L * t.rt)) * ((p.Cout + 32L * t.nt - 1) / (32L * t.nt)) * p.ncls * par_segs;
+    size_t nwg = (size_t)((M + 128L * t.rt - 1) / (128L * t.rt)) * ((p.Cout + 32L * t.nt - 1) / (32L * t.nt)) * p.ncls * par_segs;
+    if (t.pair && g_last_pair_mode == 1) { int gx, groups, n; f32_pair_grid(p.M, p.Cout, &gx, &groups, &n); nwg = (size_t)n; }
     std::vector<unsigned long long> hbuf(8 * nwg);
     HIPCHK(c, hipMemcpy(hbuf.data(), c->stage_tbs.p, hbuf.size() * 8, hipMemcpyDeviceToHost));
+    if (t.pair && g_last_pair_mode == 1) {
+        const int gx = (int)((M + 127) / 128);
+        double sum[2][4] = {}; size_t cnt[2] = {0, 0};
+        unsigned long long r0 = ~0ull, r1 = 0, end[2] = {0, 0};
+        std::map<unsigned long long, std::pair<int, int>> per_cu;
+        std::map<int, unsigned long long> cu_of[2];
+        for (size_t i = 0; i < nwg; i++) {
+            const unsigned long long* d = &hbuf[8 * i];
+            if (!d[3]) continue;
+            const PairTile pt = f32_pair_tile((int)i, gx);
+            const int k = pt.narrow;
+            for (int j = 0; j < 4; j++) sum[k][j] += (double)d[j];
+            cnt[k]++;
+            r0 = std::min(r0, d[4]); r1 = std::max(r1, d[4] + d[3]); end[k] = std::max(end[k], d[4] + d[3]);
+            const unsigned long long cu = ((d[5] >> 32) & 0xf) << 16 | (d[5] & 0xff00);
+            (k ? per_cu[cu].second : per_cu[cu].first)++;
+            cu_of[k][pt.group * gx + pt.bx] = cu;
+        }
+        size_t one_each = 0, together = 0;
+        for (const auto& kv : per_cu) one_each += kv.second.first == 1 && kv.second.second == 1;
+        for (const auto& kv : cu_of[1]) { const auto w = cu_of[0].find(kv.first); together += w != cu_of[0].end() && w->second == kv.second; }
+        for (int k = 0; k < 2; k++)
+            fprintf(stderr, "[pnn-f32diag] M=%ld K=%.0f N=%d pair kc %d %s: %zu WGs; wave 0 mean cycles: prologue %.0f  loop %.0f  epilogue %.0f; lifetime %.1f us; last end %.1f us after the first start\n",
+                    M, L.k_total, p.Cout, t.kc, k ? "narrow 128x64" : "wide 128x96", cnt[k], sum[k][0] / std::max<size_t>(cnt[k], 1), sum[k][1] / std::max<size_t>(cnt[k], 1),
+                    sum[k][2] / std::max<size_t>(cnt[k], 1), sum[k][3] / std::max<size_t>(cnt[k], 1) / 100.0, (double)(end[k] - r0) / 100.0);
+        fprintf(stderr, "[pnn-f32diag]   first start -> last end %.1f us; %zu CUs in use, %zu of them with one wide and one narrow workgroup; %zu of %zu pairs with both tiles on one CU\n",
+                (double)(r1 - r0) / 100.0, per_cu.size(), one_each, together, cu_of[1].size());
+        return PNN_OK;
+    }
     double sum[4] = {0, 0, 0, 0};
     unsigned long long r0 = ~0ull, r1 = 0;
     for (size_t i = 0; i < nwg; i++) {
diff --git a/context_adaptive_neural_network_based_prediction_amd/csrc/pnn_gemm_f32.hip b/context_adaptive_neural_network_based_prediction_amd/csrc/pnn_gemm_f32.hip
--- a/context_adaptive_neural_network_based_prediction_amd/csrc/pnn_gemm_f32.hip
+++ b/context_adaptive_neural_network_based_prediction_amd/csrc/pnn_gemm_f32.hip
@@ -25,7 +25,7 @@
 }
 
 template <int RT, int NT, int KC, bool FUSE, int SEQ>
-__device__ __forceinline__ void f32_tile(const TapGemmParams& p, f32x4* const lds, const int bx, const int by, const int bz, const int gx, const int gy)
+__device__ __forceinline__ void f32_tile(const TapGemmParams& p, f32x4* const lds, const int bx, const int by, const int bz, const int n0, const int lin)
 {
     static_assert(KC >= 2 && KC % 2 == 0, "fragment sets alternate by chunk parity");
     constexpr int BM = 128 * RT, BN = 32 * NT;
@@ -45,7 +45,6 @@
     const int nseg = (!FUSE && !SEQ && p.nseg > 1) ? p.nseg : 1;
     const int cls = nseg > 1 ? bz / nseg : bz;
     const int seg = bz - cls * nseg;
-    const int n0 = by * BN;
     const int m0 = bx * BM + wave * (32 * RT);
 #ifdef PNN_F32_DIAG
     const unsigned long long dq0 = __builtin_amdgcn_s_memtime(), dr0 = __builtin_amdgcn_s_memrealtime();
@@ -349,9 +348,10 @@
     dq2 = __builtin_amdgcn_s_memtime();
     auto diag_out = [&]() {
         if (tid == 0 && p.Xlo) {
-            unsigned long long* d = (unsigned long long*)p.Xlo + 8 * ((bz * gy + by) * gx + bx);
+            unsigned long long* d = (unsigned long long*)p.Xlo + 8 * lin;
             d[0] = dq1 - dq0; d[1] = dq2 - dq1; d[2] = __builtin_amdgcn_s_memtime() - dq2; d[3] = __builtin_amdgcn_s_memrealtime() - dr0;
             d[4] = dr0;
+            d[5] = ((unsigned long long)__builtin_amdgcn_s_getreg(20 | (31 << 11)) << 32) | (unsigned)__builtin_amdgcn_s_getreg(4 | (31 << 11));
         }
     };
 #else
@@ -467,8 +467,20 @@
     for (int lin = blockIdx.x; lin < ntiles; lin += gridDim.x) {
         if (lin != (int)blockIdx.x) __syncthreads();
         const int bx = lin % gx, rest = lin / gx;
-        f32_tile<RT, NT, KC, FUSE, SEQ>(p, lds, bx, rest % gy, rest / gy, gx, gy);
-    }
+        f32_tile<RT, NT, KC, FUSE, SEQ>(p, lds, bx, rest % gy, rest / gy, (rest % gy) * (32 * NT), lin);
+    }
+}
+
+template <int KC, int SEQ>
+__global__ __launch_bounds__(256, 2) void tapgemm_f32_pair_kernel(const TapGemmParams p)
+{
+    touch_kernargs<sizeof(TapGemmParams)>();
+    extern __shared__ __attribute__((aligned(16))) f32x4 lds[];
+    const PairTile t = f32_pair_tile((int)blockIdx.x, p.grid_x);
+    if (t.group >= p.grid_y) return;
+    const int n0 = t.group * (kPairWide + kPairNarrow);
+    if (!t.narrow) f32_tile<1, kPairWide / 32, KC, false, SEQ>(p, lds, t.bx, t.group, 0, n0, (int)blockIdx.x);
+    else if (n0 + kPairWide < p.Cout) f32_tile<1, kPairNarrow / 32, KC, false, SEQ>(p, lds, t.bx, t.group, 0, n0 + kPairWide, (int)blockIdx.x);
 }
 
 __global__ __launch_bounds__(64) void fc_out_f32_kernel(const TapGemmParams p)
@@ -646,9 +658,10 @@
 #define X(rt, nt, kc) {rt, nt, kc, 32},
     PNN_F32_CFGS(X)
 #undef X
+    {1, 5, 4, 32, 4, 2, 1}, {1, 5, 2, 32, 4, 2, 1},
 };
 
-static const int kRegsF32[] = {360, 360, 296, 296, 224, 176, 152, 116, 92, 492, 288, 252, 208, 360};
+static const int kRegsF32[] = {360, 360, 296, 296, 224, 176, 152, 116, 92, 492, 288, 252, 208, 360, 252, 220};
 static_assert(sizeof(kRegsF32) / sizeof(kRegsF32[0]) == sizeof(kCfgsF32) / sizeof(kCfgsF32[0]), "one register count per tile");
 int tapgemm_f32_regs(int idx) { return kRegsF32[idx]; }
 
@@ -659,7 +672,16 @@
     const size_t ring = (size_t)3 * t.kc * 4 * 32 * t.nt, out_tile = (size_t)128 * t.rt * (8 * t.nt + 1);
     return (std::max(ring, (row_out && !fuse) ? out_tile : (size_t)0) + (fuse ? (size_t)8 * t.nt * 64 : 0)) * 16;
 }
-bool tapgemm_f32_can_fuse(int idx) { return kCfgsF32[idx].rt == 1 && kCfgsF32[idx].nt == 5; }
+bool tapgemm_f32_can_fuse(int idx) { return kCfgsF32[idx].rt == 1 && kCfgsF32[idx].nt == 5 && !kCfgsF32[idx].pair; }
+
+static hipError_t set_lds_attr(const DeviceInfo& di, const void* fn, int (&done)[16])
+{
+    const int dev = di.dev >= 0 && di.dev < 16 ? di.dev : 0;
+    if (done[dev]) return hipSuccess;
+    const hipError_t e = hipFuncSetAttribute(fn, hipFuncAttributeMaxDynamicSharedMemorySize, (int)di.lds);
+    if (e == hipSuccess) done[dev] = 1;
+    return e;
+}
 
 template <int RT, int NT, int KC>
 static hipError_t launch_f32(const TapGemmParams& p0, bool fuse, hipStream_t s)
@@ -702,13 +724,7 @@
         g1.x = (unsigned)di.cus * (unsigned)W;
         lds = std::max(lds, (size_t)(di.lds / (W + 1) + 1024) / 16 * 16);
     }
-    auto set_attr = [&](const void* fn, int (&done)[16]) -> hipError_t {
-        const int dev = di.dev >= 0 && di.dev < 16 ? di.dev : 0;
-        if (done[dev]) return hipSuccess;
-        const hipError_t e = hipFuncSetAttribute(fn, hipFuncAttributeMaxDynamicSharedMemorySize, (int)di.lds);
-        if (e == hipSuccess) done[dev] = 1;
-        return e;
-    };
+    auto set_attr = [&](const void* fn, int (&done)[16]) { return set_lds_attr(di, fn, done); };
     const bool one_tap = p0.ncls == 1 && p0.tap_begin[1] - p0.tap_begin[0] == 1;
     if (seq && (one_tap ? (p0.seg_chunks == 0 || p0.seg_chunks % (2 * KC) || (long)(p0.nseg - 1) * p0.seg_chunks >= p0.Cin / 16) : ((p0.Cin / 16) % KC) != 0)) return hipErrorInvalidValue;
     if constexpr (RT == 1 && NT == 5) {
@@ -757,13 +773,56 @@
     return hipGetLastError();
 }
 
+thread_local int g_last_pair_mode = 0;
+
+template <int KC>
+static hipError_t launch_f32_pair(const TapGemmParams& p0, bool fuse, hipStream_t s)
+{
+    const bool seq = p0.nseg > 1 && p0.seg_seq;
+    const bool one_tap = p0.ncls == 1 && p0.tap_begin[1] - p0.tap_begin[0] == 1;
+    if (fuse || !one_tap || (p0.nseg > 1 && !seq)) return hipErrorInvalidValue;
+    if (seq && (p0.seg_chunks == 0 || p0.seg_chunks % (2 * KC) || (long)(p0.nseg - 1) * p0.seg_chunks >= p0.Cin / 16)) return hipErrorInvalidValue;
+    const DeviceInfo& di = device_info();
+    const void* const fn = seq ? (const void*)tapgemm_f32_pair_kernel<KC, 2> : (const void*)tapgemm_f32_pair_kernel<KC, 0>;
+    static int done[2][16] = {}, occ[2][16] = {};
+    hipError_t e = set_lds_attr(di, fn, done[seq]);
+    if (e != hipSuccess) return e;
+    const size_t lds = std::max(tapgemm_f32_lds_bytes(TileCfg{1, kPairWide / 32, KC, 32}, false, p0.SH * p0.SW == 1), (size_t)(di.lds / 3 + 1024) / 16 * 16);
+    const int dev = di.dev >= 0 && di.dev < 16 ? di.dev : 0;
+    if (!occ[seq][dev]) {
+        int n = 0;
+        e = hipOccupancyMaxActiveBlocksPerMultiprocessor(&n, fn, 256, lds);
+        if (e != hipSuccess) return e;
+        occ[seq][dev] = std::max(n, 1);
+    }
+    if ((p0.pair_occ > 0 ? p0.pair_occ : occ[seq][dev]) < 2) {
+        TapGemmParams q = p0;
+        q.persist = 0;
+        const hipError_t r = launch_f32<1, 5, KC>(q, false, s);
+        g_last_pair_mode = 2;
+        return r;
+    }
+    TapGemmParams p = p0;
+    int nwg = 0;
+    f32_pair_grid(p0.M, p0.Cout, &p.grid_x, &p.grid_y, &nwg);
+    p.grid_z = 1; p.pm_groups = 0;
+    g_last_issued_frac = 1.0;
+    g_last_pair_mode = 1;
+    if (seq) pnn_launch(tapgemm_f32_pair_kernel<KC, 2>, dim3((unsigned)nwg), dim3(256), lds, s, p);
+    else pnn_launch(tapgemm_f32_pair_kernel<KC, 0>, dim3((unsigned)nwg), dim3(256), lds, s, p);
+    return hipGetLastError();
+}
+
 hipError_t launch_tapgemm_f32(const TapGemmParams& p, int idx, bool fuse, hipStream_t s)
 {
     if (p.M <= 0) return hipSuccess;
+    g_last_pair_mode = 0;
     int i = 0;
 #define X(rt, nt, kc) if (idx == i++) return launch_f32<rt, nt, kc>(p, fuse, s);
     PNN_F32_CFGS(X)
 #undef X
+    if (idx == i++) return launch_f32_pair<4>(p, fuse, s);
+    if (idx == i++) return launch_f32_pair<2>(p, fuse, s);
     return hipErrorInvalidValue;
 }
 
diff --git a/context_adaptive_neural_network_based_prediction_amd/csrc/pnn_kernels.h b/context_adaptive_neural_network_based_prediction_amd/csrc/pnn_kernels.h
--- a/context_adaptive_neural_network_based_prediction_amd/csrc/pnn_kernels.h
+++ b/context_adaptive_neural_network_based_prediction_amd/csrc/pnn_kernels.h
@@ -72,7 +72,7 @@
     int nseg; union { unsigned seg_stride; unsigned seg_chunks; };
     int seg_seq;
     int grid_x, grid_y, grid_z;
-    int persist;
+    union { int persist; int pair_occ; };
 };
 static_assert(sizeof(TapGemmParams) <= 512, "the argument block of the tap-GEMM kernels: 8 lines of 64 bytes");
 inline int pack_tap(int dy, int dx) { return (int)(((unsigned)dy << 16) | ((unsigned)dx & 0xffffu)); }
@@ -80,7 +80,7 @@
 constexpr int kChunkPad = 4;
 constexpr int kSegDepth = 1600, kSegMinDepth = 2304;
 constexpr int kFcSegChunks = 20;
-struct TileCfg { int rt, nt, kc, mf, wm = 4, d = 2; };
+struct TileCfg { int rt, nt, kc, mf, wm = 4, d = 2, pair = 0; };
 int tapgemm_sp_num_cfgs();
 TileCfg tapgemm_sp_cfg(int idx);
 hipError_t launch_tapgemm_sp(const TapGemmParams& p, int idx, hipStream_t s);
@@ -111,6 +111,20 @@
 size_t tapgemm_f32_lds_bytes(const TileCfg& t, bool fuse, bool row_out = false);
 bool tapgemm_f32_can_fuse(int idx);
 int tapgemm_f32_regs(int idx);
+struct PairTile { int bx, group, narrow; };
+constexpr int kPairGridStep = 16, kPairWide = 96, kPairNarrow = 64;
+__host__ __device__ inline PairTile f32_pair_tile(int w, int gx)
+{
+    const int k = w >> 3, q = (k >> 1) * 8 + (w & 7);
+    return PairTile{q % gx, q / gx, (k ^ (k >> 5)) & 1};
+}
+inline void f32_pair_grid(int M, int Cout, int* gx, int* groups, int* nwg)
+{
+    *gx = (M + 127) / 128;
+    *groups = (Cout + kPairWide + kPairNarrow - 1) / (kPairWide + kPairNarrow);
+    *nwg = (*gx * *groups + 7) / 8 * kPairGridStep;
+}
+extern thread_local int g_last_pair_mode;
 hipError_t launch_tapgemm_f32(const TapGemmParams& p, int idx, bool fuse, hipStream_t s);
 long tapgemm_f32_small_tiles(const TapGemmParams& p);
 hipError_t launch_tapgemm_f32_small(const TapGemmParams& p, hipStream_t s, const float* host_input = nullptr, int deep_mode = 1);
diff --git a/context_adaptive_neural_network_based_prediction_amd/csrc/pnn_passes.cpp b/context_adaptive_neural_network_based_prediction_amd/csrc/pnn_passes.cpp
--- a/context_adaptive_neural_network_based_prediction_amd/csrc/pnn_passes.cpp
+++ b/context_adaptive_neural_network_based_prediction_amd/csrc/pnn_passes.cpp
@@ -182,6 +182,7 @@
         const TileCfg t = tapgemm_f32_cfg(code % ntile);
         if (fcseg && L.fc_seg_chunks % (2 * t.kc)) return false;
         if (fcseg && t.rt * t.nt >= 8) return false;
+        if (t.pair && (!one_tap || next || nseg > 1)) return false;
         return (one_tap || cpt % t.kc == 0) && (!next || tapgemm_f32_can_fuse(code % ntile));
     };
     float* const Yreal = Y;
@@ -189,6 +190,11 @@
     const int act_real = L.proto.act;
     std::function<hipError_t(int)> launch = [&, p, pseq, Yreal, bias_real, act_real, fcseg](int code) {
         if (code >= ntile) return launch_tapgemm_f32(pseq, code - ntile, false, s);
+        if (tapgemm_f32_cfg(code).pair) {
+            TapGemmParams q = p;
+            q.pair_occ = (int)std::max(0L, c->opt_f32_pair_occ);
+            return launch_tapgemm_f32(q, code, false, s);
+        }
         const hipError_t e = launch_tapgemm_f32(p, code, next != nullptr, s);
         if (e != hipSuccess || p.nseg <= 1 || fcseg) return e;
         return launch_seg_reduce(p.Y, p.nseg, out_floats, p.Cout, bias_real, act_real, Yreal, s);
@@ -199,7 +205,10 @@
     if (fcseg && !legal(cfg)) {
         const TileCfg want = tapgemm_f32_cfg(cfg);
         int alt = -1;
-        for (int i = 0; i < ntile; i++) if (legal(i) && (alt < 0 || (tapgemm_f32_cfg(i).rt == want.rt && tapgemm_f32_cfg(i).nt == want.nt))) alt = i;
+        for (int i = 0; i < ntile; i++) {
+            const TileCfg ti = tapgemm_f32_cfg(i);
+            if (legal(i) && (!ti.pair || want.pair) && (alt < 0 || (ti.rt == want.rt && ti.nt == want.nt && ti.pair == want.pair))) alt = i;
+        }
         if (alt < 0) return fail(c, PNN_E_ARG, "no tapgemm_f32 tile fits K segments of %d chunks", L.fc_seg_chunks);
         cfg = alt;
     }
@@ -229,13 +238,15 @@
     const TileCfg t = tapgemm_f32_cfg(cfg % ntile);
     if (tiles_out) *tiles_out = (int)((p.Cout + 32L * t.nt - 1) / (32L * t.nt));
     if (debug) fprintf(stderr, "[pnn] gemm M=%ld K=%.0f N=%d ncls=%d -> f32 cfg %d {rt %d, nt %d, kc %d}%s%s\n", M, L.k_total, p.Cout, p.ncls,
-                       cfg, t.rt, t.nt, t.kc, next ? " + fused output layer" : "",
+                       cfg, t.rt, t.nt, t.kc, t.pair ? " as paired 128 x 96 + 128 x 64 tiles" : next ? " + fused output layer" : "",
                        nseg > 1 ? (seq ? ", K segments in sequence" : ", K segments in parallel + reduce") : "");
     const int trc = timed_launch(c, 0, flops, env_profile(), [&] { return launch(cfg); },
                                  "[pnn-prof] M=%ld K=%.0f N=%d ncls=%d f32 cfg=%d rt=%d nt=%d kc=%d mf=%d us=%.1f tflops=%.1f\n", M, L.k_total,
                                  p.Cout, p.ncls, cfg, t.rt, t.nt, t.kc, t.mf);
     if (trc) return trc;
     if (nseg > 1 && !seq) c->stat_launches++;
+    if (g_last_pair_mode == 1) c->stat_pair_launches++;
+    if (g_last_pair_mode == 2) c->stat_pair_fallbacks++;
     c->stat_gemm_flops_skipped += flops * (1.0 - g_last_issued_frac);
     return env_f32_diag() ? diag_f32_tiles(c, L, seq ? pseq : p, cfg % ntile, next != nullptr, seq ? 1 : nseg, s) : PNN_OK;
 }
diff --git a/context_adaptive_neural_network_based_prediction_amd/csrc/pnn_tiles.cpp b/context_adaptive_neural_network_based_prediction_amd/csrc/pnn_tiles.cpp
--- a/context_adaptive_neural_network_based_prediction_amd/csrc/pnn_tiles.cpp
+++ b/context_adaptive_neural_network_based_prediction_amd/csrc/pnn_tiles.cpp
@@ -16,7 +16,7 @@
     const bool one_tap = (k_total == (double)cin);
     if (c->opt_f32_cfg >= 0 && c->opt_f32_cfg < tapgemm_f32_num_cfgs()) {
         const TileCfg t = tapgemm_f32_cfg((int)c->opt_f32_cfg);
-        if ((one_tap || cpt % t.kc == 0) && (!fused || tapgemm_f32_can_fuse((int)c->opt_f32_cfg))) { if (cost_out) *cost_out = 0.0; return (int)c->opt_f32_cfg; }
+        if ((one_tap || cpt % t.kc == 0) && (!fused || tapgemm_f32_can_fuse((int)c->opt_f32_cfg)) && (!t.pair || (one_tap && !fused))) { if (cost_out) *cost_out = 0.0; return (int)c->opt_f32_cfg; }
     }
     int best = -1;
     double best_cost = 1e300;
@@ -26,6 +26,7 @@
         const TileCfg t = tapgemm_f32_cfg(i);
         if (fused && !tapgemm_f32_can_fuse(i)) continue;
         if (!one_tap && cpt % t.kc) continue;
+        if (t.pair) continue;
         const long bm = 128L * t.rt, bn = 32L * t.nt;
         const double wgs = (double)((M + bm - 1) / bm) * (double)((cout + bn - 1) / bn) * ncls;
         const double regs = tapgemm_f32_regs(i);
@@ -43,6 +44,13 @@
         if (cost < best_cost) { best_cost = cost; best = i; }
     }
     if (cost_out) *cost_out = best_cost;
+    if (best >= 0 && one_tap && !fused) {
+        const TileCfg t = tapgemm_f32_cfg(best);
+        const double wgs = (double)((M + 127) / 128) * (double)((cout + 159) / 160) * ncls;
+        if (t.rt == 1 && t.nt == 5 && wgs == ncu)
+            for (int i = 0; i < tapgemm_f32_num_cfgs(); i++)
+                if (tapgemm_f32_cfg(i).pair && tapgemm_f32_cfg(i).kc == t.kc) return i;
+    }
     return best;
 }
 
diff --git a/include/pnn_hip.h b/include/pnn_hip.h
--- a/include/pnn_hip.h
+++ b/include/pnn_hip.h
@@ -38,6 +38,8 @@
 
 int pnn_num_split_configs(void);
 int pnn_num_f32_configs(void);
+int pnn_f32_pair_stats(const pnn_ctx* ctx, long* paired, long* fell_back);
+int pnn_f32_pair_tile(int M, int cout, int wg, int* num_wgs, int* row0, int* col0, int* cols);
 int pnn_cache_stats(pnn_ctx* ctx, long* hits, long* misses);
 
 
```

Result: faster. 18.05 million blocks/s (median of 6 runs) (+2.8%).
